# ezorita/seeq

Hardware: AMD Instinct MI355X
Metric: lines/s scanned (20 bp pattern, d=3, 150 bp reads; GB/s in gb_per_s) (higher is better)
Workload: dtype int (u16 automaton state ids; exact-pass columns u32 bit-vectors)

## Files before the change

### include/seeq_amd.h

```cpp
#ifndef SEEQ_AMD_H_
#define SEEQ_AMD_H_

#include <stddef.h>
#include <stdint.h>

#include "libseeq.h"

#ifdef __cplusplus
extern "C" {
#endif

#define SEEQ_AMD_VERSION "seeq-mi355x-0.1"

#define SEEQDEV_MAX_WLEN 512

#define SEEQDEV_WANT_COUNTLINES 0
#define SEEQDEV_WANT_COUNTMATCH 1
#define SEEQDEV_WANT_RECORDS    2

#define SEEQDEV_FASTA       0x100
#define SEEQDEV_SINGLELINE  0x200

typedef struct {
   uint32_t line;
// ... 39 lines not shown

const seeqdev_hit_t * seeqdevScanRecordsDevice(const seeqdev_scan_t * scan);
int seeqdevScanCopyRecords(seeqdev_scan_t * scan, seeqdev_hit_t * host_out, size_t first, size_t n);
int seeqdevScanCopyOffsets(seeqdev_scan_t * scan, uint64_t * host_out, size_t first, size_t n);

void * seeqdevHostAlloc(size_t bytes);
void   seeqdevHostFree(void * p);

void * seeqdevTextAlloc(size_t bytes, int candidates, float * probe_ms, int * nprobed);
typedef struct seeqdev_textinfo {
   float  probe_ms[12];
   int    nprobed;
   int    chosen;
   size_t allocated_bytes;
   size_t probe_peak_bytes;
} seeqdev_textinfo_t;
void * seeqdevTextAllocInfo(size_t bytes, int candidates, seeqdev_textinfo_t * info);
void * seeqdevTextAllocFor(seeqdev_scan_t * scan, size_t bytes, int candidates, seeqdev_textinfo_t * info);
void   seeqdevTextFree(void * d_text);

int seeqdevScanHost(seeqdev_scan_t * scan, const seeqdev_pattern_t * pat, const char * host_text, size_t nbytes,
                    int options, int want, seeqdev_counts_t * counts);

int seeqdevStringMatch(seeqdev_scan_t * scan, const seeqdev_pattern_t * pat, const char * data, size_t n, int options,
                       const seeqdev_hit_t ** rec, size_t * nrec);

int seeqdevScanHostBegin(seeqdev_scan_t * scan, const seeqdev_pattern_t * pat, const char * host_text, size_t nbytes,
                         int options, int want);
int seeqdevScanRunMulti(seeqdev_scan_t * scan, const seeqdev_pattern_t * const * pats, int npat, const void * d_text, size_t nbytes,
                        int options, int want, seeqdev_counts_t * counts);
int seeqdevScanHostMulti(seeqdev_scan_t * scan, const seeqdev_pattern_t * const * pats, int npat, const char * host_text, size_t nbytes,
                         int options, int want, seeqdev_counts_t * counts);
int seeqdevScanMultiRecords(const seeqdev_scan_t * scan, int k, const seeqdev_hit_t ** rec, size_t * nrec);
int seeqdevScanLastMulti(const seeqdev_scan_t * scan);

typedef struct {
   const void * bases;
   const void * nmask;
   uint64_t     nreads;
   uint32_t     read_len;
   uint32_t     stride;
   uint32_t     nstride;
} seeqdev_packed_t;
int  seeqdevScanPacked(seeqdev_scan_t * scan, const seeqdev_pattern_t * pat, const seeqdev_packed_t * batch, int options, int want);
long seeqdevPackReads(const char * text, size_t nbytes, uint32_t read_len, void * bases_out, void * nmask_out, uint32_t stride, uint32_t nstride);
int  seeqdevPackReadsDevice(const void * d_text, uint64_t nreads, uint32_t read_len, void * d_bases, void * d_nmask, uint32_t stride, uint32_t nstride,
                            void * hip_stream);

int seeqdevScanLastCopyMs(const seeqdev_scan_t * scan, float * h2d_ms);

int seeqdevScanSetProfiling(seeqdev_scan_t * scan, int on);
int seeqdevScanLastTimes(const seeqdev_scan_t * scan, float ms[4]);
int seeqdevScanLastLaunches(const seeqdev_scan_t * scan);
int seeqdevScanLastLaunchTimes(const seeqdev_scan_t * scan, float * ms, int cap);
float seeqdevScanLastClockMHz(const seeqdev_scan_t * scan);

int seeqdevSynthReads(void * d_out, uint64_t first, uint64_t n, int len, const char * pattern_plain, int plen,
                      int tau, uint64_t seed, void * hip_stream);

#ifdef __cplusplus
}
#endif
#endif
```

### seeq_amd/_capi.py

```python
import ctypes as C
import os
import subprocess

HERE = os.path.dirname(os.path.abspath(__file__))
LIB_PATH = os.path.join(HERE, "lib", "libseeq_amd.so")
CLI_PATH = os.path.join(HERE, "bin", "seeq")
CSRC = os.path.join(HERE, "csrc")

SQ_FIRST, SQ_BEST, SQ_ALL, SQ_COUNT = 0x00, 0x01, 0x02, 0x03
SQ_FAIL, SQ_CONVERT, SQ_IGNORE = 0x00, 0x04, 0x08
SQ_LINES, SQ_STREAM = 0x00, 0x10
SQ_ANY, SQ_MATCH, SQ_NOMATCH, SQ_COUNTLINES, SQ_COUNTMATCH = 0, 1, 2, 3, 4
WANT_COUNTLINES, WANT_COUNTMATCH, WANT_RECORDS = 0, 1, 2
SEEQDEV_FASTA, SEEQDEV_SINGLELINE = 0x100, 0x200


class match_t(C.Structure):
    _fields_ = [("start", C.c_size_t), ("end", C.c_size_t), ("dist", C.c_size_t)]


class seeq_t(C.Structure):
    _fields_ = [("hits", C.c_size_t), ("stacksize", C.c_size_t), ("match", C.POINTER(match_t)),
                ("bufsz", C.c_size_t), ("string", C.c_void_p), ("tau", C.c_int), ("wlen", C.c_int),
                ("keys", C.POINTER(C.c_char)), ("rkeys", C.POINTER(C.c_char)),
                ("dfa", C.c_void_p), ("rdfa", C.c_void_p)]


class seeqdev_packed_t(C.Structure):
    _fields_ = [("bases", C.c_void_p), ("nmask", C.c_void_p), ("nreads", C.c_uint64), ("read_len", C.c_uint32),
                ("stride", C.c_uint32), ("nstride", C.c_uint32)]


class seeqfile_t(C.Structure):
    _fields_ = [("flags", C.c_int), ("line", C.c_size_t), ("info", C.c_char_p), ("fdi", C.c_void_p)]


class seeqdev_hit_t(C.Structure):
    _fields_ = [("line", C.c_uint32), ("start", C.c_uint32), ("end", C.c_uint32), ("dist", C.c_uint32)]


class seeqdev_counts_t(C.Structure):
    _fields_ = [("nlines", C.c_uint64), ("nmatchlines", C.c_uint64), ("nhits", C.c_uint64),
                ("nrecords", C.c_uint64), ("nheaders", C.c_uint64)]


class seeqdev_textinfo_t(C.Structure):
    _fields_ = [("probe_ms", C.c_float * 12), ("nprobed", C.c_int), ("chosen", C.c_int), ("allocated_bytes", C.c_size_t),
                ("probe_peak_bytes", C.c_size_t)]


EXPORTS = [
    "seeqNew", "seeqFree", "seeqMatchIter", "seeqGetString", "seeqStringMatch", "seeqPrintError",
    "seeqAddMatch", "stackNew", "stackAddMatch", "recursive_merge", "seeqerr",
    "seeq", "seeqFileMatch", "seeqOpen", "seeqClose",
    "seeqdevDeviceCount", "seeqdevSetDevice", "seeqdevLastError", "seeqdevPatternNew", "seeqdevPatternFree",
    "seeqdevPatternOf", "seeqdevScanNew", "seeqdevScanFree", "seeqdevScanReserve", "seeqdevScanRun",
    "seeqdevScanFetch", "seeqdevScanRecordsDevice", "seeqdevScanCopyRecords", "seeqdevScanHost",
    "seeqdevScanSetProfiling", "seeqdevScanLastTimes", "seeqdevScanLastLaunches", "seeqdevScanLastLaunchTimes", "seeqdevScanLastClockMHz", "seeqdevSynthReads",
    "seeqdevScanSetLineHint", "seeqdevScanLastPath", "seeqdevScanLastFilter", "seeqdevScanLastPackedQuad", "seeqdevScanCopyOffsets", "seeqdevHostAlloc", "seeqdevTextAlloc", "seeqdevTextAllocInfo", "seeqdevTextAllocFor", "seeqdevTextFree",
    "seeqdevHostFree", "seeqdevStringMatch", "seeqdevScanHostBegin", "seeqdevScanLastCopyMs", "seeqdevPatternDevice",
    "seeqdevScanRunMulti", "seeqdevScanHostMulti", "seeqdevScanMultiRecords", "seeqdevScanLastMulti", "seeqdevScanPacked", "seeqdevPackReads", "seeqdevPackReadsDevice",
]


def build(verbose=False):
    cmd = ["make", "-C", CSRC, "all"]
    if not verbose:
        cmd.insert(1, "-s")
    subprocess.check_call(cmd)


_lib = None


def _share_torch_hip_runtime():
    if os.environ.get("SEEQ_AMD_SYSTEM_HIP") == "1":
        return
    import importlib.util
    try:
        spec = importlib.util.find_spec("torch")
    except (ImportError, ValueError):
        spec = None
    if spec is None or not spec.submodule_search_locations:
        return
    path = os.path.join(list(spec.submodule_search_locations)[0], "lib", "libamdhip64.so")
    if os.path.exists(path):
        C.CDLL(path, mode=C.RTLD_GLOBAL)


def lib():
    global _lib
    if _lib is not None:
        return _lib
    if not os.path.exists(LIB_PATH):
        raise OSError("%s is not built: run `python -c 'import __graft_entry__ as g; g.build()'` "
                      "or `make -C seeq_amd/csrc`; seeq_amd has no fallback matcher" % LIB_PATH)
    _share_torch_hip_runtime()
    L = C.CDLL(LIB_PATH, use_errno=True)
    P = C.POINTER
    L.seeqNew.argtypes = [C.c_char_p, C.c_int, C.c_size_t]
    L.seeqNew.restype = P(seeq_t)
    L.seeqFree.argtypes = [P(seeq_t)]
    L.seeqFree.restype = None
    L.seeqMatchIter.argtypes = [P(seeq_t)]
    L.seeqMatchIter.restype = P(match_t)
    L.seeqGetString.argtypes = [P(seeq_t)]
    L.seeqGetString.restype = C.c_char_p
    L.seeqStringMatch.argtypes = [C.c_char_p, P(seeq_t), C.c_int]
    L.seeqStringMatch.restype = C.c_long
    L.seeqPrintError.argtypes = []
    L.seeqPrintError.restype = C.c_char_p
    L.seeqAddMatch.argtypes = [P(seeq_t), match_t]
    L.seeqAddMatch.restype = C.c_int
    L.seeqOpen.argtypes = [C.c_char_p]
    L.seeqOpen.restype = P(seeqfile_t)
    L.seeqClose.argtypes = [P(seeqfile_t)]
    L.seeqClose.restype = C.c_int
    L.seeqFileMatch.argtypes = [P(seeqfile_t), P(seeq_t), C.c_int, C.c_int]
    L.seeqFileMatch.restype = C.c_long
    L.seeqdevDeviceCount.argtypes = []
    L.seeqdevDeviceCount.restype = C.c_int
    L.seeqdevSetDevice.argtypes = [C.c_int]
    L.seeqdevSetDevice.restype = C.c_int
    L.seeqdevLastError.argtypes = []
    L.seeqdevLastError.restype = C.c_char_p
    L.seeqdevPatternNew.argtypes = [C.c_char_p, C.c_int, C.c_int]
    L.seeqdevPatternNew.restype = C.c_void_p
    L.seeqdevPatternFree.argtypes = [C.c_void_p]
    L.seeqdevPatternFree.restype = None
    L.seeqdevPatternOf.argtypes = [P(seeq_t)]
    L.seeqdevPatternOf.restype = C.c_void_p
    L.seeqdevScanNew.argtypes = [C.c_void_p]
    L.seeqdevScanNew.restype = C.c_void_p
    L.seeqdevScanFree.argtypes = [C.c_void_p]
    L.seeqdevScanFree.restype = None
    L.seeqdevScanReserve.argtypes = [C.c_void_p, C.c_size_t, C.c_size_t, C.c_size_t, C.c_size_t]
    L.seeqdevScanReserve.restype = C.c_int
    L.seeqdevScanRun.argtypes = [C.c_void_p, C.c_void_p, C.c_void_p, C.c_size_t, C.c_int, C.c_int]
    L.seeqdevScanRun.restype = C.c_int
    L.seeqdevScanFetch.argtypes = [C.c_void_p, P(seeqdev_counts_t)]
    L.seeqdevScanFetch.restype = C.c_int
    L.seeqdevScanRecordsDevice.argtypes = [C.c_void_p]
    L.seeqdevScanRecordsDevice.restype = C.c_void_p
    L.seeqdevScanCopyRecords.argtypes = [C.c_void_p, C.c_void_p, C.c_size_t, C.c_size_t]
    L.seeqdevScanCopyRecords.restype = C.c_int
    L.seeqdevScanCopyOffsets.argtypes = [C.c_void_p, C.c_void_p, C.c_size_t, C.c_size_t]
    L.seeqdevScanCopyOffsets.restype = C.c_int
    L.seeqdevScanHost.argtypes = [C.c_void_p, C.c_void_p, C.c_char_p, C.c_size_t, C.c_int, C.c_int,
                                  P(seeqdev_counts_t)]
    L.seeqdevScanHost.restype = C.c_int
    L.seeqdevScanSetProfiling.argtypes = [C.c_void_p, C.c_int]
    L.seeqdevScanSetProfiling.restype = C.c_int
    L.seeqdevScanLastTimes.argtypes = [C.c_void_p, P(C.c_float)]
    L.seeqdevScanLastTimes.restype = C.c_int
    L.seeqdevScanLastLaunches.argtypes = [C.c_void_p]
    L.seeqdevScanLastLaunches.restype = C.c_int
    L.seeqdevScanLastLaunchTimes.argtypes = [C.c_void_p, P(C.c_float), C.c_int]
    L.seeqdevScanLastLaunchTimes.restype = C.c_int
    L.seeqdevScanLastClockMHz.argtypes = [C.c_void_p]
    L.seeqdevScanLastClockMHz.restype = C.c_float
    L.seeqdevScanSetLineHint.argtypes = [C.c_void_p, C.c_double]
    L.seeqdevScanSetLineHint.restype = C.c_int
    L.seeqdevScanLastPath.argtypes = [C.c_void_p]
    L.seeqdevScanLastPath.restype = C.c_int
    L.seeqdevScanLastFilter.argtypes = [C.c_void_p]
    L.seeqdevScanLastFilter.restype = C.c_int
    L.seeqdevScanLastPackedQuad.argtypes = [C.c_void_p]
    L.seeqdevScanLastPackedQuad.restype = C.c_int
    L.seeqdevScanRunMulti.argtypes = [C.c_void_p, C.POINTER(C.c_void_p), C.c_int, C.c_void_p, C.c_size_t, C.c_int, C.c_int, C.c_void_p]
    L.seeqdevScanRunMulti.restype = C.c_int
    L.seeqdevScanHostMulti.argtypes = [C.c_void_p, C.POINTER(C.c_void_p), C.c_int, C.c_char_p, C.c_size_t, C.c_int, C.c_int, C.c_void_p]
    L.seeqdevScanHostMulti.restype = C.c_int
    L.seeqdevScanMultiRecords.argtypes = [C.c_void_p, C.c_int, C.POINTER(C.c_void_p), C.POINTER(C.c_size_t)]
    L.seeqdevScanMultiRecords.restype = C.c_int
    L.seeqdevScanLastMulti.argtypes = [C.c_void_p]
    L.seeqdevScanLastMulti.restype = C.c_int
    L.seeqdevScanPacked.argtypes = [C.c_void_p, C.c_void_p, C.POINTER(seeqdev_packed_t), C.c_int, C.c_int]
    L.seeqdevScanPacked.restype = C.c_int
    L.seeqdevPackReads.argtypes = [C.c_char_p, C.c_size_t, C.c_uint32, C.c_void_p, C.c_void_p, C.c_uint32, C.c_uint32]
    L.seeqdevPackReads.restype = C.c_long
    L.seeqdevPackReadsDevice.argtypes = [C.c_void_p, C.c_uint64, C.c_uint32, C.c_void_p, C.c_void_p, C.c_uint32, C.c_uint32, C.c_void_p]
    L.seeqdevPackReadsDevice.restype = C.c_int
    L.seeqdevHostAlloc.argtypes = [C.c_size_t]
    L.seeqdevHostAlloc.restype = C.c_void_p
    L.seeqdevHostFree.argtypes = [C.c_void_p]
    L.seeqdevHostFree.restype = None
    L.seeqdevTextAlloc.argtypes = [C.c_size_t, C.c_int, C.POINTER(C.c_float), C.POINTER(C.c_int)]
    L.seeqdevTextAlloc.restype = C.c_void_p
    L.seeqdevTextAllocInfo.argtypes = [C.c_size_t, C.c_int, C.POINTER(seeqdev_textinfo_t)]
    L.seeqdevTextAllocInfo.restype = C.c_void_p
    L.seeqdevTextAllocFor.argtypes = [C.c_void_p, C.c_size_t, C.c_int, C.POINTER(seeqdev_textinfo_t)]
    L.seeqdevTextAllocFor.restype = C.c_void_p
    L.seeqdevTextFree.argtypes = [C.c_void_p]
    L.seeqdevTextFree.restype = None
    L.seeqdevSynthReads.argtypes = [C.c_void_p, C.c_uint64, C.c_uint64, C.c_int, C.c_char_p, C.c_int, C.c_int,
                                    C.c_uint64, C.c_void_p]
    L.seeqdevSynthReads.restype = C.c_int
    _lib = L
    return L


def seeqerr():
    return C.c_int.in_dll(lib(), "seeqerr").value


def error_text():
    L = lib()
    msg = L.seeqPrintError().decode(errors="replace")
    dev = L.seeqdevLastError().decode(errors="replace")
# ... 2 lines not shown
```

### seeq_amd/csrc/seeq_device.hip

```cpp
#include <hip/hip_runtime.h>

#include <errno.h>
#include <pthread.h>
#include <stdint.h>
#include <stdio.h>
#include <stdlib.h>
#include <string.h>
#include <time.h>

#include "seeq_amd.h"
#include "seeq_kernel_core.h"
extern "C" {
#include "seeq_pattern.h"
}

static thread_local char g_last_error[256] = "";

static int hip_fail(hipError_t e, const char *what, int err_no)
{
   snprintf(g_last_error, sizeof g_last_error, "%s: %s", what, hipGetErrorString(e));
   seeqerr = 0;
   errno = err_no;
   return -1;
}
// ... 741 lines not shown
      uint32_t *wg_part;
      uint32_t *wg_lastnl;
   } ow;
   size_t cap_ftiles, cap_slices;
   uint32_t *d_eqtab, *h_eqtab;
   unsigned long eq_pat_id; int eq_options;
   double avg_line;
   double line_hint;
   uint8_t *h_sample;
   const void *avg_text; size_t avg_nbytes;
   int force_path;
   int last_path;
   seeqdev_hit_t *records; uint64_t *rec_off; size_t cap_records;
   uint32_t *scan_ws;           size_t cap_scan_ws;
   uint32_t *lead_fidx, *lead_flag, *lead_wend; unsigned long long *lead_key; size_t cap_lead;
   Counters *d_cnt;
   Counters *h_cnt;
   uint8_t *h_str; size_t cap_str;
   uint32_t *h_strout; size_t cap_strout;
   uint32_t  str_seq;
   uint8_t *d_text; size_t cap_text;
   seeqdev_counts_t *multi_cnt; size_t *multi_first; int multi_n, cap_multi_n;
   seeqdev_hit_t *multi_rec; size_t cap_multi_rec, multi_nrec;
   struct MultiPlan *mplan;
   bool      multi_active;
   int       multi_rc;
   uint32_t *ml_mask, *ml_first, *ml_last; size_t cap_ml;
   uint32_t *mp_idx, *mp_nh; size_t cap_mp;
   uint32_t *m_bsum; size_t cap_m_bsum;
   Counters *d_mcnt, *h_mcnt;
   MultiExact *d_mx, *h_mx; size_t mx_slots, mx_next;
   uint32_t *m_scan_ws; size_t cap_m_scan_ws;
   int       last_multi;
   uint32_t *pk_cand, *pk_slot, *pk_coff; uint64_t *pk_bmask; size_t cap_pk_reads;
   uint8_t  *pk_stage; size_t cap_pk_stage;
   uint8_t  *d_unpack; size_t cap_unpack;
   uint32_t *pk_last; size_t cap_pk_last;
   bool      is_packed; seeqdev_packed_t packed;
   const seeqdev_pattern *pat; const void *text; size_t nbytes; int options, want;
   bool ran;
   seeqdev_counts_t counts;
   bool prof;
   hipEvent_t *ev;
   size_t nev_seg;
   size_t prof_segs;
   float acc_ms[4];
   float fwd_ms_avg;
   size_t seg_bytes;
   bool user_reserved;
   bool no_stream;
   bool force_ll;
   bool no_stream_nd;
   bool no_leaders;
   bool no_window;
   int  fallback_ttl;
   bool sample_dirty;
   unsigned sample_age;
};

static int ws_alloc(void **p, size_t bytes)
{
   void *g = NULL;
   hipError_t e = hipMalloc(&g, bytes ? bytes : 16);
   if (e != hipSuccess) { (void)hipGetLastError(); return hip_fail(e, "hipMalloc(workspace)", ENOMEM); }
   if (*p) (void)hipFree(*p);
   *p = g;
   return 0;
}

extern "C" seeqdev_scan_t *seeqdevScanNew(void *hip_stream)
{
   seeqerr = 0;
   if (seeqdevDeviceCount() < 1) {
      snprintf(g_last_error, sizeof g_last_error, "no HIP device: seeq-mi355x has no CPU matcher");
      errno = ENODEV;
      return NULL;
   }
   seeqdev_scan *s = (seeqdev_scan *)calloc(1, sizeof *s);
   if (!s) return NULL;
   if (hipGetDevice(&s->device) != hipSuccess) s->device = 0;
   s->seg_bytes = (size_t)0xF0000000u;
   const char *env = getenv("SEEQ_SEGMENT_BYTES");
   if (env && atoll(env) >= 65536) s->seg_bytes = ((size_t)atoll(env) + 15) & ~(size_t)15;
   if (s->seg_bytes > 0xFFFF0000ull) s->seg_bytes = 0xFFFF0000ull;
   hipError_t e = hipSuccess;
   if (hip_stream) s->stream = (hipStream_t)hip_stream;
   else {
      e = hipStreamCreateWithFlags(&s->stream, hipStreamDefault);
      s->own_stream = true;
   }
   if (e == hipSuccess) e = hipMalloc((void **)&s->d_cnt, sizeof(Counters));
   if (e == hipSuccess) e = hipHostMalloc((void **)&s->h_cnt, sizeof(Counters), hipHostMallocDefault);
   if (e == hipSuccess) e = hipHostMalloc((void **)&s->h_eqtab, 2048 * sizeof(uint32_t), hipHostMallocDefault);
   if (e == hipSuccess) e = hipMalloc((void **)&s->d_eqtab, 2048 * sizeof(uint32_t));
   if (e == hipSuccess) e = hipHostMalloc((void **)&s->h_sample, SAMPLE_BYTES, hipHostMallocDefault);
   {
      const char *pe = getenv("SEEQ_PATH");
      s->force_path = pe ? (!strcmp(pe, "generic") ? 1 : !strcmp(pe, "fused") ? 2 : 0) : 0;
      ScanKnobs &kn = s->knobs;
      const char *v;
      v = getenv("SEEQ_FUSED_KERNEL"); kn.kernel = v ? (!strcmp(v, "stream") ? 1 : !strcmp(v, "direct") ? 2 : !strcmp(v, "pair") ? 3 : 0) : 0;
      v = getenv("SEEQ_NO_LEADERS");   kn.no_leaders = v && atoi(v) == 1;
      v = getenv("SEEQ_TILE_BYTES");   kn.tile_bytes = v ? atoi(v) : 0;
      v = getenv("SEEQ_NO_FILTER");    kn.no_filter = v && atoi(v) == 1;
      v = getenv("SEEQ_STREAM_SUB");   kn.no_sub = v && atoi(v) == 0;
      v = getenv("SEEQ_STREAM_WU");    kn.min_wu = v ? atoi(v) : 0;
      v = getenv("SEEQ_NO_MYERS");     kn.no_myers = v && atoi(v) == 1;
      v = getenv("SEEQ_NO_WINDOW");    kn.no_window = v && atoi(v) == 1;
      v = getenv("SEEQ_EXPLAIN");      kn.explain = v && atoi(v) == 1;
      v = getenv("SEEQ_PACKED_QUAD");  kn.no_packed_quad = v && atoi(v) == 0;
      v = getenv("SEEQ_PACKED_SEG_READS");
      s->pk_seg_reads = v && atol(v) >= 64 && (size_t)atol(v) <= ((size_t)1 << 26) ? (size_t)atol(v) & ~(size_t)63 : PACKED_SEG_READS_DEFAULT;
      s->ncu = 256;
      s->lds_per_wg = 65536;
      s->lds_per_cu = 65536;
      int dev = 0;
      hipDeviceProp_t prop;
      if (e == hipSuccess && hipGetDevice(&dev) == hipSuccess && hipGetDeviceProperties(&prop, dev) == hipSuccess)
      { s->ncu = prop.multiProcessorCount; s->lds_per_wg = prop.sharedMemPerBlock; s->lds_per_cu = prop.maxSharedMemoryPerMultiProcessor; }
   }
   if (e != hipSuccess) {
      hip_fail(e, "seeqdevScanNew", EIO);
      seeqdevScanFree(s);
      return NULL;
   }
   return s;
}

extern "C" void seeqdevScanFree(seeqdev_scan_t *s)
{
   if (!s) return;
   (void)use_device(s->device);
   if (s->have_h2d_ev) { (void)hipEventDestroy(s->ev_h2d[0]); (void)hipEventDestroy(s->ev_h2d[1]); }
   (void)hipStreamSynchronize(s->stream);
   {
      void *ob[] = {s->ow.tile_cl, s->ow.tile_hits, s->ow.tile_dirty, s->ow.tile_dmask, s->ow.tmp, s->ow.wg_hits, s->ow.wg_part, s->ow.wg_lastnl};
      for (void *b : ob) if (b) (void)hipFree(b);
   }
   { void *pk[] = {s->pk_cand, s->pk_slot, s->pk_coff, s->pk_bmask, s->pk_stage, s->pk_last, s->d_unpack}; for (void *b : pk) if (b) (void)hipFree(b); }
   { void *mw[] = {s->ml_mask, s->ml_first, s->ml_last, s->mp_idx, s->mp_nh, s->m_bsum, s->d_mcnt, s->d_mx, s->m_scan_ws}; for (void *b : mw) if (b) (void)hipFree(b); }
   if (s->h_mcnt) (void)hipHostFree(s->h_mcnt);
   if (s->h_mx) (void)hipHostFree(s->h_mx);
   multi_plan_free(s->mplan);
   void *bufs[] = {s->rec_off, s->line_start, s->tile_cnt, s->hitmask, s->hdrmask, s->wave_off, s->hdr_off, s->hit_start,
                   s->hit_line, s->d_eqtab,
                   s->nh, s->hit_col, s->nh_sum, s->ent, s->records, s->scan_ws, s->lead_fidx, s->lead_flag, s->lead_wend, s->lead_key, s->d_cnt, s->d_text};
   for (void *b : bufs) if (b) (void)hipFree(b);
   if (s->h_cnt) (void)hipHostFree(s->h_cnt);
   if (s->h_eqtab) (void)hipHostFree(s->h_eqtab);
   if (s->h_sample) (void)hipHostFree(s->h_sample);
   if (s->h_str) (void)hipHostFree(s->h_str);
   if (s->h_strout) (void)hipHostFree(s->h_strout);
   for (size_t i = 0; i < 4 * s->nev_seg; i++) (void)hipEventDestroy(s->ev[i]);
   free(s->ev);
   free(s->launch_ms);
   if (s->clk_probe) (void)hipHostFree(s->clk_probe);
   free(s->multi_cnt); free(s->multi_first);
   if (s->multi_rec) (void)hipHostFree(s->multi_rec);
   if (s->own_stream && s->stream) (void)hipStreamDestroy(s->stream);
   free(s);
}

static int reserve_impl(seeqdev_scan *s, size_t max_bytes, size_t max_lines, size_t max_hitlines, size_t max_records)
{
   seeqerr = 0;
   if (!s) { errno = EINVAL; return -1; }
   if (max_bytes) {
      const size_t seg = max_bytes < s->seg_bytes ? max_bytes : s->seg_bytes;
      const size_t tiles = (seg + TILE - 1) / TILE + 1;
      if (tiles > s->cap_tiles) {
         if (ws_alloc((void **)&s->tile_cnt, tiles * sizeof(uint32_t))) return -1;
         s->cap_tiles = tiles;
      }
      const size_t ftiles = seg / FUSED_MIN_TILE + 2;
      const size_t slices = MAX_FUSED_GRID;
      if (ftiles > s->cap_ftiles) {
         if (ws_alloc((void **)&s->ow.tile_cl, ftiles * sizeof(uint32_t))) return -1;
         if (ws_alloc((void **)&s->ow.tile_dirty, ftiles * sizeof(uint32_t))) return -1;
         if (ws_alloc((void **)&s->ow.tile_dmask, ftiles * sizeof(uint64_t))) return -1;
         if (ws_alloc((void **)&s->ow.tile_hits, ftiles * sizeof(uint32_t))) return -1;
         s->cap_ftiles = ftiles;
      }
      if (slices > s->cap_slices) {
         if (ws_alloc((void **)&s->ow.wg_hits, slices * sizeof(uint32_t))) return -1;
         if (ws_alloc((void **)&s->ow.wg_part, 4 * slices * sizeof(uint32_t))) return -1;
         if (ws_alloc((void **)&s->ow.wg_lastnl, slices * sizeof(uint32_t))) return -1;
         s->cap_slices = slices;
      }
   }
   if (max_lines > s->cap_lines) {
      const size_t chunks = (max_lines + 63) / 64 + 1;
      if (ws_alloc((void **)&s->line_start, (max_lines + 1) * sizeof(uint32_t))) return -1;
      if (ws_alloc((void **)&s->hitmask, chunks * sizeof(uint64_t))) return -1;
      if (ws_alloc((void **)&s->hdrmask, chunks * sizeof(uint64_t))) return -1;
      if (ws_alloc((void **)&s->wave_off, chunks * sizeof(uint32_t))) return -1;
      if (ws_alloc((void **)&s->hdr_off, chunks * sizeof(uint32_t))) return -1;
      s->cap_lines = max_lines;
      s->cap_chunks = chunks;
   }
   if (max_hitlines > s->cap_hitlines) {
      if (ws_alloc((void **)&s->hit_start, max_hitlines * sizeof(uint32_t))) return -1;
      if (ws_alloc((void **)&s->hit_line, max_hitlines * sizeof(uint32_t))) return -1;
      if (ws_alloc((void **)&s->ow.tmp, max_hitlines * sizeof(uint4))) return -1;
      if (ws_alloc((void **)&s->nh, max_hitlines * sizeof(uint32_t))) return -1;
      if (ws_alloc((void **)&s->hit_col, max_hitlines * sizeof(uint32_t))) return -1;
      if (ws_alloc((void **)&s->ent, max_hitlines * sizeof(uint4))) return -1;
      if (ws_alloc((void **)&s->nh_sum, 2 * (max_hitlines / 256 + 2) * sizeof(uint32_t))) return -1;
      s->cap_hitlines = max_hitlines;
   }
   if (max_records > s->cap_records) {
      if (ws_alloc((void **)&s->records, max_records * sizeof(seeqdev_hit_t))) return -1;
      if (ws_alloc((void **)&s->rec_off, max_records * sizeof(uint64_t))) return -1;
      s->cap_records = max_records;
   }
   size_t largest = s->cap_tiles;
   if (s->cap_chunks > largest) largest = s->cap_chunks;
   if (s->cap_hitlines > largest) largest = s->cap_hitlines;
   if (s->cap_ftiles > largest) largest = s->cap_ftiles;
   size_t nb = largest / SCAN_BLOCK + 2;
   if (3 * (s->cap_ftiles / SCAN_BLOCK + 2) > nb) nb = 3 * (s->cap_ftiles / SCAN_BLOCK + 2);
   if (nb > s->cap_scan_ws) {
      if (ws_alloc((void **)&s->scan_ws, nb * sizeof(uint32_t))) return -1;
      s->cap_scan_ws = nb;
   }
   return 0;
}

extern "C" int seeqdevScanReserve(seeqdev_scan_t *s, size_t max_bytes, size_t max_lines, size_t max_hitlines,
                                  size_t max_records)
{
   if (reserve_impl(s, max_bytes, max_lines, max_hitlines, max_records)) return -1;
   if (max_lines) s->user_reserved = true;
   return 0;
}

extern "C" int seeqdevScanSetLineHint(seeqdev_scan_t *s, double avg_bytes_per_line)
{
   if (!s || avg_bytes_per_line < 0) { errno = EINVAL; return -1; }
   s->line_hint = avg_bytes_per_line;
   return 0;
}

extern "C" int seeqdevScanLastPath(const seeqdev_scan_t *s) { return s ? s->last_path : 0; }
extern "C" int seeqdevScanLastFilter(const seeqdev_scan_t *s) { return s && s->last_filter ? 1 : 0; }
extern "C" int seeqdevScanLastPackedQuad(const seeqdev_scan_t *s) { return s && s->last_packed_quad ? 1 : 0; }

extern "C" int seeqdevScanSetProfiling(seeqdev_scan_t *s, int on)
{
   if (!s) { errno = EINVAL; return -1; }
   s->prof = on != 0;
   return 0;
}

extern "C" int seeqdevScanLastTimes(const seeqdev_scan_t *s, float ms[4])
{
   if (!s || !ms) { errno = EINVAL; return -1; }
   for (int i = 0; i < 4; i++) ms[i] = s->acc_ms[i];
   return 0;
}

struct ScanSet { uint32_t *arr[3]; uint32_t *total[3]; };

__global__ __launch_bounds__(WG) void k_scanset_reduce(ScanSet ss, uint32_t *bsum, uint32_t n, uint32_t nb)
{
   __shared__ uint32_t s_wave[4];
   const uint32_t *in = ss.arr[blockIdx.y];
   const uint32_t base = blockIdx.x * SCAN_BLOCK;
   uint32_t v = 0;
#pragma unroll
   for (int k = 0; k < SCAN_ITEMS; k++) {
      const uint32_t i = base + threadIdx.x * SCAN_ITEMS + k;
      if (i < n) v += in[i];
   }
// ... 228 lines not shown
         }
         int per_cu = occupancy_of(s, stream_fn, 64 * nw, dfa_lds);
         if (per_cu < 0) return -1;
         fused_grid = (unsigned)(ncu * per_cu);
         if ((size_t)fused_grid * nw > MAX_FUSED_GRID) fused_grid = (unsigned)(MAX_FUSED_GRID / nw);
         nslices = fused_grid * nw;
      } else {
         nw = 4;
         double want = s->avg_line * 63.5;
         if (want < 512) want = 512;
         if (want > DIRECT_MAXRR * 1024) want = DIRECT_MAXRR * 1024;
         tile_bytes = ((uint32_t)want) & ~15u;
         if (kn.tile_bytes >= 512 && kn.tile_bytes <= DIRECT_MAXRR * 1024) tile_bytes = (uint32_t)kn.tile_bytes & ~15u;
         int per_cu = occupancy_of(s, fw == 1 ? (const void *)k_direct<4, 1> : (const void *)k_direct<4, 2>, 256, 0);
         if (per_cu < 0) return -1;
         fused_grid = (unsigned)(ncu * per_cu);
         if ((size_t)fused_grid * nw > MAX_FUSED_GRID) fused_grid = (unsigned)(MAX_FUSED_GRID / nw);
         nslices = fused_grid * nw;
      }
      if (eq_tables_upload(s, pat, options, fw)) return -1;
   }
   const bool use_direct = plan.use_direct;
   s->last_path = plan.path;
   s->last_filter = filter;
   const bool superset = plan.superset;
   const bool need_nh = plan.need_nh, nh_is_count = plan.nh_is_count;

   const size_t seg_bytes = single ? (nbytes ? nbytes : 1) : s->seg_bytes;
   if (single && nbytes > 0xFFFF0000ull) { seeqerr = 0; errno = E2BIG; return -1; }
   const size_t nseg = nbytes ? (nbytes + seg_bytes - 1) / seg_bytes : 0;
   s->prof_segs = 0;
   if (s->prof && nseg > s->nev_seg) {
      hipEvent_t *g = (hipEvent_t *)realloc(s->ev, 4 * nseg * sizeof(hipEvent_t));
      if (!g) { seeqerr = 0; errno = ENOMEM; return -1; }
      s->ev = g;
      for (size_t i = 4 * s->nev_seg; i < 4 * nseg; i++) HIP_TRY(hipEventCreate(&s->ev[i]), EIO);
      s->nev_seg = nseg;
   }
   if (s->prof) s->prof_segs = nseg;
   if (s->prof && nseg > s->cap_clk_probe) {
      if (s->clk_probe) (void)hipHostFree(s->clk_probe);
      s->clk_probe = nullptr; s->cap_clk_probe = 0;
      if (hipHostMalloc((void **)&s->clk_probe, nseg * 4 * sizeof(unsigned long long), hipHostMallocDefault) == hipSuccess) s->cap_clk_probe = nseg;
   }
   if (s->prof && s->clk_probe) memset(s->clk_probe, 0, nseg * 4 * sizeof(unsigned long long));
   s->clk_valid = s->prof && s->clk_probe && use_pair && use_fused;
   r.pat = pat; r.options = options; r.want = want;
   r.fw = fw; r.nw = nw; r.tile_bytes = tile_bytes; r.fused_grid = fused_grid; r.nslices = nslices; r.grid_lines = grid_lines;
   r.stream_fn = stream_fn; r.dfa_lds = dfa_lds; r.seg_bytes = seg_bytes; r.nseg = nseg;
   (void)use_direct; (void)superset; (void)need_nh; (void)nh_is_count; (void)use_myers;
   return 0;
}

static int seg_onepass(seeqdev_scan *s, const SegRun &r, ScanArgs &a, size_t sg, hipEvent_t *ev, bool &order2, uint32_t &stream_ntiles)
{
   const seeqdev_pattern *pat = r.pat;
   const int options = r.options, want = r.want, match_opt = r.options & 3, fw = r.fw, ncu = s->ncu;
   const ScanPlan &plan = r.plan;
   const bool fasta = (options & SEEQDEV_FASTA) != 0, single = (options & SEEQDEV_SINGLELINE) != 0;
   const bool use_stream = plan.use_stream, use_pair = plan.use_pair, use_myers = plan.use_myers, filter = plan.filter, use_fused = plan.use_fused, use_direct = plan.use_direct;
   const bool stream_ll = plan.stream_ll, superset = plan.superset, need_nh = plan.need_nh, nh_is_count = plan.nh_is_count;
   const int stream_sub = plan.stream_sub, stream_ch = 128, nw = r.nw;
   const uint32_t tile_bytes = r.tile_bytes;
   const unsigned fused_grid = r.fused_grid, nslices = r.nslices, grid_lines = r.grid_lines;
   const void *stream_fn = r.stream_fn;
   const size_t dfa_lds = r.dfa_lds, nbytes = s->nbytes;
   Counters *c = s->d_cnt;
   seeqdev_scan::OnePassWs &ow = s->ow;
   hipStream_t st = s->stream;
   (void)pat; (void)want; (void)match_opt; (void)fw; (void)ncu; (void)fasta; (void)single; (void)use_stream; (void)use_pair; (void)use_myers; (void)filter; (void)use_fused;
   (void)use_direct; (void)stream_ll; (void)superset; (void)need_nh; (void)nh_is_count; (void)stream_sub; (void)stream_ch; (void)nw; (void)tile_bytes; (void)fused_grid;
   (void)nslices; (void)grid_lines; (void)stream_fn; (void)dfa_lds; (void)nbytes; (void)c; (void)ow; (void)st;

   FusedArgs f;
   memset(&f, 0, sizeof f);
   f.text = a.text; f.nbytes = nbytes; f.seg_base = a.seg_base; f.seg_len = a.seg_len; f.first_seg = a.first_seg;
   f.tile_bytes = tile_bytes;
   f.ntiles = (uint32_t)(((uint64_t)a.seg_len + tile_bytes - 1) / tile_bytes);
   stream_ntiles = f.ntiles;
   f.eqtab = s->d_eqtab; f.peq = pat->d_peq;
   f.m = pat->wlen; f.tau = pat->tau; f.options = options; f.want = want;
   f.tile_cl = ow.tile_cl; f.tile_hits = ow.tile_hits; f.tmp = ow.tmp; f.cap_tmp = (uint32_t)s->cap_hitlines;
   f.wg_hits = ow.wg_hits; f.wg_part = ow.wg_part; f.wg_lastnl = stream_ll ? ow.wg_lastnl : nullptr;
   f.tile_dirty = f.wg_lastnl ? ow.tile_dirty : nullptr;
   f.tile_dmask = f.wg_lastnl ? ow.tile_dmask : nullptr;
   f.cnt = c;
   f.clk_probe = (s->prof && s->clk_probe && use_pair) ? s->clk_probe + 4 * sg : nullptr;
   uint32_t pos_bias = 0;
   if (use_stream) {
      f.dfa = stream_sub == 2 ? pat->d_sdfa_skip : plan.ll_restart ? pat->d_sdfa_restart : pat->d_sdfa; f.dfa_rows = pat->sdfa_rows; f.dfa_final_base = pat->sdfa_final_base;
      f.ll_filter = plan.ll_restart ? 2u : plan.ll_filter ? 1u : 0u;
      f.skip_thr = plan.skip_thr;
      if (use_pair) { f.dfa = pat->d_pair; f.dfa_rows = pat->pair_units; f.dfa_final_base = 0; f.pair = 1; f.ig_thr = plan.ig ? (uint32_t)(pat->wlen - pat->tau) : 0u; }
      if (use_myers) { f.dfa = (const uint16_t *)(s->d_eqtab + (size_t)512 * fw); f.dfa_rows = (uint32_t)(64 * fw); f.dfa_final_base = 0; f.pair = 2; }
      uint64_t room = 0xFFFFFFF0ull - a.seg_len;
      if (room > ((uint64_t)1 << 30)) room = (uint64_t)1 << 30;
      pos_bias = (uint32_t)(a.seg_base < room ? a.seg_base : room) & ~127u;
      f.pos_bias = pos_bias;
   }
   if (ev) { HIP_TRY(hipEventRecord(ev[0], st), EIO); HIP_TRY(hipEventRecord(ev[1], st), EIO); }
   unsigned fgrid = fused_grid;
   const unsigned nsl = nslices;
   f.slice_cap = f.cap_tmp / nsl;
   if (use_stream) {
      void *kargs[] = {&f};
      HIP_TRY(hipLaunchKernel(stream_fn, dim3(fgrid), dim3(64 * (unsigned)nw), kargs, dfa_lds, st), EIO);
   }
   else if (use_direct && fw == 2) hipLaunchKernelGGL((k_direct<4, 2>), dim3(fgrid), dim3(256), 0, st, f);
   else hipLaunchKernelGGL((k_direct<4, 1>), dim3(fgrid), dim3(256), 0, st, f);
   if (ev) HIP_TRY(hipEventRecord(ev[2], st), EIO);
   const uint32_t order_nb = (f.ntiles + SEEQ_ORDER_BLOCK - 1) / SEEQ_ORDER_BLOCK;
   order2 = plan.order2 && order_nb <= SEEQ_ORDER_MAX_BLOCKS && 2 * (size_t)order_nb <= s->cap_scan_ws;
   if (plan.ig) {
      if (!order2) { snprintf(g_last_error, sizeof g_last_error, "SQ_IGNORE on k_pair needs the three-launch ordering (segment too large for its block sums)"); seeqerr = 0; errno = EIO; return -1; }
      a.ig_thr = f.ig_thr; a.ig_ent = (const uint4 *)s->ent;
      {
         static const char base_of_key[9] = {0, 'A', 'C', 0, 'G', 0, 0, 0, 'T'};
         int cnt[4] = {0, 0, 0, 0}, best = 3;
         for (int i = 0; i < pat->wlen; i++) { const int kb = pat->keys[i] & 0x1F; if (kb == 1) cnt[0]++; else if (kb == 2) cnt[1]++; else if (kb == 4) cnt[2]++; else if (kb == 8) cnt[3]++; }
         for (int b = 2; b >= 0; b--) if (cnt[b] > cnt[best]) best = b;
         const int need = cnt[best] - pat->tau;
         a.ig_need = need > 0 ? (uint32_t)need : 0u;
         a.ig_bval = (uint32_t)(unsigned char)base_of_key[1 << best];
         a.ig_bmask = best == 3 ? 0xDEu : 0xDFu;
      }
   }
   if (order2) {
      const unsigned rgrid = nsl / 4 + 1 < 2048 ? nsl / 4 + 1 : 2048;
      seeq_launch_tiles_post(st, f, (uint32_t)nsl, s->scan_ws, order_nb);
      seeq_launch_order(rgrid, st, f, (uint32_t)nsl, (const uint32_t *)s->scan_ws, order_nb, s->ent);
   }
   else hipLaunchKernelGGL(k_fused_post, dim3(1), dim3(256), 0, st, f, (uint32_t)nsl);
   if (!order2 && (want != SEEQDEV_WANT_COUNTLINES || superset)) {
      launch_scanset(s, st, f.tile_hits, f.tile_cl, f.tile_dirty, f.ntiles, nullptr, nullptr, f.tile_dirty ? &c->seg_dirty_tiles : nullptr);
      const unsigned rgrid = nsl / 4 + 1 < 2048 ? nsl / 4 + 1 : 2048;
      if (use_stream) hipLaunchKernelGGL(k_stream_reorder, dim3(rgrid), dim3(256), 0, st, f, (uint32_t)nsl, s->hit_start, s->hit_line, s->nh, s->hit_col);
      else hipLaunchKernelGGL(k_fused_reorder, dim3(rgrid), dim3(256), 0, st, f, (uint32_t)nsl, s->hit_start, s->hit_line);
   }
   a.seg_base -= pos_bias;
   a.pos_bias = pos_bias;
   a.tile_dirty = f.tile_dirty; a.tile_dmask = f.tile_dmask; a.stream_ntiles = f.ntiles; a.stream_tile_bytes = tile_bytes;
   a.stream_ch = stream_ll ? (uint32_t)stream_ch : 0u;
   a.walk_ext = plan.walk_ext; a.ll_restart = plan.ll_restart ? 1u : 0u;
   return 0;
}

template <int W>
static int seg_index_forward(seeqdev_scan *s, const SegRun &r, ScanArgs &a, hipEvent_t *ev)
{
   const seeqdev_pattern *pat = r.pat;
   const int options = r.options, want = r.want, match_opt = r.options & 3, fw = r.fw, ncu = s->ncu;
   const ScanPlan &plan = r.plan;
   const bool fasta = (options & SEEQDEV_FASTA) != 0, single = (options & SEEQDEV_SINGLELINE) != 0;
   const bool use_stream = plan.use_stream, use_pair = plan.use_pair, use_myers = plan.use_myers, filter = plan.filter, use_fused = plan.use_fused, use_direct = plan.use_direct;
   const bool stream_ll = plan.stream_ll, superset = plan.superset, need_nh = plan.need_nh, nh_is_count = plan.nh_is_count;
   const int stream_sub = plan.stream_sub, stream_ch = 128, nw = r.nw;
   const uint32_t tile_bytes = r.tile_bytes;
   const unsigned fused_grid = r.fused_grid, nslices = r.nslices, grid_lines = r.grid_lines;
   const void *stream_fn = r.stream_fn;
   const size_t dfa_lds = r.dfa_lds, nbytes = s->nbytes;
   Counters *c = s->d_cnt;
   seeqdev_scan::OnePassWs &ow = s->ow;
   hipStream_t st = s->stream;
   (void)pat; (void)want; (void)match_opt; (void)fw; (void)ncu; (void)fasta; (void)single; (void)use_stream; (void)use_pair; (void)use_myers; (void)filter; (void)use_fused;
   (void)use_direct; (void)stream_ll; (void)superset; (void)need_nh; (void)nh_is_count; (void)stream_sub; (void)stream_ch; (void)nw; (void)tile_bytes; (void)fused_grid;
   (void)nslices; (void)grid_lines; (void)stream_fn; (void)dfa_lds; (void)nbytes; (void)c; (void)ow; (void)st;

   if (ev) HIP_TRY(hipEventRecord(ev[0], st), EIO);
   if (single) {
      hipLaunchKernelGGL(k_single_line, dim3(1), dim3(1), 0, st, a);
   } else {
      hipLaunchKernelGGL(k_nl_count, dim3(a.ntiles), dim3(WG), 0, st, a);
      hipLaunchKernelGGL(k_scan_tiles, dim3(1), dim3(WG), 0, st, a.tile_cnt, a.ntiles, &c->seg_nlines);
      hipLaunchKernelGGL(k_index_finalize, dim3(1), dim3(1), 0, st, a);
      hipLaunchKernelGGL(k_nl_write, dim3(a.ntiles), dim3(WG), 0, st, a);
   }
   if (ev) HIP_TRY(hipEventRecord(ev[1], st), EIO);
   hipLaunchKernelGGL(k_forward<W>, dim3(grid_lines), dim3(WG), 0, st, a);
   if (ev) HIP_TRY(hipEventRecord(ev[2], st), EIO);
   launch_scan<1>(s, st, a.hitmask, a.wave_off, s->cap_chunks, &c->seg_nlines, 63u, 6u, &c->seg_nhitlines);
   if (fasta) launch_scan<1>(s, st, a.hdrmask, a.hdr_off, s->cap_chunks, &c->seg_nlines, 63u, 6u, &c->seg_nheaders);
   return 0;
}

template <int W>
static int seg_post(seeqdev_scan *s, const SegRun &r, ScanArgs &a, hipEvent_t *ev, bool order2, uint32_t stream_ntiles)
{
   const seeqdev_pattern *pat = r.pat;
   const int options = r.options, want = r.want, match_opt = r.options & 3, fw = r.fw, ncu = s->ncu;
   const ScanPlan &plan = r.plan;
   const bool fasta = (options & SEEQDEV_FASTA) != 0, single = (options & SEEQDEV_SINGLELINE) != 0;
   const bool use_stream = plan.use_stream, use_pair = plan.use_pair, use_myers = plan.use_myers, filter = plan.filter, use_fused = plan.use_fused, use_direct = plan.use_direct;
   const bool stream_ll = plan.stream_ll, superset = plan.superset, need_nh = plan.need_nh, nh_is_count = plan.nh_is_count;
// ... 66 lines not shown
   #define SEEQ_COUNT1(WW, WK) hipLaunchKernelGGL((k_exact1<SQ_MODE_COUNT, WW, -1, WK>), dim3(grid_hits), dim3(WG), 0, st, a, eqp, hcol, ecache)
         if (fw == 2) { if (a.stream_ch) SEEQ_COUNT1(2, true); else SEEQ_COUNT1(2, false); }
         else { if (a.stream_ch) SEEQ_COUNT1(1, true); else SEEQ_COUNT1(1, false); }
   #undef SEEQ_COUNT1
      }
      else hipLaunchKernelGGL((k_exact<W, SQ_MODE_COUNT>), dim3(grid_hits), dim3(WG), 0, st, a);
      if (leaders) {
         hipLaunchKernelGGL(k_lead_check, dim3(grid_hits), dim3(256), 0, st, a, (const uint32_t *)s->hit_col, (const uint32_t *)s->lead_flag, lead_wback);
         if (lead_best) {
            hipLaunchKernelGGL(k_lead_best, dim3(grid_hits), dim3(256), 0, st, a, (const uint32_t *)s->lead_fidx, s->lead_key, (const uint4 *)ecache, 0);
            hipLaunchKernelGGL(k_lead_best, dim3(grid_hits), dim3(256), 0, st, a, (const uint32_t *)s->lead_fidx, s->lead_key, (const uint4 *)ecache, 1);
         }
         else hipLaunchKernelGGL(k_lead_lines, dim3(grid_hits < 512 ? grid_hits : 512), dim3(256), 0, st, a, (const uint32_t *)s->lead_fidx, s->lead_flag);
      }
      else if (superset && nh_is_count) hipLaunchKernelGGL(k_count_nonzero, dim3(grid_hits < 512 ? grid_hits : 512), dim3(WG), 0, st, a);
      launch_scan<0>(s, st, a.nh, a.nh, s->cap_hitlines, &c->seg_nhitlines, 0u, 0u, &c->seg_nrec);
   }
   if (want == SEEQDEV_WANT_RECORDS && !emitted) {
      if (!verify) hipLaunchKernelGGL(k_rec_check, dim3(1), dim3(1), 0, st, a);
      if (use_fused) {
         const uint32_t *eqp = (const uint32_t *)s->d_eqtab;
         const int mo = (options & 3) == SQ_COUNT ? SQ_FIRST : (options & 3);
   #define SEEQ_EMIT1(WW, OO, WK) hipLaunchKernelGGL((k_exact1<SQ_MODE_EMIT, WW, OO, WK>), dim3(grid_hits), dim3(WG), 0, st, a, eqp, hcol, ecache)
         if (a.stream_ch) {
            if (fw == 2) { if (mo == SQ_BEST) SEEQ_EMIT1(2, SQ_BEST, true); else SEEQ_EMIT1(2, -1, true); }
            else { if (mo == SQ_BEST) SEEQ_EMIT1(1, SQ_BEST, true); else SEEQ_EMIT1(1, -1, true); }
         } else {
            if (fw == 2) { if (mo == SQ_BEST) SEEQ_EMIT1(2, SQ_BEST, false); else SEEQ_EMIT1(2, -1, false); }
            else { if (mo == SQ_BEST) SEEQ_EMIT1(1, SQ_BEST, false); else SEEQ_EMIT1(1, -1, false); }
         }
   #undef SEEQ_EMIT1
      }
      else {
         hipLaunchKernelGGL((k_exact<W, SQ_MODE_EMIT>), dim3(grid_hits), dim3(WG), 0, st, a);
         hipLaunchKernelGGL(k_rec_offsets, dim3(grid_hits), dim3(WG), 0, st, a);
      }
   }
   return 0;
}

template <int W>
static int run_segments(seeqdev_scan *s)
{
   Counters *c = s->d_cnt;
   HIP_TRY(hipMemsetAsync(c, 0, sizeof(Counters), s->stream), EIO);
   SegRun r;
   memset(&r, 0, sizeof r);
   { const int rc = run_setup(s, r); if (rc) return rc; }
   const seeqdev_pattern *pat = r.pat;
   const ScanPlan &plan = r.plan;
   const int options = r.options, want = r.want;
   const size_t nbytes = s->nbytes, seg_bytes = r.seg_bytes, nseg = r.nseg;
   const bool use_stream = plan.use_stream, use_fused = plan.use_fused, filter = plan.filter, superset = plan.superset, need_nh = plan.need_nh, nh_is_count = plan.nh_is_count;
   for (size_t sg = 0; sg < nseg; sg++) {

      hipEvent_t *ev = s->prof ? s->ev + 4 * sg : NULL;
      uint32_t stream_ntiles = 0;
      bool order2 = false;
      hipStream_t st = s->stream;
      ScanArgs a;
      memset(&a, 0, sizeof a);
      a.text = (const uint8_t *)s->text;
      a.nbytes = nbytes;
      a.seg_base = (uint64_t)sg * seg_bytes;
      a.seg_len = (uint32_t)((nbytes - a.seg_base) < seg_bytes ? (nbytes - a.seg_base) : seg_bytes);
      a.first_seg = sg == 0;
      a.peq = pat->d_peq;
      a.m = pat->wlen; a.tau = pat->tau; a.options = options; a.want = want;
      a.line_start = s->line_start; a.cap_lines = (uint32_t)s->cap_lines;
      a.tile_cnt = s->tile_cnt; a.ntiles = (a.seg_len + TILE - 1) / TILE;
      a.hitmask = s->hitmask; a.hdrmask = s->hdrmask; a.wave_off = s->wave_off; a.hdr_off = s->hdr_off;
      a.hit_start = s->hit_start; a.hit_line = s->hit_line; a.cap_hitlines = (uint32_t)s->cap_hitlines; a.nh = s->nh;
      a.records = s->records; a.cap_records = s->cap_records; a.rec_off = s->rec_off;
      a.use_nh = need_nh ? (use_stream ? 3u : 1u) : 0u;
      a.filter = filter ? 1u : 0u;
      a.skip_back = plan.skip_back;
      a.window_ok = plan.window_ok ? 1u : 0u;
      a.cnt = c;

      if (use_fused) { if (seg_onepass(s, r, a, sg, ev, order2, stream_ntiles)) return -1; }
      else if (seg_index_forward<W>(s, r, a, ev)) return -1;
      if (want != SEEQDEV_WANT_COUNTLINES || superset) {
         const int pr = seg_post<W>(s, r, a, ev, order2, stream_ntiles);
         if (pr < 0) return pr;
         if (pr > 0) continue;
      }
      if (!a.fin) hipLaunchKernelGGL(k_seg_end, dim3(1), dim3(1), 0, st, a, (need_nh ? 1 : 0) | (superset && !nh_is_count ? 2 : 0));
      if (ev) HIP_TRY(hipEventRecord(ev[3], st), EIO);
      HIP_TRY(hipGetLastError(), EIO);
   }
   HIP_TRY(hipMemcpyAsync(s->h_cnt, c, sizeof(Counters), hipMemcpyDeviceToHost, s->stream), EIO);
   return 0;
}


static int run_packed(seeqdev_scan *s)
{
   const seeqdev_pattern *pat = s->pat;
   const seeqdev_packed_t &b = s->packed;
   const int options = s->options, want = s->want;
   const int match_opt = options & 3;
   const bool nh_is_count = want == SEEQDEV_WANT_COUNTMATCH || (want == SEEQDEV_WANT_RECORDS && match_opt == SQ_ALL);
   const int fw = pat->wlen <= FUSED_MAX_WLEN ? 1 : 2;
   Counters *c = s->d_cnt;
   hipStream_t st = s->stream;
   const uint32_t L = b.read_len;
   const bool direct = !(want == SEEQDEV_WANT_RECORDS && match_opt == SQ_ALL);
   const uint32_t pitch = (L + 1u + 15u) & ~15u;
   size_t PACKED_SEG_READS = s->pk_seg_reads;
   const size_t stage_lines_max = (size_t)(0xFFFF0000ull / pitch);
   if (!direct && PACKED_SEG_READS + 64u * MAX_FUSED_GRID > stage_lines_max)
      PACKED_SEG_READS = (stage_lines_max - 64u * MAX_FUSED_GRID) & ~(size_t)63;
   const size_t seg_reads = b.nreads < PACKED_SEG_READS ? (size_t)b.nreads : PACKED_SEG_READS;
   const size_t cap_use = (!direct && s->cap_hitlines > stage_lines_max) ? stage_lines_max : s->cap_hitlines;
   if (seg_reads > s->cap_pk_reads) {
      if (ws_alloc((void **)&s->pk_cand, seg_reads * sizeof(uint32_t))) return -1;
      if (ws_alloc((void **)&s->pk_slot, seg_reads * sizeof(uint32_t))) return -1;
      if (ws_alloc((void **)&s->pk_coff, (seg_reads / 64 + 1) * sizeof(uint32_t))) return -1;
      if (ws_alloc((void **)&s->pk_bmask, (seg_reads / 64 + 1) * sizeof(uint64_t))) return -1;
      s->cap_pk_reads = seg_reads;
   }
   if (!direct && cap_use * (size_t)pitch > s->cap_pk_stage) {
      if (ws_alloc((void **)&s->pk_stage, cap_use * (size_t)pitch + 64)) return -1;
      s->cap_pk_stage = cap_use * (size_t)pitch;
   }
   if (s->cap_hitlines > s->cap_pk_last) {
      if (ws_alloc((void **)&s->pk_last, s->cap_hitlines * sizeof(uint32_t))) return -1;
      s->cap_pk_last = s->cap_hitlines;
   }
   {
      const size_t nb = seg_reads / SCAN_BLOCK + 2;
      if (nb > s->cap_scan_ws) { if (ws_alloc((void **)&s->scan_ws, nb * sizeof(uint32_t))) return -1; s->cap_scan_ws = nb; }
   }
   if (eq_tables_upload(s, pat, options, fw)) return -1;
   HIP_TRY(hipMemsetAsync(c, 0, sizeof(Counters), st), EIO);
   s->clk_valid = false;
   const bool quad = pat->quad_state == 1 && !s->knobs.no_packed_quad && (pat->quad_pacc - pat->pair_pacc) * (double)L <= 0.04;
   s->last_packed_quad = quad;
   const size_t dfa_lds = quad ? (size_t)pat->quad_units * 16 : (size_t)pat->pair_units * 16;
   const void *walk_fn = quad ? (const void *)k_packed_walk<true> : (const void *)k_packed_walk<false>;
   int per_cu = occupancy_of(s, walk_fn, 64 * STREAM_NW, dfa_lds);
   if (per_cu < 0) return -1;
   unsigned wgrid = (unsigned)(s->ncu * per_cu);
   {
      const size_t nblocks = (seg_reads + 63) / 64, need = (nblocks + STREAM_NW_HOST - 1) / STREAM_NW_HOST;
      if (need < wgrid) wgrid = (unsigned)(need ? need : 1);
   }
   const size_t hit_blocks = (s->cap_hitlines + WG - 1) / WG;
   unsigned grid_hits = (unsigned)(hit_blocks < (size_t)s->ncu * 16 ? hit_blocks : (size_t)s->ncu * 16);
   if (grid_hits == 0) grid_hits = 1;
   const size_t nseg = (size_t)((b.nreads + PACKED_SEG_READS - 1) / PACKED_SEG_READS);
   s->prof_segs = 0;
   if (s->prof && nseg > s->nev_seg) {
      hipEvent_t *g = (hipEvent_t *)realloc(s->ev, 4 * nseg * sizeof(hipEvent_t));
      if (!g) { seeqerr = 0; errno = ENOMEM; return -1; }
      s->ev = g;
      for (size_t i = 4 * s->nev_seg; i < 4 * nseg; i++) HIP_TRY(hipEventCreate(&s->ev[i]), EIO);
      s->nev_seg = nseg;
   }
   if (s->prof) s->prof_segs = nseg;
   for (size_t sg = 0; sg < nseg; sg++) {
      hipEvent_t *ev = s->prof ? s->ev + 4 * sg : NULL;
      PackedArgs p;
      memset(&p, 0, sizeof p);
      p.bases = (const uint8_t *)b.bases; p.nmask = (const uint8_t *)b.nmask;
      p.first = (uint64_t)sg * PACKED_SEG_READS;
      p.nreads = (uint32_t)(b.nreads - p.first < PACKED_SEG_READS ? b.nreads - p.first : PACKED_SEG_READS);
      p.read_len = L; p.stride = b.stride; p.nstride = b.nstride;
      p.total_bytes = b.nreads * (uint64_t)b.stride;
      p.dfa = quad ? pat->d_quad : pat->d_pair; p.dfa_units = quad ? pat->quad_units : pat->pair_units;
      p.cand = s->pk_cand; p.cslot = s->pk_slot; p.boff = s->pk_coff; p.bmask = s->pk_bmask; p.stage = direct ? nullptr : s->pk_stage;
      p.wave_cap = (uint32_t)(cap_use / ((size_t)wgrid * STREAM_NW_HOST));
      p.pitch = pitch;
      p.hit_start = s->hit_start; p.hit_line = s->hit_line; p.hit_col = s->hit_col; p.hit_last = s->pk_last; p.nh = s->nh;
      p.cap = (uint32_t)cap_use;
      p.line_base = p.first;
      p.cnt = c;
      if (ev) { HIP_TRY(hipEventRecord(ev[0], st), EIO); HIP_TRY(hipEventRecord(ev[1], st), EIO); }
      {
         void *kargs[] = {&p};
         HIP_TRY(hipLaunchKernel(walk_fn, dim3(wgrid), dim3(64 * STREAM_NW), kargs, dfa_lds, st), EIO);
      }
      if (ev) HIP_TRY(hipEventRecord(ev[2], st), EIO);
      launch_scanset(s, st, s->pk_coff, nullptr, nullptr, (p.nreads + 63u) >> 6, &c->seg_nhitlines, nullptr, nullptr);
      hipLaunchKernelGGL(k_packed_counts, dim3(1), dim3(1), 0, st, p);
      hipLaunchKernelGGL(k_packed_list, dim3((unsigned)(((size_t)p.nreads / 1024 + 4) / 4)), dim3(256), 0, st, p);
      ScanArgs a;
      memset(&a, 0, sizeof a);
      a.text = direct ? nullptr : s->pk_stage;
      a.nbytes = direct ? 0 : cap_use * (uint64_t)pitch;
      a.seg_base = 0; a.seg_len = (uint32_t)a.nbytes; a.first_seg = sg == 0;
      a.peq = pat->d_peq;
      a.m = pat->wlen; a.tau = pat->tau; a.options = options & ~(MASK_NONDNA | MASK_INPUT); a.want = want;
      a.hit_start = s->hit_start; a.hit_line = s->hit_line; a.cap_hitlines = (uint32_t)s->cap_hitlines; a.nh = s->nh;
      a.records = s->records; a.cap_records = s->cap_records; a.rec_off = s->rec_off;
      a.use_nh = 3u; a.filter = 1u;
      a.skip_back = (uint32_t)(pat->wlen + pat->tau);
      a.hit_last = s->pk_last;
      a.window_ok = 1u;
      a.cnt = c;
      a.rec_pitch = L + 1u;
      const uint32_t *eqp = (const uint32_t *)s->d_eqtab;
      const uint32_t *hcol = s->hit_col;
      uint4 *ecache = want == SEEQDEV_WANT_RECORDS ? s->ow.tmp : nullptr;
      const int seg_flags = 1 | (!nh_is_count ? 2 : 0);
      {
         const bool count_any = want != SEEQDEV_WANT_COUNTMATCH && !(want == SEEQDEV_WANT_RECORDS && match_opt == SQ_ALL);
         const int var = (want == SEEQDEV_WANT_RECORDS && match_opt == SQ_BEST) ? VERIFY_BEST : count_any ? VERIFY_ANY : VERIFY_ALL;
         a.nh_sum = s->nh_sum;
         a.nz_sum = nh_is_count ? s->nh_sum + (s->cap_hitlines / 256 + 2) : nullptr;
         a.fin = (want == SEEQDEV_WANT_RECORDS && var == VERIFY_ALL) ? 0u : 1u + (uint32_t)seg_flags;
         if (direct) seeq_launch_verify_packed(fw, var, grid_hits, st, a, b.bases, b.nmask, b.stride, b.nstride, L, p.total_bytes,
                                               b.nmask ? b.nreads * (uint64_t)b.nstride : 0ull, eqp, hcol, ecache);
// ... 138 lines not shown
   if (nh_is_count) hipLaunchKernelGGL(k_multi_count_nonzero, dim3(grid_hits < 128 ? grid_hits : 128, (unsigned)npat), dim3(WG), 0, st, (const MultiExact *)dx);
   hipLaunchKernelGGL(k_multi_scan_reduce, dim3(nbp, (unsigned)npat), dim3(WG), 0, st, (const MultiExact *)dx);
   hipLaunchKernelGGL(k_multi_scan_top, dim3((unsigned)npat), dim3(WG), 0, st, (const MultiExact *)dx, want == SEEQDEV_WANT_RECORDS ? 1 : 0);
   hipLaunchKernelGGL(k_multi_scan_apply, dim3(nbp, (unsigned)npat), dim3(WG), 0, st, (const MultiExact *)dx);
   if (want == SEEQDEV_WANT_RECORDS) {
      if (mo == SQ_BEST) {
         if (n1) hipLaunchKernelGGL((k_exact1m<SQ_MODE_EMIT, 1, SQ_BEST>), dim3(grid_hits, (unsigned)n1), dim3(WG), 0, st, (const MultiExact *)dx);
         if (n2) hipLaunchKernelGGL((k_exact1m<SQ_MODE_EMIT, 2, SQ_BEST>), dim3(grid_hits, (unsigned)n2), dim3(WG), 0, st, (const MultiExact *)(dx + n1));
      } else {
         if (n1) hipLaunchKernelGGL((k_exact1m<SQ_MODE_EMIT, 1, -1>), dim3(grid_hits, (unsigned)n1), dim3(WG), 0, st, (const MultiExact *)dx);
         if (n2) hipLaunchKernelGGL((k_exact1m<SQ_MODE_EMIT, 2, -1>), dim3(grid_hits, (unsigned)n2), dim3(WG), 0, st, (const MultiExact *)(dx + n1));
      }
   }
   hipLaunchKernelGGL(k_multi_seg_end, dim3((unsigned)npat), dim3(1), 0, st, (const MultiExact *)dx);
   HIP_TRY(hipGetLastError(), EIO);
   return 0;
}

static int dispatch_run(seeqdev_scan *s)
{
   if (s->is_packed) return run_packed(s);
   const int W = s->pat->words;
   if (W <= 1) return run_segments<1>(s);
   if (W <= 2) return run_segments<2>(s);
   if (W <= 4) return run_segments<4>(s);
   if (W <= 8) return run_segments<8>(s);
   return run_segments<16>(s);
}

static int scan_setup(seeqdev_scan_t *s, const seeqdev_pattern_t *pat, const void *d_text, size_t nbytes, int options, int want, int hl_div);

extern "C" int seeqdevScanRun(seeqdev_scan_t *s, const seeqdev_pattern_t *pat, const void *d_text, size_t nbytes,
                              int options, int want)
{
   if (scan_setup(s, pat, d_text, nbytes, options, want, 8)) return -1;
   if (dispatch_run(s)) return -1;
   s->ran = true;
   return 0;
}

static int scan_setup(seeqdev_scan_t *s, const seeqdev_pattern_t *pat, const void *d_text, size_t nbytes, int options, int want, int hl_div)
{
   seeqerr = 0;
   if (!s || !pat || (!d_text && nbytes) || want < 0 || want > 2) { errno = EINVAL; return -1; }
   if (pat->device != s->device) {
      snprintf(g_last_error, sizeof g_last_error, "pattern lives on device %d, scan context on device %d", pat->device, s->device);
      errno = EINVAL;
      return -1;
   }
   if (use_device(s->device)) return -1;
   s->pat = pat; s->text = d_text; s->nbytes = nbytes; s->options = options; s->want = want;
   s->ran = false;
   s->is_packed = false;
   if ((s->no_stream || s->no_stream_nd || s->force_ll || s->no_window || s->no_leaders) && --s->fallback_ttl <= 0) s->no_stream = s->no_stream_nd = s->force_ll = s->no_window = s->no_leaders = false;
   const size_t seg = nbytes < s->seg_bytes ? nbytes : s->seg_bytes;
   size_t want_lines = s->cap_lines, want_hl = s->cap_hitlines, want_rec = s->cap_records;
   if (!s->user_reserved) {
      const size_t guess = (options & SEEQDEV_SINGLELINE) ? 1 : seg / 32 + 1024;
      if (guess > want_lines) want_lines = guess;
      if (want_lines / (size_t)hl_div + 1024 > want_hl) want_hl = want_lines / (size_t)hl_div + 1024;
      if (!(options & SEEQDEV_SINGLELINE) && want_hl < (size_t)8192 * 64) want_hl = (size_t)8192 * 64;
      if (want_hl > want_rec) want_rec = want_hl;
   }
   if (reserve_impl(s, nbytes ? nbytes : 1, want_lines, want_hl, want_rec)) return -1;
   if (s->line_hint > 0) {
      s->avg_line = s->line_hint;
   } else if (!(options & SEEQDEV_SINGLELINE) && nbytes && (s->avg_text != d_text || s->avg_nbytes != nbytes || ++s->sample_age >= 64)) {
      s->sample_age = 0;
      const size_t n = nbytes < SAMPLE_BYTES ? nbytes : SAMPLE_BYTES;
      HIP_TRY(hipMemcpyAsync(s->h_sample, d_text, n, hipMemcpyDeviceToHost, s->stream), EIO);
      HIP_TRY(hipStreamSynchronize(s->stream), EIO);
      size_t nl = 0;
      size_t foreign = 0;
      for (size_t i = 0; i < n; i++) {
         const uint8_t b = s->h_sample[i];
         nl += b == '\n';
         foreign += b != '\n' && sq_class_of(b, 0) >= 5;
      }
      s->avg_line = nl ? (double)n / (double)nl : 1e9;
      s->sample_dirty = foreign * 4096 > n;
      s->avg_text = d_text;
      s->avg_nbytes = nbytes;
   }
   return 0;
}

extern "C" int seeqdevScanFetch(seeqdev_scan_t *s, seeqdev_counts_t *counts)
{
   seeqerr = 0;
   if (!s || !s->ran) { errno = EINVAL; return -1; }
   if (use_device(s->device)) return -1;
   for (int attempt = 0; attempt < 8; attempt++) {
      HIP_TRY(hipStreamSynchronize(s->stream), EIO);
      const Counters h = *s->h_cnt;
      if (!h.overflow) {
         s->counts.nlines = h.lines;
         s->counts.nmatchlines = h.matchlines;
         s->counts.nhits = h.hits;
         s->counts.nrecords = h.records;
         s->counts.nheaders = h.headers;
         if (counts) *counts = s->counts;
         for (int i = 0; i < 4; i++) s->acc_ms[i] = 0.f;
         s->fwd_ms_avg = 0.f;
         for (size_t sg = 0; sg < s->prof_segs; sg++) {
            hipEvent_t *ev = s->ev + 4 * sg;
            float t01 = 0, t12 = 0, t23 = 0;
            if (sg == 0 && s->prof_segs > s->cap_launch_ms) {
               float *g = (float *)realloc(s->launch_ms, s->prof_segs * sizeof(float));
               if (g) { s->launch_ms = g; s->cap_launch_ms = s->prof_segs; }
            }
            (void)hipEventElapsedTime(&t01, ev[0], ev[1]);
            (void)hipEventElapsedTime(&t12, ev[1], ev[2]);
            (void)hipEventElapsedTime(&t23, ev[2], ev[3]);
            s->acc_ms[0] += t01; s->acc_ms[1] += t12; s->acc_ms[2] += t23; s->acc_ms[3] += t01 + t12 + t23;
            if (sg < s->cap_launch_ms) s->launch_ms[sg] = t12;
         }
         s->clk_mhz = 0.f;
         if (s->clk_valid && s->prof_segs && s->clk_probe && s->cap_clk_probe >= s->prof_segs) {
            double sum = 0; size_t nn = 0;
            for (size_t sg = 0; sg < s->prof_segs; sg++) {
               const unsigned long long *q = s->clk_probe + 4 * sg;
               if (q[3] > q[1] && q[2] > q[0]) { sum += (double)(q[2] - q[0]) / (double)(q[3] - q[1]) * 100.0; nn++; }
            }
            if (nn) s->clk_mhz = (float)(sum / (double)nn);
         }
         if (s->prof_segs) s->fwd_ms_avg = s->acc_ms[1] / (float)s->prof_segs;
         s->h2d_ms = 0.f;
         if (s->prof && s->have_h2d_ev) (void)hipEventElapsedTime(&s->h2d_ms, s->ev_h2d[0], s->ev_h2d[1]);
         return 0;
      }
      size_t nl = s->cap_lines, nhl = s->cap_hitlines, nrec = s->cap_records;
      if (h.overflow & 1u) nl = (size_t)h.need_lines + (h.need_lines >> 3) + 64;
      if (h.overflow & 2u) nhl = (size_t)h.need_hitlines + (h.need_hitlines >> 3) + 64;
      if (h.overflow & 64u) {
         snprintf(g_last_error, sizeof g_last_error, "internal inconsistency in the hit list (k_stream_bounds)");
         errno = EIO;
         return -1;
      }
      if (h.overflow & 8u) s->no_stream = true;
      if (h.overflow & 16u) s->no_stream_nd = true;
      if (h.overflow & 32u) s->force_ll = true;
      if (h.overflow & 128u) s->no_window = true;
      if (h.overflow & 256u) s->no_leaders = true;
      if (h.overflow & (8u | 16u | 32u | 128u | 256u)) s->fallback_ttl = 32;
      if (h.overflow & 4u) {
         nrec = (size_t)h.need_records + (size_t)(h.need_records >> 3) + 64;
      }
      if ((h.overflow & 1u) && nhl < nl / 8) nhl = nl / 8 + 64;
      if (attempt == 7) break;
      if (reserve_impl(s, s->nbytes, nl, nhl, nrec)) return -1;
      if (dispatch_run(s)) return -1;
   }
   snprintf(g_last_error, sizeof g_last_error, "workspace did not converge");
   errno = ENOMEM;
   return -1;
}

extern "C" const seeqdev_hit_t *seeqdevScanRecordsDevice(const seeqdev_scan_t *s) { return s ? s->records : NULL; }

extern "C" int seeqdevScanCopyRecords(seeqdev_scan_t *s, seeqdev_hit_t *host_out, size_t first, size_t n)
{
   seeqerr = 0;
   if (!s || (!host_out && n)) { errno = EINVAL; return -1; }
   if (first + n > s->counts.nrecords) { errno = EINVAL; return -1; }
   if (n == 0) return 0;
   if (use_device(s->device)) return -1;
   HIP_TRY(hipMemcpyAsync(host_out, s->records + first, n * sizeof(seeqdev_hit_t), hipMemcpyDeviceToHost, s->stream),
           EIO);
   HIP_TRY(hipStreamSynchronize(s->stream), EIO);
   return 0;
}

extern "C" int seeqdevScanPacked(seeqdev_scan_t *s, const seeqdev_pattern_t *pat, const seeqdev_packed_t *batch, int options, int want)
{
   seeqerr = 0;
   if (!s || !pat || !batch || want < 0 || want > 2 || (batch->nreads && !batch->bases)) { errno = EINVAL; return -1; }
   if (batch->read_len < 1 || batch->read_len > 256 || batch->stride < (batch->read_len + 3) / 4 ||
       (batch->nmask && batch->nstride < (batch->read_len + 7) / 8) || (options & (MASK_INPUT | SEEQDEV_FASTA | SEEQDEV_SINGLELINE))) { errno = EINVAL; return -1; }
   if (pat->device != s->device) { errno = EINVAL; return -1; }
   if (use_device(s->device)) return -1;
   seeqdev_pattern *mp = const_cast<seeqdev_pattern *>(pat);
   if (pat->wlen <= FUSED_MAX_WLEN2 && __atomic_load_n(&mp->pair_state, __ATOMIC_ACQUIRE) == 0) pattern_plan_pair(mp);
   if (pat->wlen <= FUSED_MAX_WLEN2 && mp->pair_state == 1 && __atomic_load_n(&mp->quad_state, __ATOMIC_ACQUIRE) == 0) pattern_plan_quad(mp);
   if (pat->wlen > FUSED_MAX_WLEN2 || mp->pair_state != 1) {
      const size_t tbytes = (size_t)batch->nreads * (batch->read_len + 1u);
      if (tbytes > s->cap_unpack) {
         if (ws_alloc((void **)&s->d_unpack, tbytes + 64)) return -1;
         s->cap_unpack = tbytes;
      }
      if (batch->nreads) {
         const uint64_t threads = batch->nreads * (uint64_t)(batch->read_len / 16u + 1u), blocks = (threads + 255) / 256;
         if (blocks > 0x7FFFFFFFull) { errno = E2BIG; return -1; }
         hipLaunchKernelGGL(k_unpack_ascii, dim3((unsigned)blocks), dim3(256), 0, s->stream, (const uint8_t *)batch->bases, (const uint8_t *)batch->nmask,
                            batch->nreads, batch->read_len, batch->stride, batch->nstride, s->d_unpack);
         HIP_TRY(hipGetLastError(), EIO);
      }
      s->avg_text = NULL;
// ... 346 lines not shown
   }
   s->multi_nrec = 0;
   for (int k = 0; k < npat; k++) {
      if (seeqdevScanRun(s, pats[k], d_text, nbytes, options, want)) return -1;
      if (seeqdevScanFetch(s, &s->multi_cnt[k])) return -1;
      s->multi_first[k] = s->multi_nrec;
      const size_t n = want == SEEQDEV_WANT_RECORDS ? (size_t)s->multi_cnt[k].nrecords : 0;
      if (n) {
         if (multi_grow_host(s, n)) return -1;
         if (seeqdevScanCopyRecords(s, s->multi_rec + s->multi_nrec, 0, n)) return -1;
         s->multi_nrec += n;
      }
      if (counts) counts[k] = s->multi_cnt[k];
   }
   s->multi_first[npat] = s->multi_nrec;
   s->multi_n = npat;
   return 0;
}

extern "C" int seeqdevScanLastMulti(const seeqdev_scan_t *s) { return s ? s->last_multi : 0; }

extern "C" int seeqdevScanHostMulti(seeqdev_scan_t *s, const seeqdev_pattern_t *const *pats, int npat, const char *host_text, size_t nbytes,
                                    int options, int want, seeqdev_counts_t *counts)
{
   seeqerr = 0;
   if (!s || !pats || npat < 1 || (!host_text && nbytes)) { errno = EINVAL; return -1; }
   if (use_device(s->device)) return -1;
   if (nbytes > s->cap_text) {
      const size_t cap = nbytes + (nbytes >> 2) + 4096;
      if (ws_alloc((void **)&s->d_text, cap)) return -1;
      s->cap_text = cap;
   }
   if (nbytes) HIP_TRY(hipMemcpyAsync(s->d_text, host_text, nbytes, hipMemcpyHostToDevice, s->stream), EIO);
   s->avg_text = NULL;
   return seeqdevScanRunMulti(s, pats, npat, s->d_text, nbytes, options, want, counts);
}

extern "C" int seeqdevScanMultiRecords(const seeqdev_scan_t *s, int k, const seeqdev_hit_t **rec, size_t *nrec)
{
   if (!s || !rec || !nrec || k < 0 || k >= s->multi_n) { errno = EINVAL; return -1; }
   *rec = s->multi_rec + s->multi_first[k];
   *nrec = s->multi_first[k + 1] - s->multi_first[k];
   return 0;
}

extern "C" int seeqdevScanLastCopyMs(const seeqdev_scan_t *s, float *h2d_ms)
{
   if (!s || !h2d_ms) { errno = EINVAL; return -1; }
   *h2d_ms = s->h2d_ms;
   return 0;
}

extern "C" int seeqdevScanLastLaunches(const seeqdev_scan_t *s) { return s ? (int)s->prof_segs : 0; }

extern "C" float seeqdevScanLastClockMHz(const seeqdev_scan_t *s) { return s ? s->clk_mhz : 0.f; }

extern "C" int seeqdevScanLastLaunchTimes(const seeqdev_scan_t *s, float *ms, int cap)
{
   if (!s || (!ms && cap > 0)) { errno = EINVAL; return -1; }
   const size_t n = s->prof_segs < s->cap_launch_ms ? s->prof_segs : s->cap_launch_ms;
   for (size_t i = 0; i < n && (int)i < cap; i++) ms[i] = s->launch_ms[i];
   return (int)n;
}

static constexpr uint32_t STRING_LDS_MAX = 48u * 1024;
static constexpr uint32_t STRING_ZC_MAX = 4096;
static constexpr uint32_t STRING_PAR_MAX = 32768;

template <int W>
__global__ __launch_bounds__(WG) void k_string(const uint8_t *text, uint32_t n, const uint32_t *peq, int m, int tau, int options,
                                               uint32_t *out, uint32_t cap, uint32_t seq)
{
   extern __shared__ __align__(16) uint8_t s_text[];
   __shared__ uint32_t s_peq[10 * W];
   __shared__ uint8_t s_lut[256];
   const int Wp = (m + 31) >> 5;
   for (int i = threadIdx.x; i < 10 * W; i += WG) {
      const int dir = i / (5 * W), rem = i % (5 * W), cls = rem / W, w = rem % W;
      s_peq[i] = w < Wp ? peq[(dir * 5 + cls) * Wp + w] : 0u;
   }
   for (int b = threadIdx.x; b < 256; b += WG) s_lut[b] = sq_class_of((uint32_t)b, options);
   const bool staged = n <= STRING_LDS_MAX;
   if (staged) {
      for (uint32_t o = threadIdx.x * 16; o < n; o += WG * 16) {
         const sq_chunk16_t c = sq_load16(text, o, n);
         *reinterpret_cast<uint4 *>(s_text + o) = make_uint4(c.w[0], c.w[1], c.w[2], c.w[3]);
      }
   }
   __shared__ uint32_t s_first, s_skip, s_key, s_wave[WG / 64];
   const bool par = n <= STRING_PAR_MAX;
   if (threadIdx.x == 0) { s_first = n; s_skip = 0; s_key = 0xFFFFFFFFu; }
   __syncthreads();
   if (par) {
      for (uint32_t j = threadIdx.x; j < n; j += WG) if (s_lut[s_text[j]] == SQC_TERM) atomicMin(&s_first, j);
      __syncthreads();
      const uint32_t len = s_first;
      for (uint32_t j = threadIdx.x; j < len; j += WG) if (s_lut[s_text[j]] == SQC_SKIP) s_skip = 1u;
      __syncthreads();
      if (!s_skip) {
         const int match_opt = options & 3;
         const uint32_t *peq_f = s_peq, *peq_r = s_peq + 5 * W;
         uint16_t *ed = reinterpret_cast<uint16_t *>(s_text + (((size_t)n + 31) & ~(size_t)15));
         const uint32_t P = len + 1;
         const uint32_t B = (P + WG - 1) / WG;
         const uint32_t j0 = threadIdx.x * B, j1 = j0 + B < P ? j0 + B : P;
         const uint32_t cnt = j0 < P ? sq_emit_window<W>((const uint8_t *)s_text, len, j0, j1, peq_f, (const uint8_t *)s_lut, m, tau, ed) : 0u;
// ... 136 lines not shown
```

### seeq_amd/csrc/seeq_exact1.h

```cpp
#ifndef SEEQ_EXACT1_H_
#define SEEQ_EXACT1_H_

#define EXACT1_ROW 80
typedef __attribute__((address_space(3))) uint8_t exact1_lds_u8;
typedef __attribute__((address_space(3))) const uint8_t exact1_lds_cu8;

template <int W>
__device__ __forceinline__ uint32_t exact1_reverse(const uint8_t *text, uint64_t off, uint64_t nbytes, uint32_t i, uint32_t streak,
                                                   uint32_t eqr_base, uint32_t m, uint32_t tau1, uint8_t *row)
{
   const uint8_t *line = text + off;
   uint32_t lim = 0;
   if (row) {
      const uint64_t end = off + i;
      const uint64_t base = end >= 64 ? end - 64 : 0;
      lim = (uint32_t)(end - base);
#pragma unroll
      for (int q = 0; q < 4; q++)
         *reinterpret_cast<fused_v4u *>(row + 16 * q) = direct_load16(text, base + 16 * q, nbytes);
   }
   fused_state_t<W> st;
   st.init(m);
   uint32_t j = 0, d = tau1, last_d, ignores = 0;
   do {
// ... 68 lines not shown
       !exact1_clean_in_tile(a, segb + t_hi * TB, a.tile_dmask[t_hi], segb + t_hi * TB, hi)) return false;
   return true;
}

template <int W> __device__ __forceinline__ void exact1_take(fused_state_t<W> &st, const fused_state_t<W> &s2, bool take);
template <> __device__ __forceinline__ void exact1_take<1>(fused_state_t<1> &st, const fused_state_t<1> &s2, bool take)
{
   st.pv = take ? s2.pv : st.pv; st.mv = take ? s2.mv : st.mv; st.score = take ? s2.score : st.score;
}
template <> __device__ __forceinline__ void exact1_take<2>(fused_state_t<2> &st, const fused_state_t<2> &s2, bool take)
{
   st.pv0 = take ? s2.pv0 : st.pv0; st.pv1 = take ? s2.pv1 : st.pv1;
   st.mv0 = take ? s2.mv0 : st.mv0; st.mv1 = take ? s2.mv1 : st.mv1; st.score = take ? s2.score : st.score;
}

template <int MODE, int W, int OPT, bool WALK>
__device__ __forceinline__ void exact1_body(const ScanArgs &a, const uint32_t *eq2, const uint32_t *hit_col, uint4 *cache)
{
   __shared__ __align__(8) uint32_t s_eqf[256 * W];
   __shared__ __align__(8) uint32_t s_eqr[256 * W];
   __shared__ __align__(16) uint8_t s_blk[256 * EXACT1_ROW];
   __shared__ uint32_t s_novf[4];
   if (threadIdx.x < 4) s_novf[threadIdx.x] = 0;
   for (int i = threadIdx.x; i < 256 * W; i += 256) { s_eqf[i] = eq2[i]; s_eqr[i] = eq2[256 * W + i]; }
   __syncthreads();
   const uint32_t eqf_base = (uint32_t)(uintptr_t)(fused_lds_cu32 *)s_eqf;
   const uint32_t eqr_base = (uint32_t)(uintptr_t)(fused_lds_cu32 *)s_eqr;
   const Counters *c = a.cnt;
   const uint32_t nhl = c->seg_nhitlines;
   const int match_opt = OPT >= 0 ? OPT : (a.options & 3);
   if (MODE == SQ_MODE_EMIT && (c->overflow & 4u)) return;
   const uint32_t m = (uint32_t)a.m, tau1 = (uint32_t)a.tau + 1;
   const bool count_any = a.want != SEEQDEV_WANT_COUNTMATCH && !(a.want == SEEQDEV_WANT_RECORDS && match_opt == SQ_ALL);
   const bool by_nh = a.use_nh != 0;
   const bool trusted = a.use_nh == 3 && !a.filter && !c->dirty;
   const bool caching = MODE == SQ_MODE_COUNT && cache != nullptr && a.want == SEEQDEV_WANT_RECORDS;
   const bool count_best = caching && match_opt == SQ_BEST;
   const bool cache_ok = MODE == SQ_MODE_EMIT && cache != nullptr && by_nh && !(trusted && count_any);
   const uint32_t ovf_r = (a.cap_hitlines > nhl ? a.cap_hitlines - nhl : 0u) / (gridDim.x * 4u);
   const uint32_t wave_id = threadIdx.x >> 6;
   uint4 *ovf = cache ? cache + nhl + (size_t)(blockIdx.x * 4u + wave_id) * ovf_r : nullptr;
   const bool ovf_lost = MODE == SQ_MODE_EMIT && c->seg_novf != 0;
   const bool walk = WALK && a.use_nh == 3 && hit_col != nullptr && a.stream_ch != 0;
   const uint32_t wback = a.skip_back > 32u ? a.skip_back : 32u;
   const bool noskip = (a.options & (SQ_IGNORE | SQ_STREAM)) == 0;
   uint8_t *row = s_blk + threadIdx.x * EXACT1_ROW;
   const uint32_t stride = gridDim.x * 256;
   const uint32_t kmax = (nhl + stride - 1) / stride * stride;
   for (uint32_t k = blockIdx.x * 256 + threadIdx.x; k < kmax; k += stride) {
      bool done = k >= nhl;
      const uint32_t kk = (a.hit_idx && !done) ? a.hit_idx[k] : k;
      const uint32_t hs = done ? 0u : a.hit_start[kk];
      if (hs == 0xFFFFFFFFu) done = true;
      const uint64_t off = done ? a.seg_base : a.seg_base + hs;
      if (MODE == SQ_MODE_COUNT && trusted && count_any) {
         if (k < nhl) a.nh[k] = done ? 0u : 1u;
         continue;
      }
      if (a.use_nh == 3 && (a.options & SEEQDEV_FASTA) && !done && a.text[off] == '>') done = true;
      fused_state_t<W> st;
      st.init(m);
      uint32_t streak = tau1, nhits = 0, best_d = tau1, best_end = 0, pos = 0;
      bool win = false;
      uint32_t wend = 0, knext = k + 1;
      uint32_t stop_at = 0xFFFFFFFFu;
      int32_t lastsub = -0x40000000;
      if (hit_col && (trusted || walk || a.filter) && !done) {
         const uint32_t col = hit_col[kk];
         bool ig_whole = false;
         if (a.ig_ent) {
            ig_whole = (a.ig_ent[kk].w & 6u) == 2u;
            for (uint32_t j = k + 1; !ig_whole && j < nhl && a.hit_start[j] == 0xFFFFFFFFu && a.hit_line[j] == a.hit_line[kk]; j++) ig_whole = (a.ig_ent[j].w & 6u) == 2u;
         }
         if (col > a.skip_back && !ig_whole && (trusted || a.ig_ent || exact1_clean(a, off, off + col))) pos = col - a.skip_back;
         if (MODE == SQ_MODE_COUNT && a.window_ok && !ig_whole) {
            uint32_t lastcol = a.hit_last ? a.hit_last[kk] : col, unbounded = 0u;
            if (a.hit_idx) {
               unbounded = lastcol == 0xFFFFFFFFu ? 2u : 0u;
               lastcol += a.skip_back - (m + tau1 - 1u);
            }
            else for (uint32_t j = k + 1; j < nhl && a.hit_start[j] == 0xFFFFFFFFu && (!a.ig_ent || a.hit_line[j] == a.hit_line[kk]); j++) lastcol = hit_col[j] - hs;
            if (!unbounded) stop_at = lastcol + m + tau1 + 1u;
         }
         const uint32_t lastnl = c->seg_last_nl;
         const bool last_seg = a.seg_base + a.pos_bias + a.seg_len >= a.nbytes;
         win = walk && (last_seg || (lastnl != 0 && (int64_t)hs - (int64_t)a.pos_bias < (int64_t)lastnl));
         wend = a.ll_restart ? col + m + tau1 + 1u : (((hs + col) | (a.stream_ch - 1u)) + 1u) - hs + a.walk_ext;
      }
      bool latch = false;
      seeqdev_hit_t *out = nullptr;
      uint32_t out_cap = 0, line_no = 0;
      uint32_t ce0 = 0, ce1 = 0, ncached = 0;
      uint32_t cstart = 0, chas = 0;
      bool from_cache = false;
      if (MODE == SQ_MODE_EMIT && !done) {
         line_no = a.hit_line[kk];
         if (match_opt == SQ_ALL) { out = a.records + c->records + nh_at(a, k); out_cap = 0xFFFFFFFFu; }
         else { out = a.records + c->records + (by_nh ? nh_at(a, k) : k); out_cap = 1; }
         if (cache_ok) {
            ncached = (k + 1 < nhl ? nh_at(a, k + 1) : c->seg_nrec) - nh_at(a, k);
            if (ncached <= 1 || !ovf_lost) {
               if (ncached) { const uint4 ce = cache[k]; ce0 = ce.x; ce1 = ce.y; cstart = ce.z; chas = ce.w; }
               from_cache = true;
               done = true;
            }
         }
      }
// ... 141 lines not shown
                  if (ccol > pos + wback && exact1_clean(a, off + pos, off + ccol - wback + land)) {
                     pos = ccol - wback; wend = cend;
                     st.init(m); streak = tau1; latch = false; lastsub = -0x40000000;
                     break;
                  }
                  if (cend > wend) wend = cend;
                  if (wend > pos) break;
               }
            }
         }
      }
      if (k < nhl) {
         if (MODE == SQ_MODE_COUNT) {
            if (count_best) { nhits = best_d < tau1 ? 1u : 0u; ce0 = best_end; ce1 = best_d; }
            a.nh[k] = nhits;
            uint32_t ce2 = 0, ce3 = 0;
            if (caching && count_any && nhits) { ce2 = exact1_reverse<W>(a.text, off, a.nbytes, ce0, ce1, eqr_base, m, tau1, row); ce3 = 1u; }
            if (caching) cache[k] = make_uint4(ce0, ce1, ce2, ce3);
         } else if (match_opt == SQ_BEST && !from_cache) {
            if (best_d < tau1) {
               seeqdev_hit_t h;
               h.line = line_no;
               h.start = exact1_reverse<W>(a.text, off, a.nbytes, best_end, best_d, eqr_base, m, tau1, row);
               h.end = best_end;
               h.dist = best_d;
               out[0] = h;
               a.rec_off[out - a.records] = rec_off_of(a, off, line_no);
            }
         } else {
            const uint32_t n = from_cache ? (ncached ? 1u : 0u) : (nhits < out_cap ? nhits : out_cap);
            for (uint32_t i = 0; i < n; i++) {
               seeqdev_hit_t h;
               h.line = line_no;
               if (from_cache) { h.end = ce0; h.dist = ce1; }
               else { h.end = out[i].end; h.dist = out[i].dist; }
               h.start = (from_cache && chas) ? cstart : exact1_reverse<W>(a.text, off, a.nbytes, h.end, h.dist, eqr_base, m, tau1, row);
               out[i] = h;
               a.rec_off[(out - a.records) + i] = rec_off_of(a, off, line_no);
            }
         }
      }
   }
   if (MODE == SQ_MODE_COUNT && caching && ovf_r && (threadIdx.x & 63u) == 0) {
      const uint32_t n = s_novf[wave_id];
      ovf[0] = make_uint4(n, 0u, 0u, 0u);
      if (n + 1u > ovf_r) a.cnt->seg_novf = 1u;
   }
   if (MODE == SQ_MODE_COUNT && caching && !ovf_r && (threadIdx.x & 63u) == 0 && s_novf[wave_id]) a.cnt->seg_novf = 1u;
   if (MODE == SQ_MODE_EMIT && cache_ok && !ovf_lost && ovf_r) {
      const uint32_t novf = ovf[0].x;
      for (uint32_t e = 1u + (threadIdx.x & 63u); e <= novf; e += 64u) {
         const uint4 o = ovf[e];
         const uint32_t ox = a.hit_idx ? a.hit_idx[o.x] : o.x;
         const uint64_t off = a.seg_base + a.hit_start[ox];
         const uint64_t slot = c->records + nh_at(a, o.x) + o.y;
         seeqdev_hit_t h;
         h.line = a.hit_line[ox];
         h.start = exact1_reverse<W>(a.text, off, a.nbytes, o.z, o.w, eqr_base, m, tau1, row);
         h.end = o.z;
         h.dist = o.w;
         a.records[slot] = h;
         a.rec_off[slot] = rec_off_of(a, off, h.line);
      }
   }
}

template <int MODE, int W, int OPT, bool WALK>
__global__ __launch_bounds__(256, 6) void k_exact1(ScanArgs a, const uint32_t *eq2, const uint32_t *hit_col, uint4 *cache)
{
   exact1_body<MODE, W, OPT, WALK>(a, eq2, hit_col, cache);
}

struct MultiExact {
   ScanArgs        a;
   const uint32_t *eq;
   const uint32_t *hcol;
   uint4          *cache;
   uint32_t       *scan_ws;
   uint32_t        nb;
   int             seg_end_flags;
};

template <int MODE, int W, int OPT>
__global__ __launch_bounds__(256, 6) void k_exact1m(const MultiExact *mx)
{
   const MultiExact &m = mx[blockIdx.y];
   exact1_body<MODE, W, OPT, false>(m.a, m.eq, m.hcol, m.cache);
}

#endif
```

### seeq_amd/csrc/seeq_order.h

```cpp
#ifndef SEEQ_ORDER_H_
#define SEEQ_ORDER_H_

#define ORDER_SCAN_ITEMS 8
#define ORDER_SCAN_BLOCK (256 * ORDER_SCAN_ITEMS)
#define ORDER_MAX_BLOCKS 1024

__global__ __launch_bounds__(256) void k_tiles_post(FusedArgs f, uint32_t nslices, uint32_t *bsum, uint32_t nb)
{
   if (blockIdx.y == 2) {
      if (blockIdx.x == 0) fused_post_body(f, nslices);
      return;
   }
   __shared__ uint32_t s_wave[4];
   uint32_t *arr = blockIdx.y == 0 ? f.tile_hits : f.tile_cl;
   const uint32_t n = f.ntiles, base = blockIdx.x * ORDER_SCAN_BLOCK;
   uint32_t item[ORDER_SCAN_ITEMS], v = 0;
#pragma unroll
   for (int k = 0; k < ORDER_SCAN_ITEMS; k++) {
      const uint32_t i = base + threadIdx.x * ORDER_SCAN_ITEMS + k;
      item[k] = i < n ? arr[i] : 0u;
      v += item[k];
   }
   uint32_t tot;
   uint32_t ex = block_excl_scan(v, &tot, s_wave);
#pragma unroll
   for (int k = 0; k < ORDER_SCAN_ITEMS; k++) {
      const uint32_t i = base + threadIdx.x * ORDER_SCAN_ITEMS + k;
      if (i < n) arr[i] = ex;
      ex += item[k];
   }
   if (threadIdx.x == 0) bsum[blockIdx.y * nb + blockIdx.x] = tot;
}

__device__ __forceinline__ void order_block_prefix(const uint32_t *bsum, uint32_t nb, uint32_t *s_ph, uint32_t *s_pc, uint32_t *s_wave)
{
   uint32_t run_h = 0, run_c = 0;
   for (uint32_t b0 = 0; b0 < nb; b0 += 256u) {
      const uint32_t i = b0 + threadIdx.x;
      const uint32_t vh = i < nb ? bsum[i] : 0u, vc = i < nb ? bsum[nb + i] : 0u;
      uint32_t th, tc;
      const uint32_t eh = block_excl_scan(vh, &th, s_wave), ec = block_excl_scan(vc, &tc, s_wave);
      if (i < nb) { s_ph[i] = run_h + eh; s_pc[i] = run_c + ec; }
      run_h += th; run_c += tc;
   }
   __syncthreads();
}

__global__ __launch_bounds__(256) void k_order(FusedArgs f, uint32_t nslices, const uint32_t *bsum, uint32_t nb, uint4 *ent)
{
   __shared__ uint32_t s_ph[ORDER_MAX_BLOCKS], s_pc[ORDER_MAX_BLOCKS], s_wave[4];
   order_block_prefix(bsum, nb, s_ph, s_pc, s_wave);
   const Counters *c = f.cnt;
   if (c->overflow & 2u) return;
   const uint32_t lane = threadIdx.x & 63;
   const uint32_t lines0 = (uint32_t)c->lines;
   for (uint32_t sl = blockIdx.x * 4 + (threadIdx.x >> 6); sl < nslices; sl += gridDim.x * 4) {
      const uint32_t n = f.wg_hits[sl];
      const uint4 *slice = f.tmp + (size_t)sl * f.slice_cap;
      for (uint32_t i0 = lane; i0 < n; i0 += 256) {
         uint4 e[4];
         uint32_t th[4], tc[4];
#pragma unroll
         for (int u = 0; u < 4; u++) e[u] = i0 + 64u * u < n ? slice[i0 + 64u * u] : make_uint4(0u, 0u, 0u, 0u);
#pragma unroll
         for (int u = 0; u < 4; u++) {
            const uint32_t tile = e[u].x & 0x1FFFFFFFu;
            const bool ok = i0 + 64u * u < n;
            th[u] = ok ? f.tile_hits[tile] + s_ph[tile / ORDER_SCAN_BLOCK] : 0u;
            tc[u] = ok ? f.tile_cl[tile] + s_pc[tile / ORDER_SCAN_BLOCK] : 0u;
         }
#pragma unroll
         for (int u = 0; u < 4; u++) {
            if (i0 + 64u * u >= n) continue;
            const uint32_t dst = th[u] + (e[u].y & 0x1FFFu);
            ent[dst] = make_uint4(e[u].z, lines0 + tc[u] + e[u].w + 1u , (e[u].x >> 31) | (((e[u].y >> 13) & 0x3FFFFu) << 1), (e[u].x >> 29) & 3u);
         }
      }
   }
}

__device__ __forceinline__ uint32_t order_last_nl16(const fused_v4u &v)
{
   const uint32_t g3 = nl_flags(v.w), g2 = nl_flags(v.z), g1 = nl_flags(v.y), g0 = nl_flags(v.x);
   if (g3) return 13u + ((31u - (uint32_t)__builtin_clz(g3)) >> 3);
   if (g2) return 9u + ((31u - (uint32_t)__builtin_clz(g2)) >> 3);
   if (g1) return 5u + ((31u - (uint32_t)__builtin_clz(g1)) >> 3);
   if (g0) return 1u + ((31u - (uint32_t)__builtin_clz(g0)) >> 3);
   return 0u;
}

__device__ __forceinline__ uint64_t order_line_start(const uint8_t *text, uint64_t hi)
{
   uint64_t q = hi;
   while (q >= 128) {
      fused_v4u v[8];
#pragma unroll
      for (int u = 0; u < 8; u++) v[u] = *reinterpret_cast<const fused_v4u_unaligned *>(text + q - 128 + 16 * u);
#pragma unroll
      for (int u = 7; u >= 0; u--) {
         const uint32_t r = order_last_nl16(v[u]);
         if (r) return q - 128 + 16 * u + r;
      }
      q -= 128;
   }
   while (q > 0) { if (text[q - 1] == '\n') return q; q--; }
   return 0;
}

__device__ __forceinline__ void order_marker_word(uint32_t w, uint32_t nby, uint32_t bm, uint32_t bv, uint32_t &ns, uint32_t &nb)
{
   const uint32_t keepm = nby >= 4u ? 0xFFFFFFFFu : (1u << (8u * nby)) - 1u;
   const uint32_t y = (w ^ __builtin_amdgcn_perm(0x474E5554u, 0x43FF41FFu, w & 0x07070707u)) & keepm;
   ns += (uint32_t)__popc((((y & 0x5F5F5F5Fu) + 0x7F7F7F7Fu) | y) & 0x80808080u);
   const uint32_t z = ((w & bm) ^ bv) | ~keepm;
   nb += (uint32_t)__popc(~(((z & 0x7F7F7F7Fu) + 0x7F7F7F7Fu) | z) & 0x80808080u);
}

__device__ __forceinline__ bool order_marker_holds(const ScanArgs &a, uint64_t q)
{
   const uint8_t *text = a.text;
   uint32_t ns = 0, nb = 0, len = 0;
   const uint32_t bm = a.ig_bmask * 0x01010101u, bv = a.ig_bval * 0x01010101u;
   uint64_t p = q;
   for (; p + 16 <= a.nbytes; p += 16) {
      const fused_v4u v = *reinterpret_cast<const fused_v4u_unaligned *>(text + p);
      const uint32_t f0 = nl_flags(v.x), f1 = nl_flags(v.y), f2 = nl_flags(v.z), f3 = nl_flags(v.w);
      if ((f0 | f1 | f2 | f3) == 0u) {
         order_marker_word(v.x, 4u, bm, bv, ns, nb); order_marker_word(v.y, 4u, bm, bv, ns, nb);
         order_marker_word(v.z, 4u, bm, bv, ns, nb); order_marker_word(v.w, 4u, bm, bv, ns, nb);
         len += 16u;
         if (len > (1u << 20)) return true;
         continue;
      }
      const uint32_t wf = f0 ? 0u : f1 ? 1u : f2 ? 2u : 3u;
      const uint32_t fw = f0 ? f0 : f1 ? f1 : f2 ? f2 : f3;
      const uint32_t nby = (uint32_t)__builtin_ctz(fw) >> 3;
      order_marker_word(v.x, wf > 0u ? 4u : nby, bm, bv, ns, nb);
      if (wf >= 1u) order_marker_word(v.y, wf > 1u ? 4u : nby, bm, bv, ns, nb);
      if (wf >= 2u) order_marker_word(v.z, wf > 2u ? 4u : nby, bm, bv, ns, nb);
      if (wf >= 3u) order_marker_word(v.w, nby, bm, bv, ns, nb);
      len += 4u * wf + nby;
      return ns != 0u && len - ns >= a.ig_thr && nb >= a.ig_need;
   }
   for (; p < a.nbytes && text[p] != '\n'; p++) {
      const uint32_t ch = text[p], up = ch & 0xDFu;
      if (!(up == 'A' || up == 'C' || up == 'G' || up == 'T' || up == 'U' || up == 'N')) ns++;
      if (((ch & a.ig_bmask) ^ a.ig_bval) == 0u) nb++;
      len++;
   }
   return ns != 0u && len - ns >= a.ig_thr && nb >= a.ig_need;
}

__global__ __launch_bounds__(256) void k_bounds2(ScanArgs a, uint4 *ent, uint32_t *hit_col)
{
   Counters *c = a.cnt;
   const uint32_t nhl = c->seg_nhitlines;
   const uint32_t stride = gridDim.x * 256;
   const uint64_t segb = a.seg_base + a.pos_bias;
   const uint32_t prev0 = c->prev_hit_line;
   for (uint32_t k = blockIdx.x * 256 + threadIdx.x; k < nhl; k += stride) {
      const uint4 e = ent[k];
      const uint32_t prev = k ? ent[k - 1].y : prev0;
      const uint32_t unresolved = e.z & 1u, col = e.z >> 1;
      a.hit_line[k] = e.y;
      uint32_t repeat = e.y == prev ? 1u : 0u;
      if (repeat && k != 0u && a.ig_thr != 0u) {
         const uint4 pe = ent[k - 1];
         const uint32_t pprev = k > 1u ? ent[k - 2].y : prev0;
         if ((pe.w & 3u) == 2u && pprev != pe.y) {
            const uint64_t pq = (pe.z & 1u) ? order_line_start(a.text, a.seg_base + pe.x) : a.seg_base + pe.x;
            const uint32_t pholds = (pq < a.seg_base || order_marker_holds(a, pq)) ? 1u : 0u;
            if (!pholds) repeat = 0u;
         }
      }
      if (repeat) {
         hit_col[k] = unresolved ? e.x : e.x + col;
         if (a.window_ok && e.y == prev0) {
            bool voids = true;
            if (a.ig_thr && (e.w & 2u) && unresolved) {
               const uint64_t hp0 = a.seg_base + e.x;
               voids = hp0 < a.nbytes && order_marker_holds(a, order_line_start(a.text, hp0));
            }
            if (voids) atomicOr(&c->overflow, 128u);
         }
         a.hit_start[k] = 0xFFFFFFFFu;
         continue;
      }
      if (!unresolved) {
         uint32_t keep = 1u;
         if (a.ig_need != 0u && (e.w & 2u) != 0u) {
            const uint32_t holds = order_marker_holds(a, a.seg_base + e.x) ? 1u : 0u;
            if (!holds) { keep = e.w & 1u; ent[k].w = e.w | 4u; }
         }
         a.hit_start[k] = keep ? e.x : 0xFFFFFFFFu; hit_col[k] = keep ? col : 0u;
         continue;
      }
      const uint64_t hp = a.seg_base + e.x;
      if (hp >= a.nbytes || hp < segb || hp >= segb + a.seg_len) {
         atomicOr(&c->overflow, 64u);
         a.hit_start[k] = 0xFFFFFFFFu;
         hit_col[k] = 0u;
         continue;
      }
      const uint64_t q = order_line_start(a.text, hp);
      uint32_t keep = 1u, holds = 1u;
      if (a.ig_thr != 0u && (e.w & 2u) != 0u && q >= a.seg_base) holds = order_marker_holds(a, q) ? 1u : 0u;
      if (!holds) {
         keep = e.w & 1u;
         ent[k].w = e.w | 4u;
      }
      uint32_t out_start, out_col;
      if (q < a.seg_base) { atomicOr(&c->overflow, 8u); out_start = 0xFFFFFFFFu; out_col = 0u; }
      else if (!keep) { out_start = 0xFFFFFFFFu; out_col = 0u; }
      else { out_start = (uint32_t)(q - a.seg_base); out_col = (uint32_t)(hp - q); }
      a.hit_start[k] = out_start;
      hit_col[k] = out_col;
   }
}

#endif
```

### seeq_amd/csrc/seeq_plan.h

```cpp
#ifndef SEEQ_PLAN_H_
#define SEEQ_PLAN_H_

#include <stdint.h>
#include <stdio.h>
#include <string.h>

struct ScanKnobs {
   int  kernel;
   int  tile_bytes;
   bool no_filter;
   int  min_wu;
   bool no_window;
   bool no_myers;
   bool no_leaders;
   bool no_packed_quad;
   bool no_sub;
   bool explain;
};

struct PlanAutomata {
   int    sdfa_state, sdfa_parts, sdfa_warm;
   double sdfa_pacc;
   int    pair_state, pair_warm;
   double pair_pacc;
// ... 74 lines not shown
            const double ll_pacc_max = p.fw == 1 ? 0.00058 : 0.0010;
            if (long_lines ? (au.sdfa_pacc > ll_pacc_max || in.wlen + in.tau + 2 > 64) : au.sdfa_pacc * in.avg_line > 0.25) p.use_stream = false;
         }
      }
   }
   {
      const bool long_lines = (in.avg_line > 600.0 && kn.kernel != 3) || in.force_ll;
      const bool pair_ll = long_lines && (nd == 0 || nd == PLAN_SQ_CONVERT) && !fasta && !in.multi_active && kn.kernel != 1 && !kn.no_window;
      const bool ig_ok = nd == PLAN_SQ_IGNORE && !fasta && !in.multi_active;
      if (p.fusable && in.force_path != 1 && (options & PLAN_MASK_INPUT) == 0 && (nd == 0 || nd == PLAN_SQ_CONVERT || ig_ok) && (!long_lines || pair_ll) && !in.no_stream &&
          (kn.kernel == 3 || (kn.kernel == 0 && !(in.sample_dirty && in.line_hint <= 0 && fasta))) && in.seg_bytes % (64u * 128u) == 0) {
         if (au.pair_state == 0) ensure(ctx, 1, 0, &au);
         p.use_pair = au.pair_state == 1 && (kn.kernel == 3 || in.multi_active || (long_lines ? au.pair_pacc > 0.0 && au.pair_pacc <= (p.fw == 1 ? 0.00058 : 0.0010) && in.wlen + in.tau + 2 <= 64
                                                                                                   : au.pair_pacc * in.avg_line <= 0.25));
         p.pair_ll = p.use_pair && long_lines;
      }
      if (p.use_pair) { p.use_stream = true; p.can_sub = false; p.ig = nd == PLAN_SQ_IGNORE; }
      if (in.multi_active && !p.use_pair) { p.rc = -2; return p; }
   }
   if (!p.use_stream && !p.use_pair && p.fusable && in.force_path != 1 && (options & PLAN_MASK_INPUT) == 0 && (nd == 0 || nd == PLAN_SQ_CONVERT) &&
       kn.kernel != 2 && !kn.no_myers && !in.no_stream && (in.avg_line > 260.0 || in.force_ll) && in.seg_bytes % (64u * 128u) == 0) {
      p.use_myers = true; p.use_stream = true; p.can_sub = false;
   }
   p.filter = p.use_pair || (p.use_stream && !p.use_myers && au.sdfa_parts > 1);
   p.use_fused = p.fusable && (in.avg_line <= 260.0 || p.use_stream) && in.force_path != 1;
   p.stream_wu = !p.use_stream ? 8 : au.sdfa_warm <= 16 ? 4 : au.sdfa_warm <= 24 ? 6 : 8;
   if (p.use_pair) p.stream_wu = au.pair_warm <= 16 ? 4 : (au.pair_warm + 3) / 4;
   if (p.stream_wu < kn.min_wu) p.stream_wu = kn.min_wu >= 8 ? 8 : 6;
   if (p.use_myers) p.stream_wu = in.wlen + in.tau - 1 <= 64 ? 16 : 32;
   if (p.use_fused && p.use_stream) {
      p.stream_ll = in.avg_line > 600.0 || in.force_ll;
      p.stream_sub = p.can_sub ? (nd == PLAN_SQ_IGNORE ? 2 : 1) : 0;
      if (p.use_myers) { p.stream_ll = true; p.stream_sub = 0; }
      if (p.use_pair) { p.stream_ll = p.pair_ll; p.stream_sub = 0; }
   }
   p.use_direct = p.use_fused && !p.use_stream;
   p.path = p.use_fused ? (p.use_pair ? 6 : p.use_myers ? 7 : p.use_stream ? 5 : 3) : 1;
   p.superset = p.use_stream;
   if (p.superset) p.need_nh = true;
   p.skip_back = (uint32_t)(in.wlen + in.tau - 1) + (p.use_pair ? 1u : 0u);
   p.window_ok = p.use_pair && !p.pair_ll && !in.no_window && !kn.no_window;
   p.ll_filter = p.use_fused && p.use_stream && p.stream_ll && p.filter && !p.use_pair && !p.use_myers;
   p.ll_restart = (p.ll_filter && !kn.no_window && au.sdfa_pacc > 0.00005) || p.pair_ll;
   p.walk_ext = p.ll_filter ? (uint32_t)(in.wlen + in.tau + 2) : 0u;
   p.skip_thr = (p.use_fused && p.use_stream && !p.use_pair && !p.use_myers && p.stream_sub == 2 && au.sdfa_parts == 1) ? (uint32_t)(in.wlen - in.tau) : 0u;
   p.lead_best = want == PLAN_WANT_RECORDS && match_opt == PLAN_SQ_BEST;
   p.leaders = p.use_stream && p.stream_ll && (p.nh_is_count || p.lead_best) && p.use_fused && !kn.no_leaders && !in.no_leaders && !in.multi_active;
   p.order2 = p.use_fused && p.use_stream && !p.stream_ll;
   p.verify = p.need_nh && p.use_fused && p.filter && !p.stream_ll && !in.multi_active &&
              (options & (PLAN_SQ_IGNORE | PLAN_SQ_STREAM)) == 0;
   return p;
}

static inline void seeq_plan_print(FILE *f, const PlanIn &in, const PlanAutomata &au, const ScanPlan &p)
{
   static const char *const kname[8] = {"?", "generic (k_nl_* + k_forward)", "?", "k_direct", "?", "k_stream", "k_pair", "k_stream, Myers mode"};
   fprintf(f, "seeq plan: m=%d tau=%d options=0x%x want=%d avg_line=%.1f%s -> %s%s%s%s%s | column words %d, warm-up %d B, sub %d | "
              "automata: stream %s (parts %d, warm %d, p_acc %.2g), pair %s (warm %d, p_acc %.2g) | "
              "post-pass: %s, %s%s%s, skip_back %u%s\n",
           in.wlen, in.tau, (unsigned)in.options, in.want, in.avg_line, in.line_hint > 0 ? " (hint)" : "",
           kname[p.path & 7], p.filter ? " [candidates: filter / prefix]" : "", p.pair_ll ? " [long lines: LL variant, windows of the restart walk]" : p.stream_ll ? " [long lines]" : "", p.ll_restart ? " [filter on long lines, restart table]" : p.ll_filter ? " [filter on long lines]" : "",
           p.rc == -2 ? " [multi: not k_pair's -- a scan per pattern]" : "",
           p.fw, 4 * p.stream_wu, p.stream_sub,
           au.sdfa_state == 1 ? "yes" : au.sdfa_state == 0 ? "not asked" : "none", au.sdfa_parts, au.sdfa_warm, au.sdfa_pacc,
           au.pair_state == 1 ? "yes" : au.pair_state == 0 ? "not asked" : "none", au.pair_warm, au.pair_pacc,
           p.order2 ? "k_tiles_post + k_order + k_bounds2" : p.use_fused ? "k_fused_post + k_scanset_* + reorder + bounds" : "k_compact",
           p.verify ? "k_verify + k_nh_top" : p.need_nh ? "k_exact1<COUNT> + scan" : "no count pass",
           p.window_ok ? " on candidate windows" : "", p.leaders ? " [leaders]" : "", p.skip_back, p.skip_thr ? ", skip count" : "");
}

#endif
```

### seeq_amd/csrc/seeq_post.h

```cpp
#ifndef SEEQ_POST_H_
#define SEEQ_POST_H_

#include <hip/hip_runtime.h>
#include "seeq_types.h"
#include "seeq_scan_common.h"

#define VERIFY_ANY  0
#define VERIFY_BEST 1
#define VERIFY_ALL  2

void seeq_launch_verify(int fw, int var, unsigned grid, hipStream_t st, const ScanArgs &a, const uint32_t *eq, const uint32_t *hit_col,
                        uint4 *cache);
struct VerifyPacked;
void seeq_launch_verify_packed(int fw, int var, unsigned grid, hipStream_t st, const ScanArgs &a, const void *bases, const void *nmask, uint32_t stride,
                               uint32_t nstride, uint32_t read_len, uint64_t total_bytes, uint64_t ntotal_bytes, const uint32_t *eq, const uint32_t *hit_col, uint4 *cache);
void seeq_launch_emit1(unsigned grid, hipStream_t st, const ScanArgs &a, const uint4 *cache);
void seeq_launch_emit_all(int fw, unsigned grid, unsigned vgrid, hipStream_t st, const ScanArgs &a, const uint32_t *eq, const uint32_t *hit_col, uint4 *cache);

#define SEEQ_ORDER_MAX_BLOCKS 1024
#define SEEQ_ORDER_BLOCK      2048
void seeq_launch_tiles_post(hipStream_t st, const FusedArgs &f, uint32_t nslices, uint32_t *bsum, uint32_t nb);
void seeq_launch_order(unsigned grid, hipStream_t st, const FusedArgs &f, uint32_t nslices, const uint32_t *bsum, uint32_t nb, uint4 *ent);
void seeq_launch_bounds2(unsigned grid, hipStream_t st, const ScanArgs &a, uint4 *ent, uint32_t *hit_col);

#endif
```

### seeq_amd/csrc/seeq_scan_common.h

```cpp
#ifndef SEEQ_SCAN_COMMON_H_
#define SEEQ_SCAN_COMMON_H_

#include "libseeq.h"
#include "seeq_types.h"

#ifndef SEEQ_WG
#define SEEQ_WG 256
#endif

#define FUSED_FLAG_TERM 1u
#define FUSED_FLAG_SKIP 2u
#define FUSED_FLAGS     3u
#define FUSED_MAX_WLEN  30
#define FUSED_MAX_WLEN2 62

typedef unsigned int fused_v4u __attribute__((ext_vector_type(4)));
typedef fused_v4u fused_v4u_unaligned __attribute__((aligned(1)));

struct FusedArgs {
   const uint8_t *text;
   uint64_t       nbytes;
   uint64_t       seg_base;
   uint32_t       seg_len;
   uint32_t       first_seg;
   uint32_t       tile_bytes;
   uint32_t       pos_bias;
   uint32_t       ntiles;
   const uint32_t *eqtab;
   const uint32_t *peq;
   int            m, tau, options, want;
   uint32_t      *tile_cl;
   uint32_t      *tile_hits;
   uint4         *tmp;
   uint32_t       cap_tmp;
   uint32_t       slice_cap;
   uint32_t      *wg_hits;
   uint32_t      *wg_part;
   uint32_t      *tile_dirty;
   uint64_t      *tile_dmask;
   uint32_t      *wg_lastnl;
   const uint16_t *dfa;
   uint32_t       dfa_rows;
   uint32_t       dfa_final_base;
   unsigned long long *clk_probe;
   uint32_t       ll_filter;
   uint32_t       skip_thr;
   uint32_t       ig_thr;
   uint32_t       pair;
   Counters      *cnt;
};

__device__ __forceinline__ void fused_step(uint32_t eq, uint32_t &pv, uint32_t &mv, uint32_t &score)
{
   const uint32_t s = (eq & pv) + pv;
   const uint32_t d0 = ((s ^ pv) | eq) | mv;
   const uint32_t ph = mv | ~(d0 | pv);
   const uint32_t mh = pv & d0;
   uint32_t ph2, mh2;
   asm("v_add_co_u32 %0, vcc, %2, %2\n\tv_addc_co_u32 %1, vcc, 0, %1, vcc"
       : "=v"(ph2), "+v"(score) : "v"(ph) : "vcc");
   asm("v_add_co_u32 %0, vcc, %2, %2\n\tv_subbrev_co_u32 %1, vcc, 0, %1, vcc"
       : "=v"(mh2), "+v"(score) : "v"(mh) : "vcc");
   pv = mh2 | ~(d0 | ph2);
   mv = ph2 & d0;
}

__device__ __forceinline__ uint32_t fused_bad4(uint32_t w)
{
   const uint32_t idx = (w & 0x0E0E0E0Eu) >> 1;
   const uint32_t canon = __builtin_amdgcn_perm(0x4EFF0AFFu, 0x47544341u, idx);
   const uint32_t fold = __builtin_amdgcn_perm(0xDFFFFFFFu, 0xDFDEDFDFu, idx);
   return (w & fold) ^ canon;
}

__device__ __forceinline__ uint32_t wave_incl_scan_u32(uint32_t x)
{
   x += (uint32_t)__builtin_amdgcn_update_dpp(0, (int)x, 0x111, 0xf, 0xf, true);
   x += (uint32_t)__builtin_amdgcn_update_dpp(0, (int)x, 0x112, 0xf, 0xf, true);
   x += (uint32_t)__builtin_amdgcn_update_dpp(0, (int)x, 0x114, 0xf, 0xf, true);
   x += (uint32_t)__builtin_amdgcn_update_dpp(0, (int)x, 0x118, 0xf, 0xf, true);
   x += (uint32_t)__builtin_amdgcn_update_dpp(0, (int)x, 0x142, 0xa, 0xf, true);
   x += (uint32_t)__builtin_amdgcn_update_dpp(0, (int)x, 0x143, 0xc, 0xf, true);
   return x;
}

template <int W> struct fused_eq_t;
template <> struct fused_eq_t<1> { uint32_t w0; };
template <> struct fused_eq_t<2> { uint32_t w0, w1; };

typedef __attribute__((address_space(3))) const uint32_t fused_lds_cu32;
typedef __attribute__((address_space(3))) const uint64_t fused_lds_cu64;

template <int W>
__device__ __forceinline__ fused_eq_t<W> fused_eq_load(uint32_t lds_byte_addr);
template <>
__device__ __forceinline__ fused_eq_t<1> fused_eq_load<1>(uint32_t addr)
{
   fused_eq_t<1> e;
   e.w0 = *(fused_lds_cu32 *)(uintptr_t)addr;
   return e;
}
template <>
__device__ __forceinline__ fused_eq_t<2> fused_eq_load<2>(uint32_t addr)
{
// ... 45 lines not shown
   uint32_t base = 0, tot = 0;
#pragma unroll
   for (int w = 0; w < SEEQ_WG / 64; w++) {
      uint32_t s = s_wave[w];
      if (w < wave) base += s;
      tot += s;
   }
   __syncthreads();
   *total = tot;
   return base + x - v;
}

__device__ __forceinline__ uint32_t nl_flags(uint32_t w)
{
   const uint32_t x = w ^ 0x0A0A0A0Au;
   const uint32_t t = ((x & 0x7F7F7F7Fu) + 0x7F7F7F7Fu) | x;
   return ~t & 0x80808080u;
}


__device__ __forceinline__ void rec_check_body(const ScanArgs &a)
{
   Counters *c = a.cnt;
   c->need_records = c->records + c->seg_nrec;
   if (c->records + c->seg_nrec > a.cap_records) atomicOr(&c->overflow, 4u);
}

__device__ __forceinline__ void seg_end_body(const ScanArgs &a, int flags )
{
   Counters *c = a.cnt;
   const uint32_t counted = c->seg_nlines - c->seg_nheaders;
   const uint32_t seg_hits = (flags & 1) ? c->seg_nrec : c->seg_nhitlines;
   if (flags & 2) c->seg_nmatch = c->seg_nrec;
   c->lines += counted;
   c->headers += c->seg_nheaders;
   c->matchlines += a.use_nh >= 2 ? c->seg_nmatch : c->seg_nhitlines;
   if (a.use_nh == 3 && c->seg_nhitlines) {
      const uint32_t nhl = c->seg_nhitlines, lastl = a.hit_line[nhl - 1];
      uint32_t covered = 1u;
      if (a.ig_thr != 0u) {
         covered = lastl == c->prev_hit_line ? 1u : 0u;
         for (uint32_t k = nhl; !covered && k-- > 0u && a.hit_line[k] == lastl; ) covered = a.hit_start[k] != 0xFFFFFFFFu ? 1u : 0u;
      }
      c->prev_hit_line = covered ? lastl : 0xFFFFFFFFu;
   }
   c->hits += seg_hits;
   if (a.want == SEEQDEV_WANT_RECORDS) c->records += seg_hits;
   c->seg_nlines = c->seg_nhitlines = c->seg_nheaders = c->seg_nrec = c->seg_nmatch = c->seg_novf = 0;
}

__device__ __forceinline__ void fused_post_body(const FusedArgs &a, uint32_t nslices)
{
   __shared__ uint32_t s_red[4][4];
   uint32_t lines = 0, hdrs = 0, hits = 0, mx = 0, ovf = 0, lastnl = 0, flags = 0, busy = 0, crowded = 0;
   const uint4 *part = reinterpret_cast<const uint4 *>(a.wg_part);
   for (uint32_t i0 = threadIdx.x; i0 < nslices; i0 += 2048) {
      uint4 pv[8];
      uint32_t lv[8];
#pragma unroll
      for (int u = 0; u < 8; u++) {
         const uint32_t i = i0 + 256u * u;
         pv[u] = i < nslices ? part[i] : make_uint4(0u, 0u, 0u, 0u);
         lv[u] = a.wg_lastnl && i < nslices ? a.wg_lastnl[i] : 0u;
      }
#pragma unroll
      for (int u = 0; u < 8; u++) {
         lastnl = lv[u] > lastnl ? lv[u] : lastnl;
         lines += pv[u].x;
         hdrs += pv[u].y;
         const uint32_t h = pv[u].z;
         flags |= pv[u].w;
         busy += pv[u].x != 0;
         crowded += (pv[u].w >> 3) & 1u;
         hits += h & 0x7FFFFFFFu;
         mx = (h & 0x7FFFFFFFu) > mx ? (h & 0x7FFFFFFFu) : mx;
         ovf |= h >> 31;
      }
   }
#pragma unroll
   for (int d = 32; d >= 1; d >>= 1) {
      lines += __shfl_xor(lines, d, 64);
      hdrs += __shfl_xor(hdrs, d, 64);
      hits += __shfl_xor(hits, d, 64);
      const uint32_t o = __shfl_xor(mx, d, 64);
      mx = o > mx ? o : mx;
      ovf |= __shfl_xor(ovf, d, 64);
      flags |= __shfl_xor(flags, d, 64);
      busy += __shfl_xor(busy, d, 64);
      crowded += __shfl_xor(crowded, d, 64);
      const uint32_t ol = __shfl_xor(lastnl, d, 64);
      lastnl = ol > lastnl ? ol : lastnl;
   }
   __shared__ uint32_t s_last[4], s_flags[4], s_busy[4], s_crowded[4];
   const int w = threadIdx.x >> 6;
   if ((threadIdx.x & 63) == 0) { s_last[w] = lastnl; s_flags[w] = flags; s_busy[w] = busy; s_crowded[w] = crowded; }
   if ((threadIdx.x & 63) == 0) { s_red[w][0] = lines; s_red[w][1] = hdrs; s_red[w][2] = hits; s_red[w][3] = mx | (ovf << 31); }
   __syncthreads();
   if (threadIdx.x == 0) {
      lines = hdrs = hits = mx = ovf = 0;
      for (int k = 0; k < 4; k++) {
         lines += s_red[k][0]; hdrs += s_red[k][1]; hits += s_red[k][2];
         const uint32_t m = s_red[k][3] & 0x7FFFFFFFu;
         mx = m > mx ? m : mx;
         ovf |= s_red[k][3] >> 31;
      }
      Counters *c = a.cnt;
      flags = s_flags[0] | s_flags[1] | s_flags[2] | s_flags[3];
      if (flags & 1u) {
         c->dirty |= 1u;
         if ((a.options & MASK_NONDNA) && !a.pair) c->overflow |= 16u;
      }
      if (flags & 4u) {
         c->dirty |= 1u;
         busy = s_busy[0] + s_busy[1] + s_busy[2] + s_busy[3];
         crowded = s_crowded[0] + s_crowded[1] + s_crowded[2] + s_crowded[3];
         if ((a.options & MASK_NONDNA) == SQ_IGNORE && crowded * 2 > busy) c->overflow |= 16u;
      }
      if (flags & 2u) c->overflow |= 32u;
      c->seg_nlines = lines;
      c->seg_nheaders = hdrs;
      const uint64_t need = (uint64_t)mx * nslices + (uint64_t)nslices * 64;
      if (need > c->need_hitlines) c->need_hitlines = need > 0xFFFFFFFFull ? 0xFFFFFFFFu : (uint32_t)need;
      if (ovf) { atomicOr(&c->overflow, 2u); hits = 0; }
      if (c->overflow & 2u) hits = 0;
      c->seg_nhitlines = hits;
      c->seg_nrec = hits;
      if (hits > c->need_hitlines) c->need_hitlines = hits;
      c->seg_novf = 0;
      lastnl = 0;
      for (int k = 0; k < 4; k++) lastnl = s_last[k] > lastnl ? s_last[k] : lastnl;
      c->seg_last_nl = lastnl;
   }
}


#endif
```

### seeq_amd/csrc/seeq_types.h

```cpp
#ifndef SEEQ_TYPES_H_
#define SEEQ_TYPES_H_

#include <stdint.h>
#include "seeq_amd.h"

struct Counters {
   uint32_t seg_nlines;
   uint32_t seg_nhitlines;
   uint32_t seg_nheaders;
   uint32_t seg_nrec;
   uint64_t lines;
   uint64_t matchlines;
   uint64_t hits;
   uint64_t records;
   uint64_t headers;
   uint32_t overflow;
   uint32_t need_lines;
   uint32_t need_hitlines;
   uint32_t seg_novf;
   uint32_t seg_nmatch;
   uint32_t dirty;
   uint64_t need_records;
   uint32_t prev_hit_line;
   uint32_t seg_last_nl;
   uint32_t seg_dirty_tiles;
   uint32_t emit_nhl;
   uint32_t pad4[2];
   uint64_t emit_base;
};

struct ScanArgs {
   const uint8_t *text;
   uint64_t       nbytes;
   uint64_t       seg_base;
   uint32_t       seg_len;
   uint32_t       first_seg;
   const uint32_t *peq;
   int            m, tau, options, want;
   uint32_t      *line_start;   uint32_t cap_lines;
   uint32_t      *tile_cnt;     uint32_t ntiles;
   uint64_t      *hitmask;
   uint64_t      *hdrmask;
   uint32_t      *wave_off;
   uint32_t      *hdr_off;
   uint32_t      *hit_start;
   uint32_t      *hit_line;
   uint32_t       cap_hitlines;
   uint32_t      *nh;
   seeqdev_hit_t *records;      uint64_t cap_records;
   uint64_t      *rec_off;
   uint32_t       use_nh;
   uint32_t       pos_bias;
   const uint32_t *tile_dirty;
   const uint64_t *tile_dmask;
   uint32_t       stream_ntiles, stream_tile_bytes;
   uint32_t       stream_ch;
   uint32_t       filter;
   uint32_t       skip_back;
   const uint32_t *hit_last;
   uint32_t       *walk_end;
   const uint32_t *hit_idx;
   uint32_t       window_ok;
   uint32_t       *nh_sum;
   uint32_t        walk_ext;
   uint32_t        ll_restart;
   uint32_t        rec_pitch;
   uint32_t       *nz_sum;
   uint32_t        fin;
   uint32_t        ig_thr;
   uint32_t        ig_need, ig_bval, ig_bmask;
   const uint4    *ig_ent;
   uint32_t        vrange;
   Counters      *cnt;
};

#if defined(__HIPCC__)
__device__ __forceinline__ uint32_t nh_at(const ScanArgs &a, uint32_t k) { return a.nh[k] + (a.nh_sum ? a.nh_sum[k >> 8] : 0u); }
__device__ __forceinline__ uint64_t rec_off_of(const ScanArgs &a, uint64_t off, uint32_t line) { return a.rec_pitch ? (uint64_t)(line - 1u) * a.rec_pitch : off; }
#endif


#endif
```

### seeq_amd/csrc/seeq_verify.h

```cpp
#ifndef SEEQ_VERIFY_H_
#define SEEQ_VERIFY_H_

#include "seeq_post.h"

__device__ __forceinline__ uint32_t verify_top(uint32_t x, uint32_t n) { return (uint32_t)((((uint64_t)x) << 32) >> n); }

#define VERIFY_ADDR(dst, word, SEL) \
   asm("v_lshlrev_b32_sdwa %0, %1, %2 dst_sel:DWORD dst_unused:UNUSED_PAD src0_sel:DWORD src1_sel:BYTE_" #SEL : "=v"(dst) : "v"(sh), "v"(word))

#define VERIFY_BARE 0
#define VERIFY_REV  1
#define VERIFY_FWD  2
template <int W> struct verify_col;
template <> struct verify_col<1> {
   template <int MODE>
   static __device__ __forceinline__ void run(const fused_eq_t<1> &e, fused_state_t<1> &st, uint32_t lim, uint32_t &L, uint32_t &PH, uint32_t &MH, uint32_t &T)
   {
      const uint32_t eq = e.w0, pv = st.pv, mv = st.mv;
      if (MODE == VERIFY_FWD) T = __builtin_amdgcn_alignbit(eq, T, 1);
      const uint32_t s = (eq & pv) + pv;
      const uint32_t d0 = ((s ^ pv) | eq) | mv;
      const uint32_t ph = mv | ~(d0 | pv);
      const uint32_t mh = pv & d0;
      if (MODE == VERIFY_FWD) { PH = __builtin_amdgcn_alignbit(PH, ph, 31); MH = __builtin_amdgcn_alignbit(MH, mh, 31); }
// ... 172 lines not shown
   __shared__ __align__(8) uint32_t s_eqf[256 * W];
   __shared__ __align__(8) uint32_t s_eqr[256 * W];
   __shared__ uint32_t s_novf[4], s_wave[4];
   if (threadIdx.x < 4) s_novf[threadIdx.x] = 0;
   for (int i = threadIdx.x; i < 256 * W; i += 256) { s_eqf[i] = eq2[i]; s_eqr[i] = eq2[256 * W + i]; }
   __syncthreads();
   const uint32_t eqf_base = (uint32_t)(uintptr_t)(fused_lds_cu32 *)s_eqf;
   const uint32_t eqr_base = (uint32_t)(uintptr_t)(fused_lds_cu32 *)s_eqr;
   Counters *c = a.cnt;
   const uint32_t nhl = c->seg_nhitlines;
   const uint32_t m = (uint32_t)a.m, tau = (uint32_t)a.tau, tau1 = tau + 1u;
   const bool caching = cache != nullptr && a.want == SEEQDEV_WANT_RECORDS;
   const bool dirty = c->dirty != 0;
   uint32_t sh = W == 1 ? 2u : 3u;
   asm volatile("" : "+v"(sh));
   const uint32_t ovf_r = (a.cap_hitlines > nhl ? a.cap_hitlines - nhl : 0u) / (gridDim.x * 4u);
   const uint32_t wave_id = threadIdx.x >> 6;
   uint4 *const ovf_all = cache ? cache + nhl : nullptr;
   __shared__ uint16_t s_idx[1024];
   __shared__ uint32_t s_cnt[1024];
   const bool compact = a.vrange != 0u;
   const uint32_t range = (a.vrange == 512u || a.vrange == 1024u) && nhl >= 65536u ? a.vrange : 256u;
   const uint32_t nranges = (nhl + range - 1u) / range;
#define VERIFY_NR        ((nranges == 0u || nranges > gridDim.x) ? gridDim.x : nranges)
#define VERIFY_MY_LISTS  (blockIdx.x < VERIFY_NR ? (gridDim.x - blockIdx.x + VERIFY_NR - 1u) / VERIFY_NR : 0u)
#define VERIFY_LIST_ROOM (ovf_r > 1u ? ovf_r - 1u : 0u)
   for (uint32_t rg = blockIdx.x; rg < nranges; rg += gridDim.x) {
    const uint32_t r0 = rg * range;
    uint32_t nact = 0;
    if (!compact) {
       s_cnt[threadIdx.x] = 0u;
       nact = nhl - r0 < 256u ? nhl - r0 : 256u;
    }
    else for (uint32_t u = 0; u < range; u += 256u) {
       const uint32_t k = r0 + u + threadIdx.x;
       const bool live = k < nhl;
       const uint32_t kk = (a.hit_idx && live) ? a.hit_idx[k] : k;
       const bool act = live && a.hit_start[kk] != 0xFFFFFFFFu;
       s_cnt[u + threadIdx.x] = 0u;
       uint32_t tot;
       const uint32_t ex = block_excl_scan(act ? 1u : 0u, &tot, s_wave);
       if (act) s_idx[nact + ex] = (uint16_t)(u + threadIdx.x);
       if (live && !act && caching) cache[k] = make_uint4(0u, 0u, 0u, 0u);
       nact += tot;
    }
    __syncthreads();
    for (uint32_t j0 = 0; j0 < nact; j0 += 256u) {
      bool done = j0 + threadIdx.x >= nact;
      const uint32_t k = r0 + (done ? 0u : compact ? (uint32_t)s_idx[j0 + threadIdx.x] : threadIdx.x);
#define VERIFY_MINE (j0 + threadIdx.x < nact)
      const uint32_t kk = (a.hit_idx && !done) ? a.hit_idx[k] : k;
      const uint32_t hs = done ? 0u : a.hit_start[kk];
      if (hs == 0xFFFFFFFFu) done = true;
      const uint64_t off = done ? a.seg_base : a.seg_base + hs;
      if (a.use_nh == 3 && (a.options & SEEQDEV_FASTA) && !done && a.text[off] == '>') done = true;
      uint32_t pos = 0, stop_at = 0xFFFFFFFFu;
      if (!done) {
         const uint32_t col = hit_col[kk];
         if (col > a.skip_back) pos = col - a.skip_back;
         if (a.window_ok) {
            uint32_t lastcol = a.hit_last ? a.hit_last[kk] : col;
            bool unbounded = false;
            if (a.hit_idx) { unbounded = lastcol == 0xFFFFFFFFu; lastcol += a.skip_back - (m + tau1 - 1u); }
            else for (uint32_t j = k + 1; j < nhl && a.hit_start[j] == 0xFFFFFFFFu; j++) lastcol = hit_col[j] - hs;
            if (!unbounded) stop_at = lastcol + m + tau1 + 1u;
         }
      }
      if (dirty && verify_prefix_dirty(a, off, pos)) pos = 0;
      fused_state_t<W> st;
      st.init(m);
      verify_rules<VAR> r;
      r.prevL = 0; r.latch = 0; r.nhits = 0; r.best_d = tau1; r.best_end = 0; r.ce0 = 0; r.ce1 = 0; r.done = false;
      auto second = [&](uint32_t p, uint32_t streak) {
         if (VAR == VERIFY_ALL && caching) {
            const uint32_t idx = atomicAdd(&s_novf[wave_id], 1u);
            const uint32_t list_room = VERIFY_LIST_ROOM;
            if (idx < VERIFY_MY_LISTS * list_room) {
               const uint32_t t = idx / list_room;
               ovf_all[(size_t)((blockIdx.x + t * VERIFY_NR) * 4u + wave_id) * ovf_r + 1u + (idx - t * list_room)] = make_uint4(k, r.nhits, p, streak);
            }
         }
      };
      while (__any(!done)) {
         fused_v4u v[4];
         {
            const uint64_t p0 = off + pos;
            if (p0 + 64 <= a.nbytes) {
#pragma unroll
               for (int q = 0; q < 4; q++) v[q] = *reinterpret_cast<const fused_v4u_unaligned *>(a.text + p0 + 16 * q);
            } else {
#pragma unroll
               for (int q = 0; q < 4; q++) v[q] = direct_load16(a.text, p0 + 16 * q, a.nbytes);
            }
         }
         const uint32_t stop_rel = done ? 0u : stop_at - pos;
         const uint32_t s_in = st.score;
         uint32_t Lh = 0, Ll = 0, Ph = 0, Pl = 0, Mh = 0, Ml = 0, Th = 0, Tl = 0;
         uint32_t ncols = 64;
#pragma unroll
         for (int g = 0; g < 16; g++) {
            if (!__any(stop_rel > 4u * g)) { ncols = 4u * g; break; }
            verify_word<W, VERIFY_FWD>(verify_word_of(v, g), eqf_base, sh, st, tau, g < 8 ? Lh : Ll, g < 8 ? Ph : Pl, g < 8 ? Mh : Ml, g < 8 ? Th : Tl);
         }
         const uint32_t nh_ = ncols < 32u ? ncols : 32u, nl_ = ncols > 32u ? ncols - 32u : 0u;
         Lh = verify_top(~Lh, nh_); Ph = verify_top(Ph, nh_); Mh = verify_top(Mh, nh_); Th = verify_top(__builtin_bitreverse32(Th), nh_);
         Ll = verify_top(~Ll, nl_); Pl = verify_top(Pl, nl_); Ml = verify_top(Ml, nl_); Tl = verify_top(__builtin_bitreverse32(Tl), nl_);
         uint32_t tcol = Th ? (uint32_t)__builtin_clz(Th) : Tl ? 32u + (uint32_t)__builtin_clz(Tl) : 64u;
// ... 19 lines not shown
         const bool need = VERIFY_MINE && nhits != 0u;
         if (__any(need)) {
            const uint32_t s0 = verify_reverse<W>(a, need, off, ce0, ce1, eqr_base, sh, m, tau1);
            if (need) { ce2 = s0; ce3 = 1u; }
         }
      }
      if (caching && VERIFY_MINE) cache[k] = make_uint4(ce0, ce1, ce2, ce3);
      if (VERIFY_MINE) s_cnt[k - r0] = nhits;
#undef VERIFY_MINE
    }
    __syncthreads();
    for (uint32_t u = 0; u < range && r0 + u < nhl; u += 256u) {
      const uint32_t k0 = r0 + u, k = k0 + threadIdx.x;
      const uint32_t nhits = s_cnt[u + threadIdx.x];
      uint32_t tot;
      const uint32_t ex = block_excl_scan(nhits, &tot, s_wave);
      if (k < nhl) a.nh[k] = ex;
      if (threadIdx.x == 0) a.nh_sum[k0 >> 8] = tot;
      if (a.nz_sum) {
         const uint32_t nzw = (uint32_t)__popcll(__ballot(nhits != 0u));
         if ((threadIdx.x & 63u) == 0) s_wave[wave_id] = nzw;
         __syncthreads();
         if (threadIdx.x == 0) a.nz_sum[k0 >> 8] = s_wave[0] + s_wave[1] + s_wave[2] + s_wave[3];
         __syncthreads();
      }
    }
    __syncthreads();
   }
   if (caching && (threadIdx.x & 63u) == 0) {
      const uint32_t n = s_novf[wave_id];
      if (ovf_r) {
         const uint32_t my_lists = VERIFY_MY_LISTS, list_room = VERIFY_LIST_ROOM, nr = VERIFY_NR;
         for (uint32_t t = 0; t < my_lists; t++) {
            const uint32_t before = t * list_room;
            const uint32_t cnt = n > before ? (n - before < list_room ? n - before : list_room) : 0u;
            ovf_all[(size_t)((blockIdx.x + t * nr) * 4u + wave_id) * ovf_r] = make_uint4(cnt, 0u, 0u, 0u);
         }
         if (n > my_lists * list_room) c->seg_novf = 1u;
      }
      else if (n) c->seg_novf = 1u;
#undef VERIFY_NR
#undef VERIFY_MY_LISTS
#undef VERIFY_LIST_ROOM
   }
}

__global__ __launch_bounds__(256) void k_nh_top(ScanArgs a)
{
   __shared__ uint32_t s_wave[4];
   Counters *c = a.cnt;
   const uint32_t nhl = c->seg_nhitlines;
   const uint32_t nch = (nhl + 255u) >> 8;
   uint32_t running = 0, nz = 0;
   for (uint32_t b0 = 0; b0 < nch; b0 += 2048u) {
      uint32_t item[8], v = 0;
#pragma unroll
      for (int q = 0; q < 8; q++) {
         const uint32_t i = b0 + threadIdx.x * 8u + q;
         item[q] = i < nch ? a.nh_sum[i] : 0u;
         if (a.nz_sum && i < nch) nz += a.nz_sum[i];
      }
#pragma unroll
      for (int q = 0; q < 8; q++) v += item[q];
      uint32_t tot;
      uint32_t ex = running + block_excl_scan(v, &tot, s_wave);
#pragma unroll
      for (int q = 0; q < 8; q++) {
         const uint32_t i = b0 + threadIdx.x * 8u + q;
         if (i < nch) a.nh_sum[i] = ex;
         ex += item[q];
      }
      running += tot;
   }
   if (a.nz_sum) {
      uint32_t tot;
      block_excl_scan(nz, &tot, s_wave);
      nz = tot;
   }
   if (threadIdx.x == 0) {
      c->seg_nrec = running;
      if (a.nz_sum) c->seg_nmatch = nz;
      if (a.want == SEEQDEV_WANT_RECORDS) rec_check_body(a);
      c->emit_nhl = nhl;
      c->emit_base = c->records;
      if (a.fin) seg_end_body(a, (int)a.fin - 1);
   }
}

__global__ __launch_bounds__(256) void k_emit1(ScanArgs a, const uint4 *cache)
{
   const Counters *c = a.cnt;
   if (c->overflow & 4u) return;
   const uint32_t nhl = c->emit_nhl;
   const uint64_t base = c->emit_base;
   for (uint32_t k = blockIdx.x * 256u + threadIdx.x; k < nhl; k += gridDim.x * 256u) {
      const uint4 ce = cache[k];
      if (!ce.w) continue;
      const uint32_t kk = a.hit_idx ? a.hit_idx[k] : k;
      const uint64_t slot = base + nh_at(a, k);
      seeqdev_hit_t h;
      h.line = a.hit_line[kk];
      h.start = ce.z;
      h.end = ce.x;
      h.dist = ce.y;
      a.records[slot] = h;
      a.rec_off[slot] = rec_off_of(a, a.seg_base + a.hit_start[kk], h.line);
   }
}

template <int W>
__global__ __launch_bounds__(256, W == 1 ? 6 : 5) void k_emit_all(ScanArgs a, const uint32_t *eq2, const uint32_t *hit_col, uint4 *cache, uint32_t vgrid)
{
   const Counters *c = a.cnt;
   if (c->overflow & 4u) return;
   if (c->seg_novf) { exact1_body<SQ_MODE_EMIT, W, -1, false>(a, eq2, hit_col, cache); return; }
   __shared__ __align__(8) uint32_t s_eqr[256 * W];
   for (int i = threadIdx.x; i < 256 * W; i += 256) s_eqr[i] = eq2[256 * W + i];
   __syncthreads();
   const uint32_t eqr_base = (uint32_t)(uintptr_t)(fused_lds_cu32 *)s_eqr;
   const uint32_t nhl = c->seg_nhitlines;
   const uint64_t base = c->records;
   const uint32_t m = (uint32_t)a.m, tau1 = (uint32_t)a.tau + 1u;
   uint32_t sh = W == 1 ? 2u : 3u;
   asm volatile("" : "+v"(sh));
   for (uint32_t k = blockIdx.x * 256u + threadIdx.x; k < nhl; k += gridDim.x * 256u) {
      const uint4 ce = cache[k];
      if (!ce.w) continue;
      const uint32_t kk = a.hit_idx ? a.hit_idx[k] : k;
      const uint64_t slot = base + nh_at(a, k);
      seeqdev_hit_t h;
      h.line = a.hit_line[kk];
      h.start = ce.z;
      h.end = ce.x;
      h.dist = ce.y;
      a.records[slot] = h;
      a.rec_off[slot] = rec_off_of(a, a.seg_base + a.hit_start[kk], h.line);
   }
   const uint32_t nlists = vgrid * 4u;
   const uint32_t ovf_r = (a.cap_hitlines > nhl ? a.cap_hitlines - nhl : 0u) / nlists;
   if (!ovf_r) return;
   const uint32_t lane = threadIdx.x & 63u;
   for (uint32_t l = blockIdx.x * 4u + (threadIdx.x >> 6); l < nlists; l += gridDim.x * 4u) {
      const uint4 *ovf = cache + nhl + (size_t)l * ovf_r;
      const uint32_t novf = (uint32_t)__builtin_amdgcn_readfirstlane((int)ovf[0].x);
      for (uint32_t e0 = 1u; e0 <= novf; e0 += 64u) {
         const bool need = e0 + lane <= novf;
         const uint4 o = need ? ovf[e0 + lane] : make_uint4(0u, 0u, 0u, 0u);
         const uint32_t ox = (need && a.hit_idx) ? a.hit_idx[o.x] : o.x;
         const uint32_t hs = need ? a.hit_start[ox] : 0u;
         const uint64_t off = a.seg_base + hs;
         const uint32_t s0 = verify_reverse<W>(a, need, off, o.z, o.w, eqr_base, sh, m, tau1);
         if (need) {
            const uint64_t slot = base + nh_at(a, o.x) + o.y;
            seeqdev_hit_t h;
            h.line = a.hit_line[ox];
            h.start = s0;
            h.end = o.z;
            h.dist = o.w;
            a.records[slot] = h;
            a.rec_off[slot] = rec_off_of(a, off, h.line);
         }
      }
   }
}

template <int W, int VAR, int OCC>
__global__ __launch_bounds__(256, OCC) void k_verify(ScanArgs a, const uint32_t *eq2, const uint32_t *hit_col, uint4 *cache)
{
   verify_body<W, VAR>(a, eq2, hit_col, cache);
}

#undef VERIFY_ADDR

#endif
```

### seeq_amd/csrc/seeq_verify.hip

```cpp
#include <hip/hip_runtime.h>

#include <stdint.h>

#include "seeq_amd.h"
#include "seeq_kernel_core.h"
#include "seeq_types.h"
#include "seeq_scan_common.h"
#include "seeq_direct.h"
#include "seeq_exact1.h"
#include "seeq_verify.h"
#include "seeq_verify_packed.h"
#include "seeq_order.h"
#include "seeq_post.h"

void seeq_launch_verify(int fw, int var, unsigned grid, hipStream_t st, const ScanArgs &a, const uint32_t *eq, const uint32_t *hit_col,
                        uint4 *cache)
{
#define SEEQ_VERIFY(WW, VV) hipLaunchKernelGGL((k_verify<WW, VV, (WW == 1 ? 6 : 5)>), dim3(grid), dim3(256), 0, st, a, eq, hit_col, cache)
   if (fw == 1) {
      if (var == VERIFY_BEST) SEEQ_VERIFY(1, VERIFY_BEST); else if (var == VERIFY_ALL) SEEQ_VERIFY(1, VERIFY_ALL); else SEEQ_VERIFY(1, VERIFY_ANY);
   } else {
      if (var == VERIFY_BEST) SEEQ_VERIFY(2, VERIFY_BEST); else if (var == VERIFY_ALL) SEEQ_VERIFY(2, VERIFY_ALL); else SEEQ_VERIFY(2, VERIFY_ANY);
   }
#undef SEEQ_VERIFY
   hipLaunchKernelGGL(k_nh_top, dim3(1), dim3(256), 0, st, a);
}

void seeq_launch_emit1(unsigned grid, hipStream_t st, const ScanArgs &a, const uint4 *cache)
{
   hipLaunchKernelGGL(k_emit1, dim3(grid), dim3(256), 0, st, a, cache);
}

void seeq_launch_emit_all(int fw, unsigned grid, unsigned vgrid, hipStream_t st, const ScanArgs &a, const uint32_t *eq, const uint32_t *hit_col, uint4 *cache)
{
   if (fw == 1) hipLaunchKernelGGL(k_emit_all<1>, dim3(grid), dim3(256), 0, st, a, eq, hit_col, cache, vgrid);
   else hipLaunchKernelGGL(k_emit_all<2>, dim3(grid), dim3(256), 0, st, a, eq, hit_col, cache, vgrid);
}

static_assert(ORDER_MAX_BLOCKS == SEEQ_ORDER_MAX_BLOCKS && ORDER_SCAN_BLOCK == SEEQ_ORDER_BLOCK, "seeq_order.h / seeq_post.h");

void seeq_launch_tiles_post(hipStream_t st, const FusedArgs &f, uint32_t nslices, uint32_t *bsum, uint32_t nb)
{
   hipLaunchKernelGGL(k_tiles_post, dim3(nb ? nb : 1, 3), dim3(256), 0, st, f, nslices, bsum, nb);
}

void seeq_launch_order(unsigned grid, hipStream_t st, const FusedArgs &f, uint32_t nslices, const uint32_t *bsum, uint32_t nb, uint4 *ent)
{
   hipLaunchKernelGGL(k_order, dim3(grid), dim3(256), 0, st, f, nslices, bsum, nb, ent);
}

void seeq_launch_bounds2(unsigned grid, hipStream_t st, const ScanArgs &a, uint4 *ent, uint32_t *hit_col)
{
   hipLaunchKernelGGL(k_bounds2, dim3(grid), dim3(256), 0, st, a, ent, hit_col);
}

void seeq_launch_verify_packed(int fw, int var, unsigned grid, hipStream_t st, const ScanArgs &a, const void *bases, const void *nmask, uint32_t stride,
                               uint32_t nstride, uint32_t read_len, uint64_t total_bytes, uint64_t ntotal_bytes, const uint32_t *eq, const uint32_t *hit_col, uint4 *cache)
{
   VerifyPacked pk;
   pk.bases = (const uint8_t *)bases; pk.nmask = (const uint8_t *)nmask; pk.stride = stride; pk.nstride = nstride; pk.read_len = read_len;
   pk.total_bytes = total_bytes; pk.ntotal_bytes = ntotal_bytes;
#define SEEQ_VERIFYP(WW, VV) hipLaunchKernelGGL((k_verify_packed<WW, VV>), dim3(grid), dim3(256), 0, st, a, pk, eq, hit_col, cache)
   if (fw == 1) {
      if (var == VERIFY_BEST) SEEQ_VERIFYP(1, VERIFY_BEST); else if (var == VERIFY_ALL) SEEQ_VERIFYP(1, VERIFY_ALL); else SEEQ_VERIFYP(1, VERIFY_ANY);
   } else {
      if (var == VERIFY_BEST) SEEQ_VERIFYP(2, VERIFY_BEST); else if (var == VERIFY_ALL) SEEQ_VERIFYP(2, VERIFY_ALL); else SEEQ_VERIFYP(2, VERIFY_ANY);
   }
#undef SEEQ_VERIFYP
   hipLaunchKernelGGL(k_nh_top, dim3(1), dim3(256), 0, st, a);
}
```

### seeq_amd/device.py

```python
import ctypes as C

import numpy as np

from . import _capi
from ._capi import (SQ_ALL, SQ_BEST, SQ_CONVERT, SQ_FAIL, SQ_FIRST, SQ_IGNORE, SEEQDEV_FASTA,
                    WANT_COUNTLINES, WANT_COUNTMATCH, WANT_RECORDS)


class SeeqDeviceError(RuntimeError):
    pass


def _check(rc):
    if rc != 0:
        raise SeeqDeviceError(_capi.error_text())


def pack_reads(text, read_len, with_nmask=True):
    stride, nstride = (read_len + 3) // 4, (read_len + 7) // 8
    nmax = len(text) // read_len + 1
    bases = np.zeros(nmax * stride, dtype=np.uint8)
    nmask = np.zeros(nmax * nstride, dtype=np.uint8) if with_nmask else None
    n = _capi.lib().seeqdevPackReads(text, len(text), read_len, bases.ctypes.data, nmask.ctypes.data if with_nmask else None, stride, nstride)
    if n < 0:
# ... 77 lines not shown
            self._lib.seeqFree(sq)

    def __del__(self):
        try:
            self.close()
        except Exception:
            pass


class Scanner:
    def __init__(self, stream=None):
        self._lib = _capi.lib()
        self._h = self._lib.seeqdevScanNew(C.c_void_p(stream) if stream else None)
        if not self._h:
            raise SeeqDeviceError("seeqdevScanNew: " + _capi.error_text())

    def close(self):
        h, self._h = self._h, None
        if h:
            self._lib.seeqdevScanFree(h)

    def __del__(self):
        try:
            self.close()
        except Exception:
            pass

    def reserve(self, max_bytes=0, max_lines=0, max_hitlines=0, max_records=0):
        _check(self._lib.seeqdevScanReserve(self._h, max_bytes, max_lines, max_hitlines, max_records))

    def set_profiling(self, on=True):
        _check(self._lib.seeqdevScanSetProfiling(self._h, 1 if on else 0))

    def set_line_hint(self, avg_bytes_per_line):
        _check(self._lib.seeqdevScanSetLineHint(self._h, float(avg_bytes_per_line)))

    def last_path(self):
        return {1: "generic", 3: "fused", 5: "fused", 6: "fused", 7: "fused", 8: "packed"}.get(self._lib.seeqdevScanLastPath(self._h), "none")

    def last_kernel(self):
        return {1: "k_forward", 3: "k_direct", 5: "k_stream", 6: "k_pair", 7: "k_myers", 8: "k_packed"}.get(self._lib.seeqdevScanLastPath(self._h), "none")

    def last_filter(self):
        return bool(self._lib.seeqdevScanLastFilter(self._h))

    def last_packed_quad(self):
        return bool(self._lib.seeqdevScanLastPackedQuad(self._h))

    def last_times_ms(self):
        ms = (C.c_float * 4)()
        _check(self._lib.seeqdevScanLastTimes(self._h, ms))
        return dict(index=ms[0], forward=ms[1], exact=ms[2], total=ms[3],
                    forward_launches=self._lib.seeqdevScanLastLaunches(self._h))

    def last_clock_mhz(self):
        return float(self._lib.seeqdevScanLastClockMHz(self._h))

    def last_launch_times_ms(self):
        n = self._lib.seeqdevScanLastLaunches(self._h)
        ms = (C.c_float * max(1, n))()
        got = self._lib.seeqdevScanLastLaunchTimes(self._h, ms, n)
        return [float(ms[i]) for i in range(max(0, min(got, n)))]

    def run(self, pattern, d_ptr, nbytes, options=0, want=WANT_COUNTLINES):
        _check(self._lib.seeqdevScanRun(self._h, pattern.handle, C.c_void_p(d_ptr), nbytes, options, want))

    def fetch(self):
        cnt = _capi.seeqdev_counts_t()
        _check(self._lib.seeqdevScanFetch(self._h, C.byref(cnt)))
        return dict(nlines=cnt.nlines, nmatchlines=cnt.nmatchlines, nhits=cnt.nhits, nrecords=cnt.nrecords,
                    nheaders=cnt.nheaders)

    def records(self, n=None, first=0):
        if n is None:
            raise ValueError("n required")
        out = np.zeros((n, 4), dtype=np.uint32)
        if n:
            _check(self._lib.seeqdevScanCopyRecords(self._h, out.ctypes.data, first, n))
        return out

    def record_offsets(self, n, first=0):
        out = np.zeros(n, dtype=np.uint64)
        if n:
            _check(self._lib.seeqdevScanCopyOffsets(self._h, out.ctypes.data, first, n))
        return out

    def records_device_ptr(self):
        return self._lib.seeqdevScanRecordsDevice(self._h)

    def scan_tensor(self, pattern, t, options=0, want=WANT_COUNTLINES):
        self.run(pattern, t.data_ptr(), t.numel(), options, want)
        return self.fetch()

    def run_packed(self, pattern, bases_ptr, nmask_ptr, nreads, read_len, stride=None, nstride=None, options=0, want=WANT_COUNTLINES):
        b = _capi.seeqdev_packed_t(bases_ptr, nmask_ptr or None, nreads, read_len, stride or (read_len + 3) // 4,
                                   nstride or (read_len + 7) // 8)
        _check(self._lib.seeqdevScanPacked(self._h, pattern.handle, C.byref(b), options, want))

    def scan_host(self, pattern, data, options=0, want=WANT_COUNTLINES):
        cnt = _capi.seeqdev_counts_t()
        _check(self._lib.seeqdevScanHost(self._h, pattern.handle, data, len(data), options, want, C.byref(cnt)))
        res = dict(nlines=cnt.nlines, nmatchlines=cnt.nmatchlines, nhits=cnt.nhits, nrecords=cnt.nrecords,
                   nheaders=cnt.nheaders)
        if want == WANT_RECORDS:
            res["records"] = self.records(cnt.nrecords)
        return res
# ... 62 lines not shown
```

Before: 26.71 billion.

## Batch multiple segments into one ordering and verify pass

Segments in the fused scan path are now grouped so that several segments run their scan kernels back-to-back. The per-segment ordering, bounds and verify launches are deferred and issued once for the whole batch. Per-segment entry offsets (bt_ent) let post kernels binary-search each hit's segment to recover its base offset. The intent is to cut per-segment launch and synchronisation overhead. In exchange it adds binary searches in the verify kernels, larger workspace slices, and an overflow fallback flag (512) that disables batching when 32-bit line or record counts would overflow.

```diff
diff --git a/include/seeq_amd.h b/include/seeq_amd.h
--- a/include/seeq_amd.h
+++ b/include/seeq_amd.h
@@ -115,6 +115,7 @@
 int seeqdevScanSetProfiling(seeqdev_scan_t * scan, int on);
 int seeqdevScanLastTimes(const seeqdev_scan_t * scan, float ms[4]);
 int seeqdevScanLastLaunches(const seeqdev_scan_t * scan);
+int seeqdevScanLastBatches(const seeqdev_scan_t * scan);
 int seeqdevScanLastLaunchTimes(const seeqdev_scan_t * scan, float * ms, int cap);
 float seeqdevScanLastClockMHz(const seeqdev_scan_t * scan);
 
diff --git a/seeq_amd/_capi.py b/seeq_amd/_capi.py
--- a/seeq_amd/_capi.py
+++ b/seeq_amd/_capi.py
@@ -56,7 +56,7 @@
     "seeqdevDeviceCount", "seeqdevSetDevice", "seeqdevLastError", "seeqdevPatternNew", "seeqdevPatternFree",
     "seeqdevPatternOf", "seeqdevScanNew", "seeqdevScanFree", "seeqdevScanReserve", "seeqdevScanRun",
     "seeqdevScanFetch", "seeqdevScanRecordsDevice", "seeqdevScanCopyRecords", "seeqdevScanHost",
-    "seeqdevScanSetProfiling", "seeqdevScanLastTimes", "seeqdevScanLastLaunches", "seeqdevScanLastLaunchTimes", "seeqdevScanLastClockMHz", "seeqdevSynthReads",
+    "seeqdevScanSetProfiling", "seeqdevScanLastTimes", "seeqdevScanLastLaunches", "seeqdevScanLastBatches", "seeqdevScanLastLaunchTimes", "seeqdevScanLastClockMHz", "seeqdevSynthReads",
     "seeqdevScanSetLineHint", "seeqdevScanLastPath", "seeqdevScanLastFilter", "seeqdevScanLastPackedQuad", "seeqdevScanCopyOffsets", "seeqdevHostAlloc", "seeqdevTextAlloc", "seeqdevTextAllocInfo", "seeqdevTextAllocFor", "seeqdevTextFree",
     "seeqdevHostFree", "seeqdevStringMatch", "seeqdevScanHostBegin", "seeqdevScanLastCopyMs", "seeqdevPatternDevice",
     "seeqdevScanRunMulti", "seeqdevScanHostMulti", "seeqdevScanMultiRecords", "seeqdevScanLastMulti", "seeqdevScanPacked", "seeqdevPackReads", "seeqdevPackReadsDevice",
@@ -155,6 +155,8 @@
     L.seeqdevScanLastTimes.restype = C.c_int
     L.seeqdevScanLastLaunches.argtypes = [C.c_void_p]
     L.seeqdevScanLastLaunches.restype = C.c_int
+    L.seeqdevScanLastBatches.argtypes = [C.c_void_p]
+    L.seeqdevScanLastBatches.restype = C.c_int
     L.seeqdevScanLastLaunchTimes.argtypes = [C.c_void_p, P(C.c_float), C.c_int]
     L.seeqdevScanLastLaunchTimes.restype = C.c_int
     L.seeqdevScanLastClockMHz.argtypes = [C.c_void_p]
diff --git a/seeq_amd/csrc/seeq_device.hip b/seeq_amd/csrc/seeq_device.hip
--- a/seeq_amd/csrc/seeq_device.hip
+++ b/seeq_amd/csrc/seeq_device.hip
@@ -817,6 +817,9 @@
    bool force_ll;
    bool no_stream_nd;
    bool no_leaders;
+   bool no_batch;
+   int last_batches;
+   uint32_t *d_bt_ent;
    bool no_window;
    int  fallback_ttl;
    bool sample_dirty;
@@ -909,7 +912,8 @@
    multi_plan_free(s->mplan);
    void *bufs[] = {s->rec_off, s->line_start, s->tile_cnt, s->hitmask, s->hdrmask, s->wave_off, s->hdr_off, s->hit_start,
                    s->hit_line, s->d_eqtab,
-                   s->nh, s->hit_col, s->nh_sum, s->ent, s->records, s->scan_ws, s->lead_fidx, s->lead_flag, s->lead_wend, s->lead_key, s->d_cnt, s->d_text};
+                   s->nh, s->hit_col, s->nh_sum, s->ent, s->records, s->scan_ws, s->lead_fidx, s->lead_flag, s->lead_wend, s->lead_key, s->d_cnt, s->d_text,
+                   s->d_bt_ent};
    for (void *b : bufs) if (b) (void)hipFree(b);
    if (s->h_cnt) (void)hipHostFree(s->h_cnt);
    if (s->h_eqtab) (void)hipHostFree(s->h_eqtab);
@@ -937,8 +941,8 @@
          if (ws_alloc((void **)&s->tile_cnt, tiles * sizeof(uint32_t))) return -1;
          s->cap_tiles = tiles;
       }
-      const size_t ftiles = seg / FUSED_MIN_TILE + 2;
-      const size_t slices = MAX_FUSED_GRID;
+      const size_t ftiles = seg / FUSED_MIN_TILE + 2 + SEEQ_BATCH_MAX_SEGS;
+      const size_t slices = MAX_FUSED_GRID * SEEQ_BATCH_MAX_SEGS;
       if (ftiles > s->cap_ftiles) {
          if (ws_alloc((void **)&s->ow.tile_cl, ftiles * sizeof(uint32_t))) return -1;
          if (ws_alloc((void **)&s->ow.tile_dirty, ftiles * sizeof(uint32_t))) return -1;
@@ -984,6 +988,7 @@
    if (s->cap_ftiles > largest) largest = s->cap_ftiles;
    size_t nb = largest / SCAN_BLOCK + 2;
    if (3 * (s->cap_ftiles / SCAN_BLOCK + 2) > nb) nb = 3 * (s->cap_ftiles / SCAN_BLOCK + 2);
+   if (nb < 2 * (size_t)SEEQ_ORDER_MAX_BLOCKS) nb = 2 * (size_t)SEEQ_ORDER_MAX_BLOCKS;
    if (nb > s->cap_scan_ws) {
       if (ws_alloc((void **)&s->scan_ws, nb * sizeof(uint32_t))) return -1;
       s->cap_scan_ws = nb;
@@ -1318,7 +1323,8 @@
    return 0;
 }
 
-static int seg_onepass(seeqdev_scan *s, const SegRun &r, ScanArgs &a, size_t sg, hipEvent_t *ev, bool &order2, uint32_t &stream_ntiles)
+static int seg_onepass(seeqdev_scan *s, const SegRun &r, ScanArgs &a, size_t sg, hipEvent_t *ev, bool &order2, uint32_t &stream_ntiles, size_t bj, size_t bn,
+                       bool &deferred)
 {
    const seeqdev_pattern *pat = r.pat;
    const int options = r.options, want = r.want, match_opt = r.options & 3, fw = r.fw, ncu = s->ncu;
@@ -1346,8 +1352,12 @@
    stream_ntiles = f.ntiles;
    f.eqtab = s->d_eqtab; f.peq = pat->d_peq;
    f.m = pat->wlen; f.tau = pat->tau; f.options = options; f.want = want;
-   f.tile_cl = ow.tile_cl; f.tile_hits = ow.tile_hits; f.tmp = ow.tmp; f.cap_tmp = (uint32_t)s->cap_hitlines;
-   f.wg_hits = ow.wg_hits; f.wg_part = ow.wg_part; f.wg_lastnl = stream_ll ? ow.wg_lastnl : nullptr;
+   const uint32_t tps = (uint32_t)((r.seg_bytes + tile_bytes - 1) / tile_bytes);
+   f.tile_cl = ow.tile_cl + bj * tps; f.tile_hits = ow.tile_hits + bj * tps; f.cap_tmp = (uint32_t)s->cap_hitlines;
+   f.slice_cap = f.cap_tmp / (uint32_t)(nslices * bn);
+   f.tmp = ow.tmp + bj * nslices * (size_t)f.slice_cap;
+   f.wg_hits = ow.wg_hits + bj * nslices; f.wg_part = ow.wg_part + 4 * bj * nslices;
+   f.wg_lastnl = stream_ll ? ow.wg_lastnl : nullptr;
    f.tile_dirty = f.wg_lastnl ? ow.tile_dirty : nullptr;
    f.tile_dmask = f.wg_lastnl ? ow.tile_dmask : nullptr;
    f.cnt = c;
@@ -1359,15 +1369,12 @@
       f.skip_thr = plan.skip_thr;
       if (use_pair) { f.dfa = pat->d_pair; f.dfa_rows = pat->pair_units; f.dfa_final_base = 0; f.pair = 1; f.ig_thr = plan.ig ? (uint32_t)(pat->wlen - pat->tau) : 0u; }
       if (use_myers) { f.dfa = (const uint16_t *)(s->d_eqtab + (size_t)512 * fw); f.dfa_rows = (uint32_t)(64 * fw); f.dfa_final_base = 0; f.pair = 2; }
-      uint64_t room = 0xFFFFFFF0ull - a.seg_len;
-      if (room > ((uint64_t)1 << 30)) room = (uint64_t)1 << 30;
-      pos_bias = (uint32_t)(a.seg_base < room ? a.seg_base : room) & ~127u;
+      pos_bias = seeq_pos_bias(a.seg_base, a.seg_len);
       f.pos_bias = pos_bias;
    }
    if (ev) { HIP_TRY(hipEventRecord(ev[0], st), EIO); HIP_TRY(hipEventRecord(ev[1], st), EIO); }
    unsigned fgrid = fused_grid;
    const unsigned nsl = nslices;
-   f.slice_cap = f.cap_tmp / nsl;
    if (use_stream) {
       void *kargs[] = {&f};
       HIP_TRY(hipLaunchKernel(stream_fn, dim3(fgrid), dim3(64 * (unsigned)nw), kargs, dfa_lds, st), EIO);
@@ -1375,10 +1382,21 @@
    else if (use_direct && fw == 2) hipLaunchKernelGGL((k_direct<4, 2>), dim3(fgrid), dim3(256), 0, st, f);
    else hipLaunchKernelGGL((k_direct<4, 1>), dim3(fgrid), dim3(256), 0, st, f);
    if (ev) HIP_TRY(hipEventRecord(ev[2], st), EIO);
-   const uint32_t order_nb = (f.ntiles + SEEQ_ORDER_BLOCK - 1) / SEEQ_ORDER_BLOCK;
-   order2 = plan.order2 && order_nb <= SEEQ_ORDER_MAX_BLOCKS && 2 * (size_t)order_nb <= s->cap_scan_ws;
+   if (bj + 1 < bn) {
+      deferred = true;
+      if (ev) HIP_TRY(hipEventRecord(ev[3], st), EIO);
+      return 0;
+   }
+   FusedArgs fb = f;
+   fb.tile_cl = ow.tile_cl; fb.tile_hits = ow.tile_hits; fb.tmp = ow.tmp; fb.wg_hits = ow.wg_hits; fb.wg_part = ow.wg_part;
+   fb.ntiles = (uint32_t)(bj * tps) + f.ntiles;
+   const uint32_t bsl = (uint32_t)(nsl * bn);
+   const uint32_t order_nb = (fb.ntiles + SEEQ_ORDER_BLOCK - 1) / SEEQ_ORDER_BLOCK;
+   order2 = plan.order2;
+   if (order2 && (order_nb > SEEQ_ORDER_MAX_BLOCKS || 2 * (size_t)order_nb > s->cap_scan_ws)) {
+      snprintf(g_last_error, sizeof g_last_error, "internal: %u tiles exceed one ordering", fb.ntiles); seeqerr = 0; errno = EIO; return -1;
+   }
    if (plan.ig) {
-      if (!order2) { snprintf(g_last_error, sizeof g_last_error, "SQ_IGNORE on k_pair needs the three-launch ordering (segment too large for its block sums)"); seeqerr = 0; errno = EIO; return -1; }
       a.ig_thr = f.ig_thr; a.ig_ent = (const uint4 *)s->ent;
       {
          static const char base_of_key[9] = {0, 'A', 'C', 0, 'G', 0, 0, 0, 'T'};
@@ -1392,9 +1410,11 @@
       }
    }
    if (order2) {
-      const unsigned rgrid = nsl / 4 + 1 < 2048 ? nsl / 4 + 1 : 2048;
-      seeq_launch_tiles_post(st, f, (uint32_t)nsl, s->scan_ws, order_nb);
-      seeq_launch_order(rgrid, st, f, (uint32_t)nsl, (const uint32_t *)s->scan_ws, order_nb, s->ent);
+      const unsigned rgrid = bsl / 4 + 1 < 2048 ? bsl / 4 + 1 : 2048;
+      OrderBatch ob;
+      ob.seg_slices = nsl; ob.tps = tps; ob.nseg = (uint32_t)bn; ob.bt_ent = bn > 1 ? s->d_bt_ent : nullptr;
+      seeq_launch_tiles_post(st, fb, bsl, s->scan_ws, order_nb);
+      seeq_launch_order(rgrid, st, fb, bsl, (const uint32_t *)s->scan_ws, order_nb, s->ent, ob);
    }
    else hipLaunchKernelGGL(k_fused_post, dim3(1), dim3(256), 0, st, f, (uint32_t)nsl);
    if (!order2 && (want != SEEQDEV_WANT_COUNTLINES || superset)) {
@@ -1405,6 +1425,15 @@
    }
    a.seg_base -= pos_bias;
    a.pos_bias = pos_bias;
+   if (bn > 1) {
+      const size_t g0 = sg - bj;
+      uint32_t len0 = 0;
+      a.seg_base = seeq_seg_vbase(g0, r.seg_bytes, nbytes, &len0);
+      a.pos_bias = seeq_pos_bias((uint64_t)g0 * r.seg_bytes, len0);
+      a.seg_len = len0;
+      a.first_seg = g0 == 0;
+      a.bt_n = (uint32_t)bn; a.bt_seg0 = (uint32_t)g0; a.bt_seg_bytes = r.seg_bytes; a.bt_ent = s->d_bt_ent;
+   }
    a.tile_dirty = f.tile_dirty; a.tile_dmask = f.tile_dmask; a.stream_ntiles = f.ntiles; a.stream_tile_bytes = tile_bytes;
    a.stream_ch = stream_ll ? (uint32_t)stream_ch : 0u;
    a.walk_ext = plan.walk_ext; a.ll_restart = plan.ll_restart ? 1u : 0u;
@@ -1577,7 +1606,12 @@
    const int options = r.options, want = r.want;
    const size_t nbytes = s->nbytes, seg_bytes = r.seg_bytes, nseg = r.nseg;
    const bool use_stream = plan.use_stream, use_fused = plan.use_fused, filter = plan.filter, superset = plan.superset, need_nh = plan.need_nh, nh_is_count = plan.nh_is_count;
+   const bool batching = use_fused && plan.order2 && !plan.ig && !s->multi_active && !s->no_batch;
+   if (batching && !s->d_bt_ent) HIP_TRY(hipMalloc((void **)&s->d_bt_ent, SEEQ_BATCH_MAX_SEGS * sizeof(uint32_t)), ENOMEM);
+   s->last_batches = 0;
+   size_t bn = 0, bj = 0;
    for (size_t sg = 0; sg < nseg; sg++) {
+      if (bj == bn) { bn = seeq_plan_batch(batching, nseg, sg, seg_bytes, r.tile_bytes); bj = 0; s->last_batches++; }
 
       hipEvent_t *ev = s->prof ? s->ev + 4 * sg : NULL;
       uint32_t stream_ntiles = 0;
@@ -1603,8 +1637,11 @@
       a.window_ok = plan.window_ok ? 1u : 0u;
       a.cnt = c;
 
-      if (use_fused) { if (seg_onepass(s, r, a, sg, ev, order2, stream_ntiles)) return -1; }
+      bool deferred = false;
+      if (use_fused) { if (seg_onepass(s, r, a, sg, ev, order2, stream_ntiles, bj, bn, deferred)) return -1; }
       else if (seg_index_forward<W>(s, r, a, ev)) return -1;
+      bj++;
+      if (deferred) { HIP_TRY(hipGetLastError(), EIO); continue; }
       if (want != SEEQDEV_WANT_COUNTLINES || superset) {
          const int pr = seg_post<W>(s, r, a, ev, order2, stream_ntiles);
          if (pr < 0) return pr;
@@ -1684,6 +1721,7 @@
       s->nev_seg = nseg;
    }
    if (s->prof) s->prof_segs = nseg;
+   s->last_batches = (int)nseg;
    for (size_t sg = 0; sg < nseg; sg++) {
       hipEvent_t *ev = s->prof ? s->ev + 4 * sg : NULL;
       PackedArgs p;
@@ -1928,7 +1966,8 @@
    s->pat = pat; s->text = d_text; s->nbytes = nbytes; s->options = options; s->want = want;
    s->ran = false;
    s->is_packed = false;
-   if ((s->no_stream || s->no_stream_nd || s->force_ll || s->no_window || s->no_leaders) && --s->fallback_ttl <= 0) s->no_stream = s->no_stream_nd = s->force_ll = s->no_window = s->no_leaders = false;
+   if ((s->no_stream || s->no_stream_nd || s->force_ll || s->no_window || s->no_leaders || s->no_batch) && --s->fallback_ttl <= 0)
+      s->no_stream = s->no_stream_nd = s->force_ll = s->no_window = s->no_leaders = s->no_batch = false;
    const size_t seg = nbytes < s->seg_bytes ? nbytes : s->seg_bytes;
    size_t want_lines = s->cap_lines, want_hl = s->cap_hitlines, want_rec = s->cap_records;
    if (!s->user_reserved) {
@@ -2018,7 +2057,8 @@
       if (h.overflow & 32u) s->force_ll = true;
       if (h.overflow & 128u) s->no_window = true;
       if (h.overflow & 256u) s->no_leaders = true;
-      if (h.overflow & (8u | 16u | 32u | 128u | 256u)) s->fallback_ttl = 32;
+      if (h.overflow & 512u) s->no_batch = true;
+      if (h.overflow & (8u | 16u | 32u | 128u | 256u | 512u)) s->fallback_ttl = 32;
       if (h.overflow & 4u) {
          nrec = (size_t)h.need_records + (size_t)(h.need_records >> 3) + 64;
       }
@@ -2471,6 +2511,8 @@
 }
 
 extern "C" int seeqdevScanLastLaunches(const seeqdev_scan_t *s) { return s ? (int)s->prof_segs : 0; }
+
+extern "C" int seeqdevScanLastBatches(const seeqdev_scan_t *s) { return s ? s->last_batches : 0; }
 
 extern "C" float seeqdevScanLastClockMHz(const seeqdev_scan_t *s) { return s ? s->clk_mhz : 0.f; }
 
diff --git a/seeq_amd/csrc/seeq_exact1.h b/seeq_amd/csrc/seeq_exact1.h
--- a/seeq_amd/csrc/seeq_exact1.h
+++ b/seeq_amd/csrc/seeq_exact1.h
@@ -144,7 +144,7 @@
       const uint32_t kk = (a.hit_idx && !done) ? a.hit_idx[k] : k;
       const uint32_t hs = done ? 0u : a.hit_start[kk];
       if (hs == 0xFFFFFFFFu) done = true;
-      const uint64_t off = done ? a.seg_base : a.seg_base + hs;
+      const uint64_t off = done ? a.seg_base : seeq_entry_base(a, kk) + hs;
       if (MODE == SQ_MODE_COUNT && trusted && count_any) {
          if (k < nhl) a.nh[k] = done ? 0u : 1u;
          continue;
@@ -392,7 +392,7 @@
       for (uint32_t e = 1u + (threadIdx.x & 63u); e <= novf; e += 64u) {
          const uint4 o = ovf[e];
          const uint32_t ox = a.hit_idx ? a.hit_idx[o.x] : o.x;
-         const uint64_t off = a.seg_base + a.hit_start[ox];
+         const uint64_t off = seeq_entry_base(a, ox) + a.hit_start[ox];
          const uint64_t slot = c->records + nh_at(a, o.x) + o.y;
          seeqdev_hit_t h;
          h.line = a.hit_line[ox];
diff --git a/seeq_amd/csrc/seeq_order.h b/seeq_amd/csrc/seeq_order.h
--- a/seeq_amd/csrc/seeq_order.h
+++ b/seeq_amd/csrc/seeq_order.h
@@ -46,10 +46,15 @@
    __syncthreads();
 }
 
-__global__ __launch_bounds__(256) void k_order(FusedArgs f, uint32_t nslices, const uint32_t *bsum, uint32_t nb, uint4 *ent)
+__global__ __launch_bounds__(256) void k_order(FusedArgs f, uint32_t nslices, const uint32_t *bsum, uint32_t nb, uint4 *ent, OrderBatch ob)
 {
    __shared__ uint32_t s_ph[ORDER_MAX_BLOCKS], s_pc[ORDER_MAX_BLOCKS], s_wave[4];
    order_block_prefix(bsum, nb, s_ph, s_pc, s_wave);
+   if (blockIdx.x == 0 && ob.bt_ent)
+      for (uint32_t sg = threadIdx.x; sg < ob.nseg; sg += 256u) {
+         const uint32_t t = sg * ob.tps;
+         ob.bt_ent[sg] = t < f.ntiles ? f.tile_hits[t] + s_ph[t / ORDER_SCAN_BLOCK] : 0xFFFFFFFFu;
+      }
    const Counters *c = f.cnt;
    if (c->overflow & 2u) return;
    const uint32_t lane = threadIdx.x & 63;
@@ -57,6 +62,7 @@
    for (uint32_t sl = blockIdx.x * 4 + (threadIdx.x >> 6); sl < nslices; sl += gridDim.x * 4) {
       const uint32_t n = f.wg_hits[sl];
       const uint4 *slice = f.tmp + (size_t)sl * f.slice_cap;
+      const uint32_t tile0 = (sl / ob.seg_slices) * ob.tps;
       for (uint32_t i0 = lane; i0 < n; i0 += 256) {
          uint4 e[4];
          uint32_t th[4], tc[4];
@@ -64,7 +70,7 @@
          for (int u = 0; u < 4; u++) e[u] = i0 + 64u * u < n ? slice[i0 + 64u * u] : make_uint4(0u, 0u, 0u, 0u);
 #pragma unroll
          for (int u = 0; u < 4; u++) {
-            const uint32_t tile = e[u].x & 0x1FFFFFFFu;
+            const uint32_t tile = (e[u].x & 0x1FFFFFFFu) + tile0;
             const bool ok = i0 + 64u * u < n;
             th[u] = ok ? f.tile_hits[tile] + s_ph[tile / ORDER_SCAN_BLOCK] : 0u;
             tc[u] = ok ? f.tile_cl[tile] + s_pc[tile / ORDER_SCAN_BLOCK] : 0u;
@@ -156,11 +162,18 @@
    Counters *c = a.cnt;
    const uint32_t nhl = c->seg_nhitlines;
    const uint32_t stride = gridDim.x * 256;
-   const uint64_t segb = a.seg_base + a.pos_bias;
    const uint32_t prev0 = c->prev_hit_line;
    for (uint32_t k = blockIdx.x * 256 + threadIdx.x; k < nhl; k += stride) {
       const uint4 e = ent[k];
       const uint32_t prev = k ? ent[k - 1].y : prev0;
+      uint64_t vbase = a.seg_base, segb = a.seg_base + a.pos_bias;
+      uint32_t seg_len = a.seg_len, before = prev0;
+      if (a.bt_n > 1u) {
+         const uint32_t sk = seeq_entry_seg(a, k), e0 = a.bt_ent[sk];
+         vbase = seeq_seg_vbase(a.bt_seg0 + sk, a.bt_seg_bytes, a.nbytes, &seg_len);
+         segb = (uint64_t)(a.bt_seg0 + sk) * a.bt_seg_bytes;
+         before = e0 ? ent[e0 - 1u].y : prev0;
+      }
       const uint32_t unresolved = e.z & 1u, col = e.z >> 1;
       a.hit_line[k] = e.y;
       uint32_t repeat = e.y == prev ? 1u : 0u;
@@ -175,10 +188,10 @@
       }
       if (repeat) {
          hit_col[k] = unresolved ? e.x : e.x + col;
-         if (a.window_ok && e.y == prev0) {
+         if (a.window_ok && e.y == before) {
             bool voids = true;
             if (a.ig_thr && (e.w & 2u) && unresolved) {
-               const uint64_t hp0 = a.seg_base + e.x;
+               const uint64_t hp0 = vbase + e.x;
                voids = hp0 < a.nbytes && order_marker_holds(a, order_line_start(a.text, hp0));
             }
             if (voids) atomicOr(&c->overflow, 128u);
@@ -189,14 +202,14 @@
       if (!unresolved) {
          uint32_t keep = 1u;
          if (a.ig_need != 0u && (e.w & 2u) != 0u) {
-            const uint32_t holds = order_marker_holds(a, a.seg_base + e.x) ? 1u : 0u;
+            const uint32_t holds = order_marker_holds(a, vbase + e.x) ? 1u : 0u;
             if (!holds) { keep = e.w & 1u; ent[k].w = e.w | 4u; }
          }
          a.hit_start[k] = keep ? e.x : 0xFFFFFFFFu; hit_col[k] = keep ? col : 0u;
          continue;
       }
-      const uint64_t hp = a.seg_base + e.x;
-      if (hp >= a.nbytes || hp < segb || hp >= segb + a.seg_len) {
+      const uint64_t hp = vbase + e.x;
+      if (hp >= a.nbytes || hp < segb || hp >= segb + seg_len) {
          atomicOr(&c->overflow, 64u);
          a.hit_start[k] = 0xFFFFFFFFu;
          hit_col[k] = 0u;
@@ -204,15 +217,15 @@
       }
       const uint64_t q = order_line_start(a.text, hp);
       uint32_t keep = 1u, holds = 1u;
-      if (a.ig_thr != 0u && (e.w & 2u) != 0u && q >= a.seg_base) holds = order_marker_holds(a, q) ? 1u : 0u;
+      if (a.ig_thr != 0u && (e.w & 2u) != 0u && q >= vbase) holds = order_marker_holds(a, q) ? 1u : 0u;
       if (!holds) {
          keep = e.w & 1u;
          ent[k].w = e.w | 4u;
       }
       uint32_t out_start, out_col;
-      if (q < a.seg_base) { atomicOr(&c->overflow, 8u); out_start = 0xFFFFFFFFu; out_col = 0u; }
+      if (q < vbase) { atomicOr(&c->overflow, 8u); out_start = 0xFFFFFFFFu; out_col = 0u; }
       else if (!keep) { out_start = 0xFFFFFFFFu; out_col = 0u; }
-      else { out_start = (uint32_t)(q - a.seg_base); out_col = (uint32_t)(hp - q); }
+      else { out_start = (uint32_t)(q - vbase); out_col = (uint32_t)(hp - q); }
       a.hit_start[k] = out_start;
       hit_col[k] = out_col;
    }
diff --git a/seeq_amd/csrc/seeq_plan.h b/seeq_amd/csrc/seeq_plan.h
--- a/seeq_amd/csrc/seeq_plan.h
+++ b/seeq_amd/csrc/seeq_plan.h
@@ -150,6 +150,22 @@
    return p;
 }
 
+#define SEEQ_BATCH_MAX_SEGS 16
+#define SEEQ_ORDER_MAX_TILES (1024ull * 2048ull)
+#define SEEQ_SEG_MAX_BYTES 0xFFFF0000ull
+#define SEEQ_STREAM_TILE_BYTES 8192u
+static_assert((SEEQ_SEG_MAX_BYTES + SEEQ_STREAM_TILE_BYTES - 1) / SEEQ_STREAM_TILE_BYTES <= SEEQ_ORDER_MAX_TILES, "a segment must fit one ordering");
+
+static inline size_t seeq_plan_batch(bool batching, size_t nseg, size_t first, size_t seg_bytes, uint32_t tile_bytes)
+{
+   if (!batching || first >= nseg || tile_bytes == 0) return 1;
+   const size_t tps = (seg_bytes + tile_bytes - 1) / tile_bytes;
+   size_t b = tps ? (size_t)(SEEQ_ORDER_MAX_TILES / tps) : 1;
+   if (b > SEEQ_BATCH_MAX_SEGS) b = SEEQ_BATCH_MAX_SEGS;
+   if (b > nseg - first) b = nseg - first;
+   return b ? b : 1;
+}
+
 static inline void seeq_plan_print(FILE *f, const PlanIn &in, const PlanAutomata &au, const ScanPlan &p)
 {
    static const char *const kname[8] = {"?", "generic (k_nl_* + k_forward)", "?", "k_direct", "?", "k_stream", "k_pair", "k_stream, Myers mode"};
diff --git a/seeq_amd/csrc/seeq_post.h b/seeq_amd/csrc/seeq_post.h
--- a/seeq_amd/csrc/seeq_post.h
+++ b/seeq_amd/csrc/seeq_post.h
@@ -20,7 +20,7 @@
 #define SEEQ_ORDER_MAX_BLOCKS 1024
 #define SEEQ_ORDER_BLOCK      2048
 void seeq_launch_tiles_post(hipStream_t st, const FusedArgs &f, uint32_t nslices, uint32_t *bsum, uint32_t nb);
-void seeq_launch_order(unsigned grid, hipStream_t st, const FusedArgs &f, uint32_t nslices, const uint32_t *bsum, uint32_t nb, uint4 *ent);
+void seeq_launch_order(unsigned grid, hipStream_t st, const FusedArgs &f, uint32_t nslices, const uint32_t *bsum, uint32_t nb, uint4 *ent, const OrderBatch &ob);
 void seeq_launch_bounds2(unsigned grid, hipStream_t st, const ScanArgs &a, uint4 *ent, uint32_t *hit_col);
 
 #endif
diff --git a/seeq_amd/csrc/seeq_scan_common.h b/seeq_amd/csrc/seeq_scan_common.h
--- a/seeq_amd/csrc/seeq_scan_common.h
+++ b/seeq_amd/csrc/seeq_scan_common.h
@@ -50,6 +50,8 @@
    Counters      *cnt;
 };
 
+struct OrderBatch { uint32_t seg_slices, tps, nseg; uint32_t *bt_ent; };
+
 __device__ __forceinline__ void fused_step(uint32_t eq, uint32_t &pv, uint32_t &mv, uint32_t &score)
 {
    const uint32_t s = (eq & pv) + pv;
@@ -201,19 +203,20 @@
 __device__ __forceinline__ void fused_post_body(const FusedArgs &a, uint32_t nslices)
 {
    __shared__ uint32_t s_red[4][4];
-   uint32_t lines = 0, hdrs = 0, hits = 0, mx = 0, ovf = 0, lastnl = 0, flags = 0, busy = 0, crowded = 0;
+   uint64_t lines = 0;
+   uint32_t hdrs = 0, hits = 0, mx = 0, ovf = 0, lastnl = 0, flags = 0, busy = 0, crowded = 0;
    const uint4 *part = reinterpret_cast<const uint4 *>(a.wg_part);
-   for (uint32_t i0 = threadIdx.x; i0 < nslices; i0 += 2048) {
-      uint4 pv[8];
-      uint32_t lv[8];
-#pragma unroll
-      for (int u = 0; u < 8; u++) {
+   for (uint32_t i0 = threadIdx.x; i0 < nslices; i0 += 4096) {
+      uint4 pv[16];
+      uint32_t lv[16];
+#pragma unroll
+      for (int u = 0; u < 16; u++) {
          const uint32_t i = i0 + 256u * u;
          pv[u] = i < nslices ? part[i] : make_uint4(0u, 0u, 0u, 0u);
          lv[u] = a.wg_lastnl && i < nslices ? a.wg_lastnl[i] : 0u;
       }
 #pragma unroll
-      for (int u = 0; u < 8; u++) {
+      for (int u = 0; u < 16; u++) {
          lastnl = lv[u] > lastnl ? lv[u] : lastnl;
          lines += pv[u].x;
          hdrs += pv[u].y;
@@ -241,14 +244,15 @@
       lastnl = ol > lastnl ? ol : lastnl;
    }
    __shared__ uint32_t s_last[4], s_flags[4], s_busy[4], s_crowded[4];
+   __shared__ uint64_t s_lines[4];
    const int w = threadIdx.x >> 6;
-   if ((threadIdx.x & 63) == 0) { s_last[w] = lastnl; s_flags[w] = flags; s_busy[w] = busy; s_crowded[w] = crowded; }
-   if ((threadIdx.x & 63) == 0) { s_red[w][0] = lines; s_red[w][1] = hdrs; s_red[w][2] = hits; s_red[w][3] = mx | (ovf << 31); }
+   if ((threadIdx.x & 63) == 0) { s_last[w] = lastnl; s_flags[w] = flags; s_busy[w] = busy; s_crowded[w] = crowded; s_lines[w] = lines; }
+   if ((threadIdx.x & 63) == 0) { s_red[w][1] = hdrs; s_red[w][2] = hits; s_red[w][3] = mx | (ovf << 31); }
    __syncthreads();
    if (threadIdx.x == 0) {
-      lines = hdrs = hits = mx = ovf = 0;
+      lines = 0; hdrs = hits = mx = ovf = 0;
       for (int k = 0; k < 4; k++) {
-         lines += s_red[k][0]; hdrs += s_red[k][1]; hits += s_red[k][2];
+         lines += s_lines[k]; hdrs += s_red[k][1]; hits += s_red[k][2];
          const uint32_t m = s_red[k][3] & 0x7FFFFFFFu;
          mx = m > mx ? m : mx;
          ovf |= s_red[k][3] >> 31;
@@ -266,7 +270,8 @@
          if ((a.options & MASK_NONDNA) == SQ_IGNORE && crowded * 2 > busy) c->overflow |= 16u;
       }
       if (flags & 2u) c->overflow |= 32u;
-      c->seg_nlines = lines;
+      if (lines > 0xFFFFFFFFull) atomicOr(&c->overflow, 512u);
+      c->seg_nlines = (uint32_t)lines;
       c->seg_nheaders = hdrs;
       const uint64_t need = (uint64_t)mx * nslices + (uint64_t)nslices * 64;
       if (need > c->need_hitlines) c->need_hitlines = need > 0xFFFFFFFFull ? 0xFFFFFFFFu : (uint32_t)need;
diff --git a/seeq_amd/csrc/seeq_types.h b/seeq_amd/csrc/seeq_types.h
--- a/seeq_amd/csrc/seeq_types.h
+++ b/seeq_amd/csrc/seeq_types.h
@@ -71,11 +71,49 @@
    uint32_t        ig_need, ig_bval, ig_bmask;
    const uint4    *ig_ent;
    uint32_t        vrange;
+   uint32_t        bt_n;
+   uint32_t        bt_seg0;
+   uint64_t        bt_seg_bytes;
+   const uint32_t *bt_ent;
    Counters      *cnt;
 };
 
 #if defined(__HIPCC__)
+__host__ __device__
+#endif
+static inline uint32_t seeq_pos_bias(uint64_t seg_base, uint32_t seg_len)
+{
+   uint64_t room = 0xFFFFFFF0ull - seg_len;
+   if (room > ((uint64_t)1 << 30)) room = (uint64_t)1 << 30;
+   return (uint32_t)(seg_base < room ? seg_base : room) & ~127u;
+}
+#if defined(__HIPCC__)
+__host__ __device__
+#endif
+static inline uint64_t seeq_seg_vbase(uint64_t g, uint64_t seg_bytes, uint64_t nbytes, uint32_t *seg_len)
+{
+   const uint64_t b = g * seg_bytes;
+   const uint32_t len = (uint32_t)(nbytes - b < seg_bytes ? nbytes - b : seg_bytes);
+   if (seg_len) *seg_len = len;
+   return b - seeq_pos_bias(b, len);
+}
+
+#if defined(__HIPCC__)
 __device__ __forceinline__ uint32_t nh_at(const ScanArgs &a, uint32_t k) { return a.nh[k] + (a.nh_sum ? a.nh_sum[k >> 8] : 0u); }
+__device__ __forceinline__ uint32_t seeq_entry_seg(const ScanArgs &a, uint32_t k)
+{
+   uint32_t lo = 0, hi = a.bt_n - 1u;
+   while (lo < hi) {
+      const uint32_t mid = (lo + hi + 1u) >> 1;
+      if (a.bt_ent[mid] <= k) lo = mid; else hi = mid - 1u;
+   }
+   return lo;
+}
+__device__ __forceinline__ uint64_t seeq_entry_base(const ScanArgs &a, uint32_t k)
+{
+   if (a.bt_n <= 1u) return a.seg_base;
+   return seeq_seg_vbase(a.bt_seg0 + seeq_entry_seg(a, k), a.bt_seg_bytes, a.nbytes, nullptr);
+}
 __device__ __forceinline__ uint64_t rec_off_of(const ScanArgs &a, uint64_t off, uint32_t line) { return a.rec_pitch ? (uint64_t)(line - 1u) * a.rec_pitch : off; }
 #endif
 
diff --git a/seeq_amd/csrc/seeq_verify.h b/seeq_amd/csrc/seeq_verify.h
--- a/seeq_amd/csrc/seeq_verify.h
+++ b/seeq_amd/csrc/seeq_verify.h
@@ -248,7 +248,7 @@
       const uint32_t kk = (a.hit_idx && !done) ? a.hit_idx[k] : k;
       const uint32_t hs = done ? 0u : a.hit_start[kk];
       if (hs == 0xFFFFFFFFu) done = true;
-      const uint64_t off = done ? a.seg_base : a.seg_base + hs;
+      const uint64_t off = done ? a.seg_base : seeq_entry_base(a, kk) + hs;
       if (a.use_nh == 3 && (a.options & SEEQDEV_FASTA) && !done && a.text[off] == '>') done = true;
       uint32_t pos = 0, stop_at = 0xFFFFFFFFu;
       if (!done) {
@@ -374,6 +374,7 @@
    const uint32_t nhl = c->seg_nhitlines;
    const uint32_t nch = (nhl + 255u) >> 8;
    uint32_t running = 0, nz = 0;
+   uint64_t total = 0;
    for (uint32_t b0 = 0; b0 < nch; b0 += 2048u) {
       uint32_t item[8], v = 0;
 #pragma unroll
@@ -393,6 +394,7 @@
          ex += item[q];
       }
       running += tot;
+      total += tot;
    }
    if (a.nz_sum) {
       uint32_t tot;
@@ -400,6 +402,7 @@
       nz = tot;
    }
    if (threadIdx.x == 0) {
+      if (total > 0xFFFFFFFFull) atomicOr(&c->overflow, 512u);
       c->seg_nrec = running;
       if (a.nz_sum) c->seg_nmatch = nz;
       if (a.want == SEEQDEV_WANT_RECORDS) rec_check_body(a);
@@ -426,7 +429,7 @@
       h.end = ce.x;
       h.dist = ce.y;
       a.records[slot] = h;
-      a.rec_off[slot] = rec_off_of(a, a.seg_base + a.hit_start[kk], h.line);
+      a.rec_off[slot] = rec_off_of(a, seeq_entry_base(a, kk) + a.hit_start[kk], h.line);
    }
 }
 
@@ -456,7 +459,7 @@
       h.end = ce.x;
       h.dist = ce.y;
       a.records[slot] = h;
-      a.rec_off[slot] = rec_off_of(a, a.seg_base + a.hit_start[kk], h.line);
+      a.rec_off[slot] = rec_off_of(a, seeq_entry_base(a, kk) + a.hit_start[kk], h.line);
    }
    const uint32_t nlists = vgrid * 4u;
    const uint32_t ovf_r = (a.cap_hitlines > nhl ? a.cap_hitlines - nhl : 0u) / nlists;
@@ -470,7 +473,7 @@
          const uint4 o = need ? ovf[e0 + lane] : make_uint4(0u, 0u, 0u, 0u);
          const uint32_t ox = (need && a.hit_idx) ? a.hit_idx[o.x] : o.x;
          const uint32_t hs = need ? a.hit_start[ox] : 0u;
-         const uint64_t off = a.seg_base + hs;
+         const uint64_t off = (need ? seeq_entry_base(a, ox) : a.seg_base) + hs;
          const uint32_t s0 = verify_reverse<W>(a, need, off, o.z, o.w, eqr_base, sh, m, tau1);
          if (need) {
             const uint64_t slot = base + nh_at(a, o.x) + o.y;
diff --git a/seeq_amd/csrc/seeq_verify.hip b/seeq_amd/csrc/seeq_verify.hip
--- a/seeq_amd/csrc/seeq_verify.hip
+++ b/seeq_amd/csrc/seeq_verify.hip
@@ -44,9 +44,9 @@
    hipLaunchKernelGGL(k_tiles_post, dim3(nb ? nb : 1, 3), dim3(256), 0, st, f, nslices, bsum, nb);
 }
 
-void seeq_launch_order(unsigned grid, hipStream_t st, const FusedArgs &f, uint32_t nslices, const uint32_t *bsum, uint32_t nb, uint4 *ent)
+void seeq_launch_order(unsigned grid, hipStream_t st, const FusedArgs &f, uint32_t nslices, const uint32_t *bsum, uint32_t nb, uint4 *ent, const OrderBatch &ob)
 {
-   hipLaunchKernelGGL(k_order, dim3(grid), dim3(256), 0, st, f, nslices, bsum, nb, ent);
+   hipLaunchKernelGGL(k_order, dim3(grid), dim3(256), 0, st, f, nslices, bsum, nb, ent, ob);
 }
 
 void seeq_launch_bounds2(unsigned grid, hipStream_t st, const ScanArgs &a, uint4 *ent, uint32_t *hit_col)
diff --git a/seeq_amd/device.py b/seeq_amd/device.py
--- a/seeq_amd/device.py
+++ b/seeq_amd/device.py
@@ -153,6 +153,9 @@
         _check(self._lib.seeqdevScanLastTimes(self._h, ms))
         return dict(index=ms[0], forward=ms[1], exact=ms[2], total=ms[3],
                     forward_launches=self._lib.seeqdevScanLastLaunches(self._h))
+
+    def last_batches(self):
+        return int(self._lib.seeqdevScanLastBatches(self._h))
 
     def last_clock_mhz(self):
         return float(self._lib.seeqdevScanLastClockMHz(self._h))
```

Result: no change. 26.51 billion, median of 6 (-0.8%).
